# Kr-Stam/CUDA_Optical_Flow_2

Hardware: AMD Instinct MI355X
Metric: Mpix/s dense LK flow (higher is better)
Workload: dtype i32/f64; 1 GPU; 3840x2160 pair, 5-level pyramid, 9x9 window, iters=5 (BASELINE.json config as written; iterations = extension lk_iter: bilinear-warp refinement, iteration 1 = the reference bit for bit), mode lk_float, stream path: new frame's pyramid + every LK level and iteration, inputs resident in HBM; SURVEY 8d's smooth texture translating by (2,1) px per frame; warmup_steps_run=5

## Files before the change

### cuda_optical_flow_2_amd/build.py

```python
from __future__ import annotations

import os
import shutil
import subprocess
import sys
from concurrent.futures import ThreadPoolExecutor

PKG = os.path.dirname(os.path.abspath(__file__))
ROOT = os.path.dirname(PKG)
CSRC = os.path.join(PKG, "csrc")
INCLUDE = os.path.join(ROOT, "include")
OUT = os.path.join(PKG, os.environ.get("OFX_BUILD_OUT", "libofx_hip.so"))
OBJ = os.path.join(PKG, "csrc", "_obj" + os.environ.get("OFX_BUILD_TAG", ""))
ARCH = "gfx950"

SOURCES = ["lk_inst_stream_f8.hip", "lk_inst_stream_fast8.hip", "lk_inst_stream_fw.hip", "lk_inst_stream_fastw.hip", "lk_inst_stream_fwr.hip", "lk_inst_stream_fastwr.hip", "lk_inst_iter_f4.hip", "lk_inst_iter_fast4.hip", "lk_inst_stream_f.hip", "lk_inst_stream_fast.hip", "lk_inst_stream_c.hip", "lk_inst_levels_f.hip", "lk_inst_levels_fast.hip",
           "lk_inst_levels_c.hip", "lk_inst_iter_f2.hip", "lk_inst_iter_fast2.hip", "lk_inst_iter_f3.hip", "lk_inst_iter_fast3.hip", "lk_inst_iter_f1.hip", "lk_inst_iter_fast1.hip", "lk_level.hip", "corner.hip", "pyr_corner.hip", "pyramid.hip", "compose_ring.hip", "sample_ring.hip", "frontend.hip", "primitives.hip", "srm_march.hip", "ofx_core.cpp", "session.cpp",
           "compat_gpu.cpp", "compat_cpu.cpp", "compat_stage.cpp"]
FLAGS = ["-O3", "-std=c++17", "-fPIC", "-ffp-contract=off", "-fno-slp-vectorize", f"--offload-arch={ARCH}", "-I" + INCLUDE, "-I" + CSRC,
         "-Wall", "-Wno-unused-function"] + os.environ.get("OFX_BUILD_DEFS", "").split()


def hipcc() -> str:
    exe = shutil.which("hipcc") or "/opt/rocm/bin/hipcc"
    if not os.path.exists(exe):
        raise RuntimeError("hipcc not found: the HIP library cannot be built (there is no CPU fallback)")
    return exe


def _stale(target: str, deps) -> bool:
    if not os.path.exists(target):
        return True
    t = os.path.getmtime(target)
    return any(os.path.getmtime(d) > t for d in deps)


def _headers():
    hs = [os.path.join(CSRC, f) for f in os.listdir(CSRC) if f.endswith(".h")]
    hs += [os.path.join(INCLUDE, f) for f in os.listdir(INCLUDE)]
    return hs


def build(force: bool = False, verbose: bool = False) -> str:
    os.makedirs(OBJ, exist_ok=True)
    cc = hipcc()
    hdrs = _headers()
    srcs = [s for s in SOURCES if os.path.exists(os.path.join(CSRC, s))]
    jobs = []
    for s in srcs:
        src = os.path.join(CSRC, s)
        obj = os.path.join(OBJ, s + ".o")
        if force or _stale(obj, [src] + hdrs):
            lang = ["-x", "hip"] if s.endswith(".cpp") else []
            jobs.append((s, [cc] + FLAGS + lang + ["-c", src, "-o", obj]))

    def run(job):
        name, cmd = job
        r = subprocess.run(cmd, capture_output=True, text=True)
        if r.returncode != 0:
            raise RuntimeError(f"hipcc failed on {name}:\n{r.stderr}")
        if verbose and r.stderr.strip():
            print(r.stderr, file=sys.stderr)
        return name

    if jobs:
        with ThreadPoolExecutor(max_workers=min(os.cpu_count() or 4, 8, len(jobs))) as ex:
            list(ex.map(run, jobs))
    objs = [os.path.join(OBJ, s + ".o") for s in srcs]
    if force or jobs or _stale(OUT, objs):
        cmd = [cc, "-shared", "-fPIC", "-pthread", "-Wl,--no-undefined", f"--offload-arch={ARCH}", "-o", OUT] + objs + ["-ldl"]
        r = subprocess.run(cmd, capture_output=True, text=True)
        if r.returncode != 0:
            raise RuntimeError("link failed:\n" + r.stderr)
    return OUT


if __name__ == "__main__":
    print(build(force="--force" in sys.argv, verbose=True))
```

### cuda_optical_flow_2_amd/csrc/lk_body.h

```cpp
#pragma once

#include <type_traits>

#include "lk_solve.h"
#include "ofx_internal.h"

namespace ofx_dev {

struct LkArgs {
    const uint8_t *prev;
    const uint8_t *next;
    const float *uv;
    float *flow;
    int32_t *sums;
    size_t sums_plane;
    int w, h, pitch, row0, row_end;
    int out_y0, out_y1, flow_row0;
    int strip_h, tiles_x;
    int accumulate;
    float min_det;
    const uint8_t *warp_src;
    uint8_t *warp_out;
    float warp_scale;
    int *warp_status;
    int warp_status_bit;
};

struct LkTable {
    LkArgs lv[OFX_MAX_LK_ITEMS];
    int first_block[OFX_MAX_LK_ITEMS + 1];
    int n;
};

#define OFX_GLOBAL __attribute__((address_space(1)))
struct __attribute__((packed)) UnalignedU32 {
    uint32_t v;
};
typedef float f32x2 __attribute__((ext_vector_type(2)));
typedef float f32x4 __attribute__((ext_vector_type(4)));
__device__ __forceinline__ uint32_t lane_off(uint32_t off)
{
    asm volatile("" : "+v"(off));
    return off;
}
__device__ __forceinline__ uint32_t lane_off_var(uint32_t &off)
{
    asm volatile("" : "+v"(off));
    return off;
}
__device__ __forceinline__ uint32_t gload_u32_var(const uint8_t *base, uint32_t &off)
{
    return *(const OFX_GLOBAL uint32_t *)((const OFX_GLOBAL uint8_t *)base + lane_off_var(off));
}
__device__ __forceinline__ uint32_t gload_u32_unaligned_var(const uint8_t *base, uint32_t &off)
{
    return ((const OFX_GLOBAL UnalignedU32 *)((const OFX_GLOBAL uint8_t *)base + lane_off_var(off)))->v;
}
__device__ __forceinline__ uint32_t gload_u32(const uint8_t *base, uint32_t off)
{
    return *(const OFX_GLOBAL uint32_t *)((const OFX_GLOBAL uint8_t *)base + lane_off(off));
}
__device__ __forceinline__ uint32_t gload_u32_nt(const uint8_t *base, uint32_t off)
{
    return __builtin_nontemporal_load((const OFX_GLOBAL uint32_t *)((const OFX_GLOBAL uint8_t *)base + lane_off(off)));
}
typedef OFX_GLOBAL float *gfloat_ptr;
__device__ __forceinline__ gfloat_ptr gptr_f32_var(float *base, uint32_t &byte_off)
{
    return (gfloat_ptr)((OFX_GLOBAL uint8_t *)base + lane_off_var(byte_off));
}
__device__ __forceinline__ void gstore_f32x2(gfloat_ptr p, float a, float b)
{
    __builtin_nontemporal_store(f32x2{a, b}, (OFX_GLOBAL f32x2 *)p);
}
__device__ __forceinline__ void gstore_f32x4(gfloat_ptr p, f32x4 v)
{
    typedef float f32x4_a8 __attribute__((ext_vector_type(4), aligned(8)));
    __builtin_nontemporal_store((f32x4_a8)v, (OFX_GLOBAL f32x4_a8 *)p);
}
__device__ __forceinline__ void gstore_i32(int32_t *p, int32_t v) { *(OFX_GLOBAL int32_t *)p = v; }
__device__ __forceinline__ void gstore_u32(uint8_t *base, uint32_t off, uint32_t v)
{
    *(OFX_GLOBAL uint32_t *)((OFX_GLOBAL uint8_t *)base + lane_off(off)) = v;
}
__device__ __forceinline__ void gstore_u32x2(uint8_t *base, uint32_t off, uint32_t a, uint32_t b)
{
    typedef uint32_t u32x2 __attribute__((ext_vector_type(2), aligned(4)));
    *(OFX_GLOBAL u32x2 *)((OFX_GLOBAL uint8_t *)base + lane_off(off)) = u32x2{a, b};
}
__device__ __forceinline__ void gstore_u16(uint8_t *base, uint32_t off, uint16_t v)
{
    *(OFX_GLOBAL uint16_t *)((OFX_GLOBAL uint8_t *)base + lane_off(off)) = v;
}
__device__ __forceinline__ void gstore_u8(uint8_t *base, uint32_t off, uint8_t v) { *((OFX_GLOBAL uint8_t *)base + lane_off(off)) = v; }

template <typename T>
__device__ __forceinline__ void pin_scalar(T &x)
{
    asm volatile("" : "+s"(x));
}

__device__ __forceinline__ int lane_shift_right(int x)
{
    int r = __builtin_amdgcn_update_dpp(0, x, 0x138 , 0xf, 0xf, true);
    asm volatile("" : "+v"(r));
    return r;
}
__device__ __forceinline__ int lane_shift_left(int x)
{
    int r = __builtin_amdgcn_update_dpp(0, x, 0x130 , 0xf, 0xf, true);
    asm volatile("" : "+v"(r));
    return r;
}

template <int D>
__device__ __forceinline__ int lane_from(int x)
{
    if constexpr (D == 0) {
        return x;
    } else if constexpr (D > 0) {
        return lane_from<D - 1>(lane_shift_left(x));
    } else {
        return lane_from<D + 1>(lane_shift_right(x));
    }
}

template <int D>
__device__ __forceinline__ int add_from(int acc, int x)
{
    if constexpr (D == 0) {
        return acc + x;
    } else {
        const int near = lane_from<(D > 0 ? D - 1 : D + 1)>(x);
        int r = acc + __builtin_amdgcn_update_dpp(0, near, D > 0 ? 0x130  : 0x138 , 0xf, 0xf, true);
        asm volatile("" : "+v"(r));
        return r;
    }
}

template <int R, int I, int D>
__device__ __forceinline__ int hbox_right(const int (&q)[4], int acc)
{
    constexpr int hi = I + R;
    if constexpr (hi < 4 * D) {
        return acc;
    } else if constexpr (hi >= 4 * D + 3) {
        return hbox_right<R, I, D + 1>(q, add_from<D>(acc, q[3]));
    } else {
        return add_from<D>(acc, q[hi - 4 * D]);
    }
}

template <int R, int I, int D>
__device__ __forceinline__ int hbox_left(const int (&s)[4], int acc)
{
    constexpr int lo = I - R;
    if constexpr (lo > -4 * D + 3) {
        return acc;
    } else if constexpr (lo <= -4 * D) {
        return hbox_left<R, I, D + 1>(s, add_from<-D>(acc, s[0]));
    } else {
        return add_from<-D>(acc, s[lo + 4 * D]);
    }
}

template <int R, int I>
__device__ __forceinline__ int hbox_one(const int (&q)[4], const int (&s)[4])
{
    constexpr int lo = I - R, hi = I + R;
    constexpr int olo = lo > 0 ? lo : 0, ohi = hi < 3 ? hi : 3;
    int own;
    if constexpr (olo == 0) {
        own = q[ohi];
    } else if constexpr (ohi == 3) {
        own = s[olo];
    } else {
        own = q[ohi] - q[olo - 1];
    }
    return hbox_left<R, I, 1>(s, hbox_right<R, I, 1>(q, own));
}

template <int C>
__device__ __forceinline__ int col_minus(const int (&a)[4], int y)
{
    if constexpr (C >= 0 && C <= 3) {
        return a[C] - y;
    } else {
        constexpr int idx = ((C % 4) + 4) % 4;
        constexpr int dist = (C - idx) / 4;
        const int near = lane_from<(dist > 0 ? dist - 1 : dist + 1)>(a[idx]);
        int r = __builtin_amdgcn_update_dpp(0, near, dist > 0 ? 0x130  : 0x138 , 0xf, 0xf, true) - y;
        asm volatile("" : "+v"(r));
        return r;
    }
}

template <int R>
__device__ __forceinline__ void hbox4(const int (&a)[4], int (&out)[4])
{
    int q[4], s[4];
    q[0] = a[0];
    q[1] = q[0] + a[1];
    q[2] = q[1] + a[2];
    q[3] = q[2] + a[3];
    s[3] = a[3];
    s[2] = s[3] + a[2];
    s[1] = s[2] + a[1];
    s[0] = q[3];
    out[0] = hbox_one<R, 0>(q, s);
    out[3] = hbox_one<R, 3>(q, s);
    out[1] = col_minus<1 + R>(a, col_minus<0 - R>(a, out[0]));
    out[2] = col_minus<2 - R>(a, col_minus<3 + R>(a, out[3]));
}

template <int K>
__device__ __forceinline__ void lane_from5(const int (&x)[5], int (&r)[5])
{
    if constexpr (K == 0) {
#pragma unroll
        for (int n = 0; n < 5; ++n) r[n] = x[n];
    } else {
        int t[5];
#pragma unroll
        for (int n = 0; n < 5; ++n) t[n] = K > 0 ? lane_shift_left(x[n]) : lane_shift_right(x[n]);
        lane_from5<(K > 0 ? K - 1 : K + 1)>(t, r);
    }
}

template <int D>
__device__ __forceinline__ void add_from5(int (&acc)[5], const int (&x)[5])
{
    if constexpr (D == 0) {
#pragma unroll
        for (int n = 0; n < 5; ++n) acc[n] += x[n];
    } else {
        int near[5];
        lane_from5<(D > 0 ? D - 1 : D + 1)>(x, near);
#pragma unroll
        for (int n = 0; n < 5; ++n) {
            int r = acc[n] + __builtin_amdgcn_update_dpp(0, near[n], D > 0 ? 0x130  : 0x138 , 0xf, 0xf, true);
            asm volatile("" : "+v"(r));
            acc[n] = r;
        }
    }
}

template <int C>
__device__ __forceinline__ void column5(const int (&a)[5][4], int (&x)[5])
{
#pragma unroll
    for (int n = 0; n < 5; ++n) x[n] = a[n][C];
}

template <int R, int I, int D>
__device__ __forceinline__ void hbox_right5(const int (&q)[5][4], int (&acc)[5])
{
    constexpr int hi = I + R;
    if constexpr (hi < 4 * D) {
        return;
    } else if constexpr (hi >= 4 * D + 3) {
        int x[5];
        column5<3>(q, x);
        add_from5<D>(acc, x);
        hbox_right5<R, I, D + 1>(q, acc);
    } else {
        int x[5];
        column5<hi - 4 * D>(q, x);
        add_from5<D>(acc, x);
    }
}

template <int R, int I, int D>
__device__ __forceinline__ void hbox_left5(const int (&s)[5][4], int (&acc)[5])
{
    constexpr int lo = I - R;
    if constexpr (lo > -4 * D + 3) {
        return;
    } else if constexpr (lo <= -4 * D) {
        int x[5];
        column5<0>(s, x);
        add_from5<-D>(acc, x);
        hbox_left5<R, I, D + 1>(s, acc);
    } else {
        int x[5];
        column5<lo + 4 * D>(s, x);
        add_from5<-D>(acc, x);
    }
}

template <int R, int I>
__device__ __forceinline__ void hbox_one5(const int (&q)[5][4], const int (&s)[5][4], int (&out)[5])
{
    constexpr int lo = I - R, hi = I + R;
    constexpr int olo = lo > 0 ? lo : 0, ohi = hi < 3 ? hi : 3;
#pragma unroll
    for (int n = 0; n < 5; ++n) {
        if constexpr (olo == 0) out[n] = q[n][ohi];
        else if constexpr (ohi == 3) out[n] = s[n][olo];
        else out[n] = q[n][ohi] - q[n][olo - 1];
    }
    hbox_right5<R, I, 1>(q, out);
    hbox_left5<R, I, 1>(s, out);
}

template <int C>
__device__ __forceinline__ void col_minus5(const int (&a)[5][4], const int (&y)[5], int (&r)[5])
{
    if constexpr (C >= 0 && C <= 3) {
#pragma unroll
        for (int n = 0; n < 5; ++n) r[n] = a[n][C] - y[n];
    } else {
        constexpr int idx = ((C % 4) + 4) % 4;
        constexpr int dist = (C - idx) / 4;
        int x[5], near[5];
        column5<idx>(a, x);
        lane_from5<(dist > 0 ? dist - 1 : dist + 1)>(x, near);
#pragma unroll
        for (int n = 0; n < 5; ++n) {
            int t = __builtin_amdgcn_update_dpp(0, near[n], dist > 0 ? 0x130  : 0x138 , 0xf, 0xf, true) - y[n];
            asm volatile("" : "+v"(t));
            r[n] = t;
        }
    }
}

template <int R>
__device__ __forceinline__ void hbox4x5(const int (&a)[5][4], int (&out)[5][4])
{
    int q[5][4], s[5][4];
#pragma unroll
    for (int n = 0; n < 5; ++n) {
        q[n][0] = a[n][0];
        q[n][1] = q[n][0] + a[n][1];
        q[n][2] = q[n][1] + a[n][2];
        q[n][3] = q[n][2] + a[n][3];
        s[n][3] = a[n][3];
        s[n][2] = s[n][3] + a[n][2];
        s[n][1] = s[n][2] + a[n][1];
        s[n][0] = q[n][3];
    }
    int o0[5], o1[5], o2[5], o3[5];
    hbox_one5<R, 0>(q, s, o0);
    hbox_one5<R, 3>(q, s, o3);
    int t[5];
    col_minus5<0 - R>(a, o0, t);
    col_minus5<1 + R>(a, t, o1);
    col_minus5<3 + R>(a, o3, t);
    col_minus5<2 - R>(a, t, o2);
#pragma unroll
    for (int n = 0; n < 5; ++n) out[n][0] = o0[n], out[n][1] = o1[n], out[n][2] = o2[n], out[n][3] = o3[n];
}

template <int R>
struct TileGeom {
    static constexpr int LO_LANE = (R + 1 + 3) / 4;
    static constexpr int HI_LANE = (251 - R) / 4;
    static constexpr int OUT_W = (HI_LANE - LO_LANE + 1) * 4;
};

typedef short s2 __attribute__((ext_vector_type(2)));

__device__ __forceinline__ s2 as_s2(uint32_t v) { return __builtin_bit_cast(s2, v); }
__device__ __forceinline__ uint32_t as_u32(s2 v) { return __builtin_bit_cast(uint32_t, v); }
__device__ __forceinline__ s2 lane_shift_s2(s2 v, bool from_left)
{
    return as_s2((uint32_t)(from_left ? lane_shift_right((int)as_u32(v)) : lane_shift_left((int)as_u32(v))));
}

__device__ __forceinline__ s2 pk_two()
{
    uint32_t v = 0x00020002u;
    asm volatile("" : "+s"(v));
    return as_s2(v);
}

template <int MODE>
struct RowPk;
template <>
struct RowPk<OFX_MODE_LK_FLOAT> {
    s2 p[4];
    s2 d[4];
};
template <>
struct RowPk<OFX_MODE_COMPAT_CPU> {
    s2 p[4];
    s2 n[4];
};

__device__ __forceinline__ void pin_row(RowPk<OFX_MODE_LK_FLOAT> &r)
{
    asm volatile("" : "+v"(r.p[0]), "+v"(r.p[1]), "+v"(r.p[2]), "+v"(r.p[3]), "+v"(r.d[0]), "+v"(r.d[1]), "+v"(r.d[2]), "+v"(r.d[3]));
}
__device__ __forceinline__ void pin_row(RowPk<OFX_MODE_COMPAT_CPU> &r)
{
    asm volatile("" : "+v"(r.p[0]), "+v"(r.p[1]), "+v"(r.p[2]), "+v"(r.p[3]), "+v"(r.n[0]), "+v"(r.n[1]), "+v"(r.n[2]), "+v"(r.n[3]));
}

template <int J>
__device__ __forceinline__ s2 pair_bytes(uint32_t in_raw, uint32_t out_raw)
{
    constexpr uint32_t sel = (uint32_t)J | (0x0cu << 8) | ((uint32_t)(4 + J) << 16) | (0x0cu << 24);
    return as_s2(__builtin_amdgcn_perm(out_raw, in_raw, sel));
}

__device__ __forceinline__ void unpack_pk(uint32_t pi, uint32_t ni, uint32_t po, uint32_t no, RowPk<OFX_MODE_LK_FLOAT> &r)
{
    r.p[0] = pair_bytes<0>(pi, po);
    r.p[1] = pair_bytes<1>(pi, po);
    r.p[2] = pair_bytes<2>(pi, po);
    r.p[3] = pair_bytes<3>(pi, po);
    r.d[0] = pair_bytes<0>(ni, no) - r.p[0];
    r.d[1] = pair_bytes<1>(ni, no) - r.p[1];
    r.d[2] = pair_bytes<2>(ni, no) - r.p[2];
    r.d[3] = pair_bytes<3>(ni, no) - r.p[3];
}

__device__ __forceinline__ void unpack_pk(uint32_t pi, uint32_t ni, uint32_t po, uint32_t no, RowPk<OFX_MODE_COMPAT_CPU> &r)
{
    r.p[0] = pair_bytes<0>(pi, po);
    r.p[1] = pair_bytes<1>(pi, po);
    r.p[2] = pair_bytes<2>(pi, po);
    r.p[3] = pair_bytes<3>(pi, po);
    r.n[0] = pair_bytes<0>(ni, no);
    r.n[1] = pair_bytes<1>(ni, no);
    r.n[2] = pair_bytes<2>(ni, no);
    r.n[3] = pair_bytes<3>(ni, no);
}

__device__ __forceinline__ void derivs_pk(const RowPk<OFX_MODE_LK_FLOAT> &t, const RowPk<OFX_MODE_LK_FLOAT> &m,
                                          const RowPk<OFX_MODE_LK_FLOAT> &b, const s2 two, s2 (&ix)[4], s2 (&iy)[4], s2 (&it)[4])
{
    s2 sm[6], df[6], g[6];
#pragma unroll
    for (int j = 0; j < 4; ++j) {
        sm[j + 1] = m.p[j] * two + (t.p[j] + b.p[j]);
        df[j + 1] = b.p[j] - t.p[j];
        g[j + 1] = m.d[j] * two + (t.d[j] + b.d[j]);
    }
    sm[0] = lane_shift_s2(sm[4], true);
    sm[5] = lane_shift_s2(sm[1], false);
    df[0] = lane_shift_s2(df[4], true);
    df[5] = lane_shift_s2(df[1], false);
    g[0] = lane_shift_s2(g[4], true);
    g[5] = lane_shift_s2(g[1], false);
#pragma unroll
    for (int j = 0; j < 4; ++j) {
        ix[j] = sm[j + 2] - sm[j];
        iy[j] = df[j + 1] * two + (df[j] + df[j + 2]);
        it[j] = g[j + 1] * two + (g[j] + g[j + 2]) - m.d[j];
    }
}

__device__ __forceinline__ void derivs_pk(const RowPk<OFX_MODE_COMPAT_CPU> &t, const RowPk<OFX_MODE_COMPAT_CPU> &m,
                                          const RowPk<OFX_MODE_COMPAT_CPU> &b, const s2, s2 (&ix)[4], s2 (&iy)[4], s2 (&it)[4])
{
    s2 sm[6], df[6], sp[6], sn[6], mp[4], mn[4];
#pragma unroll
    for (int j = 0; j < 4; ++j) {
        sm[j + 1] = (m.p[j] + m.p[j]) + t.p[j] + b.p[j];
        df[j + 1] = b.p[j] - t.p[j];
        sp[j + 1] = (t.p[j] >> 4) + (m.p[j] >> 3) + (b.p[j] >> 4);
        sn[j + 1] = (t.n[j] >> 4) + (m.n[j] >> 3) + (b.n[j] >> 4);
        mp[j] = (t.p[j] >> 3) + (m.p[j] >> 2) + (b.p[j] >> 3);
        mn[j] = (t.n[j] >> 3) + (m.n[j] >> 2) + (b.n[j] >> 3);
    }
    sm[0] = lane_shift_s2(sm[4], true);
    sm[5] = lane_shift_s2(sm[1], false);
    df[0] = lane_shift_s2(df[4], true);
    df[5] = lane_shift_s2(df[1], false);
    sp[0] = lane_shift_s2(sp[4], true);
    sp[5] = lane_shift_s2(sp[1], false);
    sn[0] = lane_shift_s2(sn[4], true);
    sn[5] = lane_shift_s2(sn[1], false);
#pragma unroll
    for (int j = 0; j < 4; ++j) {
        constexpr uint32_t m8 = 0x00ff00ffu;
        ix[j] = as_s2(as_u32(sm[j + 2] - sm[j]) & m8);
        iy[j] = as_s2(as_u32((df[j + 1] + df[j + 1]) + df[j] + df[j + 2]) & m8);
        const s2 gp = sp[j] + mp[j] + sp[j + 2], gn = sn[j] + mn[j] + sn[j + 2];
        it[j] = as_s2(as_u32(gn - gp) & 0x00ff00ffu);
    }
}

__device__ __forceinline__ void accumulate_pk(const s2 (&ix)[4], const s2 (&iy)[4], const s2 (&it)[4], const uint32_t (&mm)[4],
                                              int (&vxx)[4], int (&vyy)[4], int (&vxy)[4], int (&vxt)[4], int (&vyt)[4])
{
#pragma unroll
    for (int j = 0; j < 4; ++j) {
        const s2 nx = ix[j] * as_s2(mm[j]), ny = iy[j] * as_s2(mm[j]);
        vxx[j] = __builtin_amdgcn_sdot2(ix[j], nx, vxx[j], false);
        vyy[j] = __builtin_amdgcn_sdot2(iy[j], ny, vyy[j], false);
        vxy[j] = __builtin_amdgcn_sdot2(ix[j], ny, vxy[j], false);
        vxt[j] = __builtin_amdgcn_sdot2(nx, it[j], vxt[j], false);
        vyt[j] = __builtin_amdgcn_sdot2(ny, it[j], vyt[j], false);
    }
}

constexpr int kLkWaveLds = 2048 + 128;
typedef __attribute__((address_space(3))) uint8_t *lds_ptr;

template <int R, int MODE, bool SUMS, bool MAY_ACC, bool FAST, bool INTERIOR>
__device__ __forceinline__ void lk_wave_impl(const LkTable &T, int wave, int lane, uint8_t *xlds)
{
    using G = TileGeom<R>;
    constexpr int NS = 2 * R + 1;

    if (wave >= T.first_block[T.n]) return;
    int level = 0, hi = T.n;
    while (hi - level > 1) {
        const int mid = (level + hi) >> 1;
        if (wave >= T.first_block[mid]) level = mid;
        else hi = mid;
    }
    LkArgs A = T.lv[level];
    pin_scalar(A.prev);
    pin_scalar(A.next);
    pin_scalar(A.flow);
    pin_scalar(A.w);
    pin_scalar(A.h);
    pin_scalar(A.pitch);
    pin_scalar(A.row0);
    pin_scalar(A.row_end);
    pin_scalar(A.flow_row0);
    pin_scalar(A.accumulate);
    pin_scalar(A.min_det);
    const SolveOpts sopt{A.min_det};
    if constexpr (SUMS) {
        pin_scalar(A.sums);
        pin_scalar(A.sums_plane);
    }
    const int block = wave - T.first_block[level];
    const int tile = block % A.tiles_x;
    const int strip = block / A.tiles_x;
    const int cb = tile * G::OUT_W - G::LO_LANE * 4 + 4 * lane;
    const int ys = A.out_y0 + strip * A.strip_h;
    const int ye = min(ys + A.strip_h, A.out_y1);

    const bool ld_ok = INTERIOR || (cb >= 0 && cb < A.w);
    uint32_t bmask = INTERIOR ? 0xffffffffu : 0u;
    int cm[4] = {-1, -1, -1, -1};
    if constexpr (!INTERIOR) {
#pragma unroll
        for (int j = 0; j < 4; ++j) {
            const bool in = (cb + j) >= 0 && (cb + j) < A.w;
            cm[j] = in ? -1 : 0;
            bmask |= in ? (0xffu << (8 * j)) : 0u;
        }
    }
    uint32_t col_off = ld_ok ? (uint32_t)cb : 0u;
    uint32_t flow_off = 8u * (uint32_t)(cb > 0 ? cb : 0);
    const int x0 = tile * G::OUT_W;
    const int nv = min(x0 + G::OUT_W, A.w) - x0;
    uint32_t l16 = 16u * (uint32_t)lane;
    const int lim = 8 * nv - 16, c16 = 16 * lane;
    const bool st_lo4 = c16 <= lim, st_lo2 = c16 == lim + 8, st_hi4 = c16 <= lim - 1024, st_hi2 = c16 == lim + 8 - 1024;
    const lds_ptr xl_w = (lds_ptr)xlds + 32 * lane;
    const lds_ptr xl_base = (lds_ptr)xlds + 32 * G::LO_LANE;

    const int y_lim = min(min(ye + R + 1, A.h), A.row_end);
    const int y_min = max(0, A.row0);
    auto fetch_row = [&](const uint8_t *img, int y) -> uint32_t {
        uint32_t v = 0u;
        if (y >= y_min && y < y_lim) {
            const uint8_t *row = img + (size_t)(uint32_t)(y - A.row0) * (size_t)(uint32_t)A.pitch;
            pin_scalar(row);
            v = gload_u32_var(row, col_off);
        }
        return v;
    };
    auto finish_row = [&](uint32_t raw) -> uint32_t {
        if constexpr (INTERIOR) return raw;
        else return raw & bmask;
    };

    const float su = A.uv ? A.uv[0] : 0.0f, sv = A.uv ? A.uv[1] : 0.0f;
    uint32_t nb_off = 0u, sel = 0u, own_sel = 0u;
    bool all_in;
    {
        int n[4], nb = 0x7fffffff;
        bool in[4], lane_all_in = true;
#pragma unroll
        for (int j = 0; j < 4; ++j) {
            const int x = cb + j;
            const float tx = (float)x + su;
            in[j] = x >= 0 && x < A.w && tx > -1.0f && tx < (float)A.w;
            n[j] = in[j] ? (int)tx : 0;
            if (in[j]) nb = min(nb, n[j]);
        }
        nb = max(0, min(nb == 0x7fffffff ? 0 : nb, A.pitch - 4));
        sel = 0u;
#pragma unroll
        for (int j = 0; j < 4; ++j) {
            const int x = cb + j;
            const uint32_t sj = !(x >= 0 && x < A.w) ? 0x0cu : (in[j] ? (uint32_t)(n[j] - nb) : (uint32_t)(4 + j));
            sel |= sj << (8 * j);
            own_sel |= (!(x >= 0 && x < A.w) ? 0x0cu : (uint32_t)(4 + j)) << (8 * j);
            if (x >= 0 && x < A.w && !in[j]) lane_all_in = false;
        }
        nb_off = (uint32_t)nb;
        all_in = __all(lane_all_in) != 0;
    }
    const int y_none = (A.h + 2) / 3, y_part = (A.h % 3) ? A.h / 3 : -1;
    struct NextRaw {
        uint32_t own, sh;
        uint32_t have;
    };
    int map_base = 0, row_map = -1;
    auto refresh_map = [&](int y0) {
        map_base = y0;
        const float ty = (float)(y0 + lane) + sv;
        const bool yin = ty > -1.0f && ty < (float)A.h;
        const int ny = yin ? (int)ty : 0;
        row_map = (yin && ny >= A.row0 && ny < A.row_end) ? ny : -1;
    };
    auto fetch_next = [&](int y) -> NextRaw {
        NextRaw r = {0u, 0u, 0u};
        if (y >= y_min && y < y_lim) {
            const int ny = __builtin_amdgcn_readlane(row_map, y - map_base);
            const bool have = ny >= 0;
            r.have = have ? ~0u : 0u;
            if (have) {
                const uint8_t *srow = A.next + (size_t)(uint32_t)(ny - A.row0) * (size_t)(uint32_t)A.pitch;
                pin_scalar(srow);
                r.sh = gload_u32_unaligned_var(srow, nb_off);
            }
            if (!(have && all_in) && y < y_none) {
                const uint8_t *orow = A.next + (size_t)(uint32_t)(y - A.row0) * (size_t)(uint32_t)A.pitch;
                pin_scalar(orow);
                r.own = gload_u32_var(orow, col_off);
                if (y == y_part) {
                    uint32_t km = 0u;
#pragma unroll
                    for (int j = 0; j < 4; ++j)
                        if (3ll * (cb + j) < (long long)A.w * (A.h % 3)) km |= 0xffu << (8 * j);
                    r.own &= km;
                }
            }
        }
        return r;
    };
    auto finish_next = [&](const NextRaw &r) -> uint32_t {
        return __builtin_amdgcn_perm(r.own, r.sh, (sel & r.have) | (own_sel & ~r.have));
    };
    auto load_row = [&](const uint8_t *img, int y) -> uint32_t { return finish_row(fetch_row(img, y)); };
    auto load_next = [&](int y) -> uint32_t { return finish_next(fetch_next(y)); };

    constexpr int H = R - 1;
    constexpr int PR = 2 * R - H;
    const int y_first = ys - R;
    const int y_lo0 = y_first + H;
    const int nsteps = (ye - ys) + PR;
    RowPk<MODE> wp[3];
    const s2 two = pk_two();
    auto fetch_out_prev = [&](int r) -> uint32_t { return r < y_first - 1 ? 0u : fetch_row(A.prev, r); };
    auto fetch_out_next = [&](int r) -> NextRaw { return r < y_first - 1 ? NextRaw{0u, 0u, 0u} : fetch_next(r); };
    refresh_map(y_first - 1);
    if constexpr (H > 0) {
        unpack_pk(load_row(A.prev, y_lo0 - 1), load_next(y_lo0 - 1), load_row(A.prev, y_first - 1), load_next(y_first - 1), wp[0]);
        unpack_pk(load_row(A.prev, y_lo0), load_next(y_lo0), load_row(A.prev, y_first), load_next(y_first), wp[1]);
        unpack_pk(load_row(A.prev, y_lo0 + 1), load_next(y_lo0 + 1), load_row(A.prev, y_first + 1), load_next(y_first + 1), wp[2]);
    } else {
        unpack_pk(load_row(A.prev, y_lo0 - 1), load_next(y_lo0 - 1), 0u, 0u, wp[0]);
        unpack_pk(load_row(A.prev, y_lo0), load_next(y_lo0), 0u, 0u, wp[1]);
        unpack_pk(load_row(A.prev, y_lo0 + 1), load_next(y_lo0 + 1), 0u, 0u, wp[2]);
    }

    int vxx[4] = {0, 0, 0, 0}, vyy[4] = {0, 0, 0, 0}, vxy[4] = {0, 0, 0, 0}, vxt[4] = {0, 0, 0, 0}, vyt[4] = {0, 0, 0, 0};

    auto body = [&](auto K, int s) {
        constexpr int k = decltype(K)::value;
        const int yy = y_lo0 + s;
        const int yo = yy - NS;
        const bool folded = H > 0 && s < H;
        const int yh = folded ? y_first + s : yo;

        if (yy + 2 - map_base >= 64) refresh_map(yo + 2);
        const int ro = (H > 1 && s + 1 < H) ? y_first + s + 2 : yo + 2;
        const uint32_t pf_ip = fetch_row(A.prev, yy + 2), pf_op = fetch_out_prev(ro);
        const NextRaw pf_in = fetch_next(yy + 2), pf_on = fetch_out_next(ro);
        const bool emit = s >= PR;
        const int y = yy - R;
        const bool out_lane = lane >= G::LO_LANE && lane <= G::HI_LANE && cb < A.w;
        const size_t rowpix = (size_t)(y - A.flow_row0) * (size_t)A.w;
        float old_uv[8] = {0.0f, 0.0f, 0.0f, 0.0f, 0.0f, 0.0f, 0.0f, 0.0f};
        if constexpr (!SUMS && MAY_ACC) {
            if (A.accumulate && emit && out_lane) {
                float *frow = A.flow + 2 * rowpix;
                pin_scalar(frow);
                const gfloat_ptr src = gptr_f32_var(frow, flow_off);
#pragma unroll
                for (int j = 0; j < 4; ++j)
                    if (cb + j < A.w) old_uv[2 * j] = src[2 * j], old_uv[2 * j + 1] = src[2 * j + 1];
            }
        }

        const uint32_t him = folded ? 0x00010000u : (yo >= y_first ? 0xffff0000u : 0u);
        uint32_t rowm = ((yy >= 0 && yy < A.h) ? 0x00000001u : 0u) | ((yh >= 0 && yh < A.h) ? him : 0u);
        if constexpr (INTERIOR) rowm = (uint32_t)__builtin_amdgcn_readfirstlane((int)rowm);
        const uint32_t mm[4] = {(uint32_t)cm[0] & rowm, (uint32_t)cm[1] & rowm, (uint32_t)cm[2] & rowm, (uint32_t)cm[3] & rowm};
        s2 ix[4], iy[4], it[4];
        derivs_pk(wp[k], wp[(k + 1) % 3], wp[(k + 2) % 3], two, ix, iy, it);
        accumulate_pk(ix, iy, it, mm, vxx, vyy, vxy, vxt, vyt);
        auto take_rows = [&]() {
            __builtin_amdgcn_sched_barrier(0);
            unpack_pk(finish_row(pf_ip), finish_next(pf_in), finish_row(pf_op), finish_next(pf_on), wp[k]);
            pin_row(wp[k]);
        };

        int hxx[4], hyy[4], hxy[4], hxt[4], hyt[4];
        float uv[8];
        f32x4 xlo, xhi;
        asm("" : "=v"(xlo), "=v"(xhi));
        if (emit) {
            hbox4<R>(vxx, hxx);
            hbox4<R>(vyy, hyy);
            hbox4<R>(vxy, hxy);
            hbox4<R>(vxt, hxt);
            hbox4<R>(vyt, hyt);
            if constexpr (!SUMS) {
                solve_lane<MODE, FAST>(hxx, hyy, hxy, hxt, hyt, sopt, uv);
                if constexpr (MAY_ACC) {
                    if (A.accumulate) {
#pragma unroll
                        for (int j = 0; j < 8; ++j) uv[j] = old_uv[j] + uv[j];
                    }
                }
                *(__attribute__((address_space(3))) f32x4 *)(xl_w) = f32x4{uv[0], uv[1], uv[2], uv[3]};
                *(__attribute__((address_space(3))) f32x4 *)(xl_w + 16) = f32x4{uv[4], uv[5], uv[6], uv[7]};
                __builtin_amdgcn_fence(__ATOMIC_SEQ_CST, "wavefront");
                __builtin_amdgcn_wave_barrier();
                const lds_ptr xl_r = xl_base + lane_off_var(l16);
                xlo = *(__attribute__((address_space(3))) f32x4 *)(xl_r);
                xhi = *(__attribute__((address_space(3))) f32x4 *)(xl_r + 1024);
            }
        }
        take_rows();
        if (emit) {
            if constexpr (SUMS) {
                if (out_lane) {
                    const size_t pix = rowpix + (uint32_t)cb;
#pragma unroll
                    for (int j = 0; j < 4; ++j) {
                        if (cb + j < A.w) {
                            gstore_i32(A.sums + pix + j, hxx[j]);
                            gstore_i32(A.sums + A.sums_plane + pix + j, hyy[j]);
                            gstore_i32(A.sums + 2 * A.sums_plane + pix + j, hxy[j]);
                            gstore_i32(A.sums + 3 * A.sums_plane + pix + j, hxt[j]);
                            gstore_i32(A.sums + 4 * A.sums_plane + pix + j, hyt[j]);
                        }
                    }
                }
            } else {
                float *frow = A.flow + 2 * (rowpix + (size_t)x0);
                pin_scalar(frow);
                if (st_lo4) {
                    gstore_f32x4(gptr_f32_var(frow, l16), xlo);
                } else if (st_lo2) {
                    gstore_f32x2(gptr_f32_var(frow, l16), xlo.x, xlo.y);
                }
                if (st_hi4) {
                    gstore_f32x4(gptr_f32_var(frow, l16) + 256, xhi);
                } else if (st_hi2) {
                    gstore_f32x2(gptr_f32_var(frow, l16) + 256, xhi.x, xhi.y);
                }
            }
        }
    };

    const int q1 = nsteps / 4, q2 = nsteps / 2, q3 = nsteps - nsteps / 4;
    __builtin_amdgcn_s_setprio(3);
#define OFX_LK_PRIO_STEP()                               \
    do {                                                 \
        if (s >= q3) __builtin_amdgcn_s_setprio(0);      \
        else if (s >= q2) __builtin_amdgcn_s_setprio(1); \
        else if (s >= q1) __builtin_amdgcn_s_setprio(2); \
    } while (0)
    int s = 0;
    while (true) {
        body(std::integral_constant<int, 0>{}, s);
        if (++s >= nsteps) break;
        body(std::integral_constant<int, 1>{}, s);
        if (++s >= nsteps) break;
        body(std::integral_constant<int, 2>{}, s);
        if (++s >= nsteps) break;
        OFX_LK_PRIO_STEP();
    }
}


}
#include "lk_body_warp.h"
#include "lk_body_buf.h"
#include "lk_body_wide.h"
#undef OFX_LK_PRIO_STEP
namespace ofx_dev {

template <int R, int MODE, bool SUMS, bool MAY_ACC = true, bool FAST = false, bool LDS_ROWS = false, int ITER = 0>
__device__ __forceinline__ void lk_wave(const LkTable &T, int wave, int lane, uint8_t *xlds)
{
    if (wave >= T.first_block[T.n]) return;
    int level = 0, hi = T.n;
    while (hi - level > 1) {
        const int mid = (level + hi) >> 1;
        if (wave >= T.first_block[mid]) level = mid;
        else hi = mid;
    }
    const int tile = (wave - T.first_block[level]) % T.lv[level].tiles_x;
    const int cb0 = tile * TileGeom<R>::OUT_W - TileGeom<R>::LO_LANE * 4;
    if constexpr (!SUMS && !MAY_ACC) {
        if (cb0 >= 0 && cb0 + 256 <= T.lv[level].w) lk_wave_buf<R, MODE, FAST, true, LDS_ROWS, ITER>(T, wave, lane, xlds);
        else lk_wave_buf<R, MODE, FAST, false, LDS_ROWS, ITER>(T, wave, lane, xlds);
        return;
    }
    if (cb0 >= 0 && cb0 + 256 <= T.lv[level].w) lk_wave_impl<R, MODE, SUMS, MAY_ACC, FAST, true>(T, wave, lane, xlds);
    else lk_wave_impl<R, MODE, SUMS, MAY_ACC, FAST, false>(T, wave, lane, xlds);
}

}
```

### cuda_optical_flow_2_amd/csrc/lk_inst.h

```cpp
#pragma once

#include "lk_launch.h"

namespace ofx_launch {

template <int MODE, bool FAST>
int levels(int radius, const LkLevelIn *lv, int n, bool sums, hipStream_t st)
{
    int rc = OFX_E_UNSUPPORTED;
    const bool known = dispatch_radius<lk_max_radius(MODE)>(radius, [&](auto R) {
        if constexpr (!FAST) {
            if (sums) {
                rc = launch_r<decltype(R)::value, MODE, true, false>(lv, n, st);
                return;
            }
        }
        rc = launch_r<decltype(R)::value, MODE, false, FAST>(lv, n, st);
    });
    if (!known) ofx_set_error("ofx_lk_level: window %d not supported in mode %d", 2 * radius + 1, MODE);
    return rc;
}

template <int MODE, bool FAST, int ITER, int NC>
int iter(int radius, const LkLevelIn *lv, int n, hipStream_t st)
{
    int rc = OFX_E_UNSUPPORTED;
    const bool known = dispatch_radius<lk_max_radius(MODE, NC)>(radius, [&](auto R) {
        if constexpr (NC == 8) rc = launch_iter_rd<decltype(R)::value, MODE, FAST, ITER, false, 8>(lv, n, st);
        else rc = launch_iter_r<decltype(R)::value, MODE, FAST, ITER>(lv, n, st);
    });
    if (!known) {
        if constexpr (NC == 8) ofx_set_error("ofx_lk_levels: window %d not supported with eight columns per lane", 2 * radius + 1);
        else ofx_set_error("ofx_lk_level: window %d not supported in mode %d", 2 * radius + 1, MODE);
    }
    return rc;
}

template <int MODE, bool FAST, int WOUT, int NC>
int stream(int radius, const LkLevelIn *lv, int n, StreamArgs &S, const int *stage_blocks, size_t lds, hipStream_t st)
{
    int rc = OFX_E_UNSUPPORTED;
    const bool known = dispatch_radius<lk_max_radius(MODE, NC)>(radius, [&](auto R) {
        if constexpr (NC == 8) rc = launch_stream_rd<decltype(R)::value, MODE, FAST, false, WOUT, 8>(lv, n, S, stage_blocks, lds, st);
        else rc = launch_stream_r<decltype(R)::value, MODE, FAST, WOUT>(lv, n, S, stage_blocks, lds, st);
    });
    if (!known) {
        if constexpr (NC == 8) ofx_set_error("ofx_stream_launch: window %d not supported with eight columns per lane", 2 * radius + 1);
        else ofx_set_error("ofx_stream_launch: window %d not supported in mode %d", 2 * radius + 1, MODE);
    }
    return rc;
}

}
```

### cuda_optical_flow_2_amd/csrc/lk_launch.h

```cpp
#pragma once

#include <stdio.h>
#include <stdlib.h>

#include "corner_body.h"
#include "lk_body.h"
#include "pyr_march.h"
#include "stages_body.h"

using namespace ofx_dev;

namespace ofx_launch {
constexpr int kPyrStages = 2 * OFX_STREAM_MAX_BATCH;
using ofx_dev::kCornerScratch;
struct StreamArgs {
    LkTable lk;
    PyrMarchArgs pyr[kPyrStages];
    CornerHead corner[OFX_STREAM_MAX_BATCH];
    CornerLevel corner_lv[OFX_MAX_LK_ITEMS];
    PatchBuild patch;
    int patch_build;
    PatchBuildSlot patch_slot[OFX_STREAM_MAX_BATCH];
    int first[kPyrStages + 1];
    int n_corner;
    unsigned long long *trace;
    int trace_blocks;
};
struct LkLevelIn {
    LkArgs a;
    int rows_out;
};
}

namespace {

constexpr int kLkMinWaves = 3;
template <int R, int MODE, bool SUMS, bool FAST>
__global__ __launch_bounds__(64, kLkMinWaves) void lk_level_kernel(const LkTable T)
{
    __shared__ __attribute__((aligned(16))) uint8_t xlds[kLkWaveLds];
    lk_wave<R, MODE, SUMS, true, FAST>(T, (int)blockIdx.x, (int)threadIdx.x, xlds);
}

template <int R, int MODE, bool FAST, int ITER, bool DMA = false, int NC = 4>
__global__ __launch_bounds__(64, NC == 8 ? 2 : 3) void lk_iter_kernel(const LkTable T)
{
    __shared__ __attribute__((aligned(16))) uint8_t xlds[NC == 8 ? kLkWaveLdsW : (DMA ? kLkWaveLdsDma : kLkWaveLdsX)];
    const int wave = (int)blockIdx.x, lane = (int)threadIdx.x;
    if constexpr (NC == 8) {
        static_assert(!DMA, "the wide march has no deep fetch");
        lk_wave_w<R, MODE, FAST, ITER, 8>(T, wave, lane, xlds);
        return;
    }
    if (wave >= T.first_block[T.n]) return;
    int level = 0, hi = T.n;
    while (hi - level > 1) {
        const int mid = (level + hi) >> 1;
        if (wave >= T.first_block[mid]) level = mid;
        else hi = mid;
    }
    const int tile = (wave - T.first_block[level]) % T.lv[level].tiles_x;
    const int cb0 = tile * TileGeom<R>::OUT_W - TileGeom<R>::LO_LANE * 4;
    if (cb0 >= 0 && cb0 + 256 <= T.lv[level].w) lk_wave_buf<R, MODE, FAST, true, DMA, ITER>(T, wave, lane, xlds);
    else lk_wave_buf<R, MODE, FAST, false, DMA, ITER>(T, wave, lane, xlds);
}

using ofx_launch::kCornerScratch;
using ofx_launch::kPyrStages;
using ofx_launch::StreamArgs;

}
namespace ofx_launch {
extern unsigned long long *g_stream_trace;
extern int g_stream_trace_blocks;
extern int g_trace_header[2 * OFX_STREAM_MAX_BATCH + 1];
extern thread_local int g_stream_deep_fetch;
}
namespace {
using ofx_launch::g_stream_trace;
using ofx_launch::g_stream_trace_blocks;
using ofx_launch::g_trace_header;
using ofx_launch::g_stream_deep_fetch;

constexpr int kPyrPrio = 3;
constexpr int stream_min_blocks(int mode, int wout, int nc)
{
    return nc == 8 ? (wout ? 2 : 3) : (wout ? 3 : (mode == OFX_MODE_LK_FLOAT ? 5 : 4));
}
template <int R, int MODE, bool FAST, bool DMA, int WOUT = 0, int NC = 4>
__global__ __launch_bounds__(256, stream_min_blocks(MODE, WOUT, NC)) void stream_kernel(const StreamArgs S)
{
    extern __shared__ __attribute__((aligned(16))) uint8_t lds[];
    const int b = (int)blockIdx.x, tid = (int)threadIdx.x;
    const unsigned long long t_start = S.trace ? wall_clock64() : 0ull;
    const int wv = __builtin_amdgcn_readfirstlane(tid >> 6);
    if (b < OFX_STREAM_MAX_BATCH) {
        __builtin_amdgcn_s_setprio(3);
        if (b < S.n_corner) {
            if (S.patch_build) patch_build_block(S.patch, S.patch_slot[b], tid);
            corner_block<MODE, FAST>(S.corner[b], S.corner_lv + S.corner[b].lv0, S.patch, tid, wv, reinterpret_cast<float *>(lds), lds + kCornerScratch,
                                     reinterpret_cast<int *>(lds + kCornerScratch - 32));
        }
    } else if (b < S.first[0]) {
        if constexpr (NC == 8) lk_wave_w<R, MODE, FAST, WOUT, 8>(S.lk, 4 * (b - OFX_STREAM_MAX_BATCH) + wv, tid & 63, lds + wv * kLkWaveLdsW);
        else lk_wave<R, MODE, false, false, FAST, DMA, WOUT>(S.lk, 4 * (b - OFX_STREAM_MAX_BATCH) + wv, tid & 63, lds + wv * (DMA ? kLkWaveLdsDma : kLkWaveLdsX));
    } else {
        int i = 0;
        while (i + 1 < kPyrStages && b >= S.first[i + 1]) ++i;
        __builtin_amdgcn_s_setprio(kPyrPrio);
        pyr_march_wave(S.pyr[i], 4 * (b - S.first[i]) + wv, tid & 63);
    }
    if (S.trace && b < S.trace_blocks && (tid & 63) == 0) {
        const unsigned hw = __builtin_amdgcn_s_getreg((4) | (0 << 6) | (15 << 11));
        const unsigned xcc = __builtin_amdgcn_s_getreg((20) | (0 << 6) | (3 << 11));
        S.trace[2 * (4 * b + wv)] = t_start;
        S.trace[2 * (4 * b + wv) + 1] = (wall_clock64() & 0x0000ffffffffffffull) | ((unsigned long long)(hw & 0xffffu) << 48);
        S.trace[2 * (4 * b + wv)] = (t_start & 0x0000ffffffffffffull) | ((unsigned long long)(xcc & 0xfu) << 48);
    }
}

using ofx_launch::LkLevelIn;

int env_int(const char *name, int dflt)
{
    const char *e = getenv(name);
    return e && atoi(e) > 0 ? atoi(e) : dflt;
}

template <int R, int NC = 4>
int plan_table(const LkLevelIn *lv, int n, int capacity, LkTable *out)
{
    using G = TileGeomW<R, NC>;
    const int min_h = env_int("OFX_LK_MIN_STRIP", 8);
    int max_rows = 1;
    for (int i = 0; i < n; ++i) max_rows = lv[i].rows_out > max_rows ? lv[i].rows_out : max_rows;
    auto height = [&](int i, int H) {
        const int hi = H < min_h ? min_h : H;
        return hi < lv[i].rows_out ? hi : lv[i].rows_out;
    };
    auto item_waves = [&](int i, int H) { return (long)ofx_div_up(lv[i].a.w, G::OUT_W) * ofx_div_up(lv[i].rows_out, height(i, H)); };
    int strip_h = min_h;
    for (; strip_h < max_rows; ++strip_h) {
        long waves = 0;
        for (int i = 0; i < n; ++i) waves += item_waves(i, strip_h);
        if (waves <= (long)capacity) break;
    }
    LkTable t{};
    t.n = n;
    int blocks = 0;
    for (int i = 0; i < n; ++i) {
        t.lv[i] = lv[i].a;
        t.lv[i].tiles_x = ofx_div_up(lv[i].a.w, G::OUT_W);
        t.lv[i].strip_h = height(i, strip_h);
        t.first_block[i] = blocks;
        blocks += t.lv[i].tiles_x * ofx_div_up(lv[i].rows_out, t.lv[i].strip_h);
    }
    t.first_block[n] = blocks;
    *out = t;
    return blocks;
}

template <typename K>
int lk_wave_target(K kernel, int threads, size_t lds, int reserve, int dflt_per_simd)
{
    int dev = 0, cus = 256, per_cu = 0;
    hipDeviceProp_t prop;
    if (hipGetDevice(&dev) == hipSuccess && hipGetDeviceProperties(&prop, dev) == hipSuccess) cus = prop.multiProcessorCount;
    if (hipOccupancyMaxActiveBlocksPerMultiprocessor(&per_cu, kernel, threads, lds) != hipSuccess || per_cu <= 0) per_cu = 8 * 64 / threads;
    (void)hipGetLastError();
    const int occ = per_cu * (threads / 64) / 4;
    int per_simd = env_int("OFX_LK_WAVES_PER_SIMD", dflt_per_simd);
    if (per_simd > occ - reserve) per_simd = occ - reserve;
    if (per_simd < 1) per_simd = 1;
    const int fill = env_int("OFX_LK_FILL", per_simd < occ ? 100 : 95);
    return env_int("OFX_LK_TARGET_WAVES", (int)((long)cus * 4 * per_simd * fill / 100));
}

template <int R, int MODE, bool SUMS, bool FAST>
int launch_r(const LkLevelIn *lv, int n, hipStream_t st)
{
    static const int capacity = lk_wave_target(lk_level_kernel<R, MODE, SUMS, FAST>, 64, 0, 0, 4);
    LkTable t{};
    const int blocks = plan_table<R>(lv, n, capacity, &t);
    hipLaunchKernelGGL((lk_level_kernel<R, MODE, SUMS, FAST>), dim3((unsigned)blocks), dim3(64), 0, st, t);
    OFX_HIP(hipGetLastError());
    return OFX_OK;
}

template <int R, int MODE, bool FAST, int ITER, bool DMA, int NC = 4>
int launch_iter_rd(const LkLevelIn *lv, int n, hipStream_t st)
{
    static const int capacity = lk_wave_target(lk_iter_kernel<R, MODE, FAST, ITER, DMA, NC>, 64, 0, 0, NC == 8 ? env_int("OFX_WIDE_WAVES_PER_SIMD", 2) : 4);
    LkTable t{};
    const int blocks = plan_table<R, NC>(lv, n, capacity, &t);
    hipLaunchKernelGGL((lk_iter_kernel<R, MODE, FAST, ITER, DMA, NC>), dim3((unsigned)blocks), dim3(64), 0, st, t);
    OFX_HIP(hipGetLastError());
    return OFX_OK;
}

template <int R, int MODE, bool FAST, int ITER>
int launch_iter_r(const LkLevelIn *lv, int n, hipStream_t st)
{
    static const int forced = [] { const char *e = getenv("OFX_ITER_DMA"); return e ? atoi(e) : -1; }();
    long max_px = 0;
    for (int i = 0; i < n; ++i) max_px = (long)lv[i].a.w * lv[i].a.h > max_px ? (long)lv[i].a.w * lv[i].a.h : max_px;
    if (forced > 0 || (forced < 0 && max_px >= 16l * 1000 * 1000)) return launch_iter_rd<R, MODE, FAST, ITER, true>(lv, n, st);
    return launch_iter_rd<R, MODE, FAST, ITER, false>(lv, n, st);
}

template <int R, int MODE, bool FAST, bool DMA, int WOUT, int NC = 4>
int launch_stream_rd(const LkLevelIn *lv, int n, StreamArgs &S, const int *stage_blocks, size_t lds, hipStream_t st)
{
    constexpr size_t wave_lds = NC == 8 ? kLkWaveLdsW : (DMA ? kLkWaveLdsDma : kLkWaveLdsX);
    static const int capacity1 = lk_wave_target(stream_kernel<R, MODE, FAST, DMA, WOUT, NC>, 256, 4 * wave_lds, 1, NC == 8 ? 1 : 2);
    static const int capacity2 = lk_wave_target(stream_kernel<R, MODE, FAST, DMA, WOUT, NC>, 256, 4 * wave_lds, 1, NC == 8 ? env_int("OFX_WIDE_WAVES_PER_SIMD", 2) : 4);
    int pairs = 0;
    for (int i = 0; i < n; ++i) pairs += (lv[i].a.w == lv[0].a.w && lv[i].a.h == lv[0].a.h) ? 1 : 0;
    const int capacity = pairs >= 2 ? capacity2 : capacity1;
    int lk_blocks = 0;
    if (n > 0) lk_blocks = ofx_div_up(plan_table<R, NC>(lv, n, capacity, &S.lk), 4);
    S.first[0] = OFX_STREAM_MAX_BATCH + lk_blocks;
    for (int i = 0; i < kPyrStages; ++i) S.first[i + 1] = S.first[i] + stage_blocks[i];
    const int blocks = S.first[kPyrStages];
    S.trace = g_stream_trace;
    S.trace_blocks = g_stream_trace_blocks;
    if (g_stream_trace)
        for (int i = 0; i <= kPyrStages; ++i) g_trace_header[i] = S.first[i];
    size_t corner_lds = 0;
    for (int i = 0; i < S.n_corner; ++i) {
        const size_t need = (size_t)kCornerScratch + kCornerTileBytes + (size_t)S.corner[i].levels * kCornerCacheBytes;
        corner_lds = need > corner_lds ? need : corner_lds;
    }
    if (lds < corner_lds) lds = corner_lds;
    if (lds < 4 * wave_lds) lds = 4 * wave_lds;
    hipLaunchKernelGGL((stream_kernel<R, MODE, FAST, DMA, WOUT, NC>), dim3((unsigned)blocks), dim3(256), lds, st, S);
    OFX_HIP(hipGetLastError());
    return OFX_OK;
}

template <int R, int MODE, bool FAST, int WOUT>
int launch_stream_r(const LkLevelIn *lv, int n, StreamArgs &S, const int *stage_blocks, size_t lds, hipStream_t st)
{
    if constexpr (!WOUT) {
        static const int forced = [] { const char *e = getenv("OFX_LK_DMA"); return e ? atoi(e) : -1; }();
        long max_px = 0;
        for (int i = 0; i < n; ++i) max_px = (long)lv[i].a.w * lv[i].a.h > max_px ? (long)lv[i].a.w * lv[i].a.h : max_px;
        const int want = forced >= 0 ? (forced > 0 ? 1 : -1) : g_stream_deep_fetch;
        if (want > 0 || (want == 0 && max_px >= 16l * 1000 * 1000)) return launch_stream_rd<R, MODE, FAST, true, WOUT>(lv, n, S, stage_blocks, lds, st);
    }
    return launch_stream_rd<R, MODE, FAST, false, WOUT>(lv, n, S, stage_blocks, lds, st);
}

template <int MAX_R, int R = 1, typename F>
bool dispatch_radius(int radius, F &&f)
{
    if constexpr (R <= MAX_R) {
        if (radius == R) {
            f(std::integral_constant<int, R>{});
            return true;
        }
        return dispatch_radius<MAX_R, R + 1>(radius, f);
    } else {
        return false;
    }
}
constexpr int lk_max_radius(int mode, int nc = 4) { return mode == OFX_MODE_COMPAT_CPU && nc == 4 ? 12 : 11; }

}

namespace ofx_launch {
template <int MODE, bool FAST>
int levels(int radius, const LkLevelIn *lv, int n, bool sums, hipStream_t st);
template <int MODE, bool FAST, int ITER, int NC = 4>
int iter(int radius, const LkLevelIn *lv, int n, hipStream_t st);
template <int MODE, bool FAST, int WOUT = 0, int NC = 4>
int stream(int radius, const LkLevelIn *lv, int n, StreamArgs &S, const int *stage_blocks, size_t lds, hipStream_t st);
}
```

### cuda_optical_flow_2_amd/csrc/lk_level.hip

```cpp
#include <string.h>

#include "lk_launch.h"


namespace ofx_launch {
unsigned long long *g_stream_trace = nullptr;
int g_stream_trace_blocks = 0;
int g_trace_header[2 * OFX_STREAM_MAX_BATCH + 1] = {0};
thread_local int g_stream_deep_fetch = 0;
}

namespace {

int lk_build_levels(const ofx_lk_desc *d, int n, int window, int mode, int32_t *d_sums, LkLevelIn *lv, int *count)
{
    OFX_REQUIRE(d != nullptr && n >= 1 && n <= OFX_MAX_LK_ITEMS, "ofx_lk_levels: bad descriptor count %d", n);
    OFX_REQUIRE(window >= 3 && (window & 1), "ofx_lk_level: window must be odd and >= 3 (got %d)", window);
    OFX_REQUIRE(mode == OFX_MODE_COMPAT_CPU || mode == OFX_MODE_LK_FLOAT || mode == OFX_MODE_LK_FLOAT_FAST, "ofx_lk_level: bad mode %d", mode);
    const int radius = window >> 1;
    int m = 0;
    for (int i = 0; i < n; ++i) {
        const ofx_geom *g = &d[i].geom;
        OFX_TRY(ofx_check_geom(g, "ofx_lk_level"));
        OFX_REQUIRE(d[i].d_prev && d[i].d_next && (d[i].d_flow || d_sums), "ofx_lk_level: null pointer");
        OFX_REQUIRE(((uintptr_t)d[i].d_prev & 3) == 0 && ((uintptr_t)d[i].d_next & 3) == 0, "ofx_lk_level: planes must be 4-byte aligned");
        OFX_REQUIRE(d[i].flow_row0 <= g->out_y0, "ofx_lk_level: flow_row0 %d > out_y0 %d", d[i].flow_row0, g->out_y0);
        OFX_TRY(ofx_check_halo(g, radius + 1, "ofx_lk_level"));
        const int rows_out = g->out_y1 - g->out_y0;
        if (rows_out <= 0) continue;
        LkArgs a{};
        a.prev = d[i].d_prev;
        a.next = d[i].d_next;
        a.uv = d[i].d_uv;
        a.accumulate = d[i].accumulate;
        a.min_det = d[0].min_det;
        a.flow = d[i].d_flow;
        a.sums = d_sums;
        a.sums_plane = (size_t)(g->out_y1 - d[i].flow_row0) * (size_t)g->w;
        a.w = g->w;
        a.h = g->h;
        a.pitch = g->pitch;
        a.row0 = g->row0;
        a.row_end = g->row0 + g->rows;
        a.out_y0 = g->out_y0;
        a.out_y1 = g->out_y1;
        a.flow_row0 = d[i].flow_row0;
        OFX_REQUIRE((d[i].d_warp_out != nullptr) == (d[0].d_warp_out != nullptr) && (d[i].accumulate != 0) == (d[0].accumulate != 0),
                    "ofx_lk_levels: accumulate and d_warp_out must be set for all descriptors of a launch or for none");
        if (d[i].d_warp_out) {
            OFX_REQUIRE(!d_sums && d[i].d_warp_src && d[i].d_flow, "ofx_lk_levels: d_warp_out needs d_warp_src and d_flow");
            OFX_REQUIRE(d[i].d_warp_out != d[i].d_next && d[i].d_warp_out != d[i].d_warp_src && d[i].d_warp_out != d[i].d_prev,
                        "ofx_lk_levels: d_warp_out must be a plane of its own");
            a.warp_src = d[i].d_warp_src;
            a.warp_out = d[i].d_warp_out;
            a.warp_scale = d[i].warp_scale;
            a.warp_status = d[i].d_warp_status;
            a.warp_status_bit = d[i].warp_status_bit;
            OFX_REQUIRE(a.warp_status == nullptr || (a.warp_status_bit >= 0 && a.warp_status_bit < 31), "ofx_lk_levels: bad warp_status_bit");
        }
        lv[m].a = a;
        lv[m].rows_out = rows_out;
        ++m;
    }
    *count = m;
    return OFX_OK;
}

bool fits_buffer_offsets(const LkArgs &a)
{
    return (long long)(a.row_end - a.row0) * a.pitch < (1ll << 31) && (long long)(a.out_y1 - a.flow_row0) * a.w * 8 < (1ll << 31);
}
bool fit_buffer_offsets(const LkLevelIn *lv, int m)
{
    for (int i = 0; i < m; ++i)
        if (!fits_buffer_offsets(lv[i].a)) return false;
    return true;
}

#ifndef OFX_LK_COLS_DEFAULT
#define OFX_LK_COLS_DEFAULT 4
#endif
int lk_cols(const LkLevelIn *lv, int m, int radius)
{
    static const int forced = [] { const char *e = getenv("OFX_LK_COLS"); return e ? atoi(e) : 0; }();
    static const int dma_forced = [] { const char *e = getenv("OFX_LK_DMA"); return e ? atoi(e) : -1; }();
    if (radius < 1 || radius > 11 || m <= 0) return 4;
    if (dma_forced < 0 && ofx_launch::g_stream_deep_fetch > 0) return 4;
    if (forced == 4 || forced == 8) return forced;
    long max_px = 0;
    for (int i = 0; i < m; ++i) max_px = (long)lv[i].a.w * lv[i].a.h > max_px ? (long)lv[i].a.w * lv[i].a.h : max_px;
    if (dma_forced > 0 || (dma_forced < 0 && max_px >= 16l * 1000 * 1000)) return 4;
    return OFX_LK_COLS_DEFAULT;
}

int lk_dispatch(const ofx_lk_desc *d, int n, int window, int mode, int32_t *d_sums, void *stream)
{
    LkLevelIn lv[OFX_MAX_LK_ITEMS];
    int m = 0;
    OFX_TRY(lk_build_levels(d, n, window, mode, d_sums, lv, &m));
    if (m == 0) return OFX_OK;
    const int radius = window >> 1;
    hipStream_t st = ofx_stream(stream);
    if ((lv[0].a.accumulate || lv[0].a.warp_out) && !d_sums) {
        const bool small = fit_buffer_offsets(lv, m);
        const bool wout = lv[0].a.warp_out != nullptr;
        OFX_REQUIRE(!wout || (small && mode != OFX_MODE_COMPAT_CPU), "ofx_lk_levels: d_warp_out needs mode lk_float and levels below 2 GB");
        bool rowwin = false;
        for (int i = 0; i < m; ++i) rowwin = rowwin || lv[i].a.row0 != 0 || lv[i].a.row_end != lv[i].a.h;
        OFX_REQUIRE(!(wout && rowwin && !lv[0].a.accumulate), "ofx_lk_levels: iteration 1 with d_warp_out on a row window runs in the stream tick only");
        const int iter = wout ? (lv[0].a.accumulate ? (rowwin ? 4 : 2) : 3) : 1;
        if (small && mode != OFX_MODE_COMPAT_CPU) {
            auto run = [&](auto FAST) {
                constexpr bool F = decltype(FAST)::value;
                switch (iter) {
                case 1: return ofx_launch::iter<OFX_MODE_LK_FLOAT, F, 1>(radius, lv, m, st);
                case 2: return ofx_launch::iter<OFX_MODE_LK_FLOAT, F, 2>(radius, lv, m, st);
                case 3: return ofx_launch::iter<OFX_MODE_LK_FLOAT, F, 3>(radius, lv, m, st);
                default: return ofx_launch::iter<OFX_MODE_LK_FLOAT, F, 4>(radius, lv, m, st);
                }
            };
            return mode == OFX_MODE_LK_FLOAT_FAST ? run(std::true_type{}) : run(std::false_type{});
        }
    }
    static const bool plain_wide = [] { const char *e = getenv("OFX_LK_PLAIN_COLS"); return e && atoi(e) == 8; }();
    if (plain_wide && !d_sums && mode == OFX_MODE_LK_FLOAT && !lv[0].a.accumulate && !lv[0].a.warp_out && radius >= 1 && radius <= 11 &&
        fit_buffer_offsets(lv, m))
        return ofx_launch::iter<OFX_MODE_LK_FLOAT, false, 0, 8>(radius, lv, m, st);
    const bool sums = d_sums != nullptr;
    if (mode == OFX_MODE_COMPAT_CPU) return ofx_launch::levels<OFX_MODE_COMPAT_CPU, false>(radius, lv, m, sums, st);
    if (mode == OFX_MODE_LK_FLOAT_FAST && !sums) return ofx_launch::levels<OFX_MODE_LK_FLOAT, true>(radius, lv, m, false, st);
    return ofx_launch::levels<OFX_MODE_LK_FLOAT, false>(radius, lv, m, sums, st);
}

}

extern "C" int ofx_stream_launch(const ofx_stream_stages *g, int window, int mode, void *stream)
{
    OFX_REQUIRE(g != nullptr, "ofx_stream_launch: null argument");
    OFX_REQUIRE(window >= 3 && (window & 1), "ofx_stream_launch: window must be odd and >= 3 (got %d)", window);
    OFX_REQUIRE(mode == OFX_MODE_COMPAT_CPU || mode == OFX_MODE_LK_FLOAT || mode == OFX_MODE_LK_FLOAT_FAST, "ofx_stream_launch: bad mode %d", mode);
    OFX_REQUIRE(g->n_pyr >= 0 && g->n_pyr <= OFX_STREAM_MAX_BATCH && g->n_corner >= 0 && g->n_corner <= OFX_STREAM_MAX_BATCH,
                "ofx_stream_launch: at most %d frames / pairs per tick", OFX_STREAM_MAX_BATCH);
    StreamArgs S{};
    size_t lds = 0;
    int stage_blocks[kPyrStages] = {0};
    int any = 0;
    static const int simds = [] {
        int dev = 0, cus = 256;
        hipDeviceProp_t prop;
        if (hipGetDevice(&dev) == hipSuccess && hipGetDeviceProperties(&prop, dev) == hipSuccess) cus = prop.multiProcessorCount;
        return 4 * cus;
    }();
    const int pyr_target = g->n_pyr > 0 ? env_int("OFX_PYR_WAVES", simds * 85 / 100) / g->n_pyr : 0;
    for (int i = 0; i < g->n_pyr; ++i) {
        const ofx_pyramid_stage &P = g->pyr[i];
        if (P.levels < 2) continue;
        int items = 0;
        OFX_TRY(ofx_pyramid_march_args(P.d_frame, P.frame_pitch, P.w, P.h, P.d_levels, P.pitches, P.levels, P.d_levels[0], P.pitches[0],
                                       P.windowed ? P.row0 : nullptr, P.windowed ? P.rows : nullptr, pyr_target, &S.pyr[2 * i], &items));
        stage_blocks[2 * i] = ofx_div_up(items, 4);
        if (P.patch_levels >= 2) {
            OFX_REQUIRE(P.patch_w > 0 && P.patch_h > 0 && P.patch_w <= P.w && P.patch_h <= P.h,
                        "ofx_stream_launch: the patch must lie inside the frame");
            OFX_TRY(ofx_pyramid_march_args(P.d_frame, P.frame_pitch, P.patch_w, P.patch_h, P.d_patch_levels, P.patch_pitches, P.patch_levels,
                                           P.d_patch_levels[0], P.patch_pitches[0], nullptr, nullptr, 16, &S.pyr[2 * i + 1], &items));
            stage_blocks[2 * i + 1] = ofx_div_up(items, 4);
        }
        any += stage_blocks[2 * i] + stage_blocks[2 * i + 1];
    }
    int n_clv = 0, n_build = 0;
    for (int i = 0; i < g->n_corner; ++i) {
        const ofx_corner_stage &C = g->corner[i];
        OFX_REQUIRE(C.levels > 0, "ofx_stream_launch: empty corner stage");
        OFX_REQUIRE(n_clv + C.levels <= OFX_MAX_LK_ITEMS, "ofx_stream_launch: the corner stages have more than %d (pair, level) items", OFX_MAX_LK_ITEMS);
        OFX_TRY(ofx_corner_args(C.level, C.levels, window, mode, C.d_uv, C.cols, C.d_status, &C.shard_rows[0][0], &S.corner[i], S.corner_lv + n_clv));
        S.corner[i].lv0 = n_clv;
        n_clv += C.levels;
        const bool reloc = C.levels >= 2 && C.d_patch_reloc[1] != nullptr;
        S.corner[i].pair_status = C.d_pair_status;
        if (C.build_patch || reloc) {
            OFX_REQUIRE(C.levels >= 2 && C.patch_w > 0 && C.patch_h > 0, "ofx_stream_launch: corner stage %d: incomplete patch description", i);
            OFX_REQUIRE(!C.build_patch || (C.d_patch_src[0] && C.d_patch_src[1] && C.d_patch[0][1] && C.d_patch[1][1]),
                        "ofx_stream_launch: corner stage %d: incomplete patch description", i);
            uint8_t *const *planes = C.build_patch ? C.d_patch[0] : C.d_patch_reloc;
            PatchBuild pb{};
            pb.n = C.levels - 1;
            pb.frame_stride = C.build_patch ? (int)(C.d_patch[1][1] - C.d_patch[0][1]) : 0;
            for (int k = 0; k < C.levels; ++k) {
                pb.pw[k] = C.patch_w >> k;
                pb.ph[k] = C.patch_h >> k;
                pb.pitch[k] = k ? C.patch_pitch[k] : 0;
                pb.off[k] = k ? (int)(planes[k] - planes[1]) : 0;
                OFX_REQUIRE(pb.pw[k] > 0 && pb.ph[k] > 0, "ofx_stream_launch: the patch is too small for %d levels", C.levels);
                if (k) {
                    OFX_REQUIRE(planes[k] != nullptr && (C.patch_pitch[k] & 3) == 0 && C.patch_pitch[k] >= ((pb.pw[k] + 3) & ~3) && ((uintptr_t)planes[k] & 3) == 0,
                                "ofx_stream_launch: corner stage %d: bad patch plane at level %d", i, k);
                    OFX_REQUIRE(!C.build_patch || C.d_patch[1][k] == C.d_patch[0][k] + pb.frame_stride,
                                "ofx_stream_launch: corner stage %d: bad patch plane at level %d", i, k);
                    OFX_REQUIRE(!reloc || (C.d_patch_reloc[k] != nullptr && C.d_patch_reloc[k] - C.d_patch_reloc[1] == pb.off[k] && ((uintptr_t)C.d_patch_reloc[k] & 3) == 0),
                                "ofx_stream_launch: corner stage %d: the relocated patch planes must be laid out like the patch planes (level %d)", i, k);
                    OFX_REQUIRE(((C.patch_w >> (k - 1)) & 1) == 0 && ((C.patch_h >> (k - 1)) & 1) == 0, "ofx_stream_launch: the patch must have even dimensions below its top level");
                }
            }
            if (C.build_patch)
                for (int f = 0; f < 2; ++f)
                    OFX_REQUIRE((C.patch_src_pitch[f] & 3) == 0 && C.patch_src_pitch[f] >= C.patch_w && ((uintptr_t)C.d_patch_src[f] & 3) == 0,
                                "ofx_stream_launch: corner stage %d: bad patch source", i);
            if (reloc) {
                const ofx_geom &g0 = C.level[0].geom;
                OFX_REQUIRE(g0.row0 == 0 && g0.rows == g0.h && (C.cols[0] == 0 || C.cols[0] >= g0.w),
                            "ofx_stream_launch: corner stage %d: the repair needs level 0 to be the whole frames", i);
                OFX_REQUIRE(C.patch_w <= g0.w && C.patch_h <= g0.h, "ofx_stream_launch: corner stage %d: the patch must lie inside the frame", i);
                const int lc = C.levels - 1, need = (window >> 1) + 5;
                OFX_REQUIRE((pb.pw[lc] >= need || pb.pw[lc] >= (g0.w >> lc)) && (pb.ph[lc] >= need || pb.ph[lc] >= (g0.h >> lc)),
                            "ofx_stream_launch: corner stage %d: a %dx%d patch leaves %dx%d at the coarsest level, the repair needs %d", i, C.patch_w,
                            C.patch_h, pb.pw[lc], pb.ph[lc], need);
                S.corner[i].reloc = C.d_patch_reloc[1];
            }
            if (S.patch.n == 0) S.patch = pb;
            else OFX_REQUIRE(memcmp(&S.patch, &pb, sizeof pb) == 0, "ofx_stream_launch: the corner stages of a launch must share one patch geometry");
            if (C.build_patch) {
                S.patch_slot[i] = PatchBuildSlot{{C.d_patch_src[0], C.d_patch_src[1]}, {C.patch_src_pitch[0], C.patch_src_pitch[1]}, C.d_patch[0][1]};
                ++n_build;
            }
        }
    }
    OFX_REQUIRE(n_build == 0 || n_build == g->n_corner, "ofx_stream_launch: either every corner stage builds its patch or none does");
    S.patch_build = n_build > 0 ? 1 : 0;
    S.n_corner = g->n_corner;
    LkLevelIn lv[OFX_MAX_LK_ITEMS];
    int m = 0;
    if (g->n_lk > 0) {
        OFX_REQUIRE(!g->lk[0].accumulate, "ofx_stream_launch: a tick's LK stage is iteration 1 (no accumulate)");
        OFX_REQUIRE(g->lk[0].d_warp_out == nullptr || mode != OFX_MODE_COMPAT_CPU, "ofx_stream_launch: d_warp_out needs mode lk_float");
        OFX_TRY(lk_build_levels(g->lk, g->n_lk, window, mode, nullptr, lv, &m));
    }
    for (int i = 0; i < m; ++i) {
        const LkArgs &a = lv[i].a;
        OFX_REQUIRE(fits_buffer_offsets(a),
                    "ofx_stream_launch: level %dx%d is too large for one launch item (planes and flow rows must stay below 2 GB: "
                    "shard the level by rows)", a.w, a.h);
    }
    if (any == 0 && m == 0 && g->n_corner == 0) return OFX_OK;
    hipStream_t st = ofx_stream(stream);
    OFX_REQUIRE(g->deep_fetch >= -1 && g->deep_fetch <= 1, "ofx_stream_launch: deep_fetch must be -1, 0 or +1 (got %d)", g->deep_fetch);
    ofx_launch::g_stream_deep_fetch = g->deep_fetch;
    const int radius = window >> 1;
    if (mode == OFX_MODE_COMPAT_CPU) return ofx_launch::stream<OFX_MODE_COMPAT_CPU, false>(radius, lv, m, S, stage_blocks, lds, st);
    auto tick = [&](auto FAST) {
        constexpr bool F = decltype(FAST)::value;
        if (m > 0 && lv[0].a.warp_out) {
            bool rw = false;
            for (int i = 0; i < m; ++i) rw = rw || lv[i].a.row0 != 0 || lv[i].a.row_end != lv[i].a.h;
            return rw ? ofx_launch::stream<OFX_MODE_LK_FLOAT, F, 5>(radius, lv, m, S, stage_blocks, lds, st)
                      : ofx_launch::stream<OFX_MODE_LK_FLOAT, F, 3>(radius, lv, m, S, stage_blocks, lds, st);
        }
        if (lk_cols(lv, m, radius) == 8) return ofx_launch::stream<OFX_MODE_LK_FLOAT, F, 0, 8>(radius, lv, m, S, stage_blocks, lds, st);
        return ofx_launch::stream<OFX_MODE_LK_FLOAT, F>(radius, lv, m, S, stage_blocks, lds, st);
    };
    return mode == OFX_MODE_LK_FLOAT_FAST ? tick(std::true_type{}) : tick(std::false_type{});
}

extern "C" int ofx_debug_stream_trace(unsigned long long *d_buf, int capacity_blocks, int *first)
{
    g_stream_trace = d_buf;
    g_stream_trace_blocks = d_buf ? capacity_blocks : 0;
    if (first)
        for (int i = 0; i <= kPyrStages; ++i) first[i] = g_trace_header[i];
    return OFX_OK;
}

extern "C" int ofx_lk_levels(const ofx_lk_desc *levels, int n, int window, int mode, void *stream)
{
    return lk_dispatch(levels, n, window, mode, nullptr, stream);
}

extern "C" int ofx_lk_level(const uint8_t *d_prev, const uint8_t *d_next, const ofx_geom *g, int window, int mode,
                            float *d_flow, int flow_row0, void *stream)
{
    OFX_REQUIRE(d_flow && g, "ofx_lk_level: null argument");
    ofx_lk_desc d{d_prev, d_next, *g, d_flow, flow_row0, nullptr, 0, 0.0f};
    return lk_dispatch(&d, 1, window, mode, nullptr, stream);
}

extern "C" int ofx_lk_level_sums(const uint8_t *d_prev, const uint8_t *d_next, const ofx_geom *g, int window, int mode,
                                 int32_t *d_sums5, int flow_row0, void *stream)
{
    OFX_REQUIRE(d_sums5 && g, "ofx_lk_level_sums: null argument");
    ofx_lk_desc d{d_prev, d_next, *g, nullptr, flow_row0, nullptr, 0, 0.0f};
    return lk_dispatch(&d, 1, window, mode, d_sums5, stream);
}
```

### cuda_optical_flow_2_amd/csrc/ofx_internal.h

```cpp
#pragma once

#include <hip/hip_runtime.h>
#include <stdint.h>

#include "ofx.h"

void ofx_set_error(const char *fmt, ...) __attribute__((format(printf, 1, 2)));

#define OFX_HIP(call)                                                                                    \
    do {                                                                                                 \
        hipError_t e_ = (call);                                                                          \
        if (e_ != hipSuccess) {                                                                          \
            ofx_set_error("%s: %s (%s:%d)", #call, hipGetErrorString(e_), __FILE__, __LINE__);           \
            return OFX_E_HIP;                                                                            \
        }                                                                                                \
    } while (0)

#define OFX_REQUIRE(cond, ...)          \
    do {                                \
        if (!(cond)) {                  \
            ofx_set_error(__VA_ARGS__); \
            return OFX_E_INVALID;       \
        }                               \
    } while (0)

#define OFX_TRY(expr)               \
    do {                            \
        int rc_ = (expr);           \
        if (rc_ != OFX_OK) return rc_; \
    } while (0)

static inline hipStream_t ofx_stream(void *s) { return reinterpret_cast<hipStream_t>(s); }

static inline int ofx_div_up(int a, int b) { return (a + b - 1) / b; }

void ofx_range_push(const char *name);
void ofx_range_pop(void);
struct OfxRange {
    explicit OfxRange(const char *name) { ofx_range_push(name); }
    ~OfxRange() { ofx_range_pop(); }
    OfxRange(const OfxRange &) = delete;
    OfxRange &operator=(const OfxRange &) = delete;
};

int ofx_check_geom(const ofx_geom *g, const char *who);

int ofx_check_halo(const ofx_geom *g, int halo, const char *who);

namespace ofx_dev {
struct PyrArgs;
struct PyrMarchArgs;
struct ShiftTable;
struct CornerHead;
struct CornerLevel;
}
int ofx_pyramid_args(const uint8_t *d_level0, int pitch0, int w, int h, uint8_t *const *d_levels, const int *pitches, int levels,
                     uint8_t *d_level0_copy, int copy_pitch, const int *row0, const int *rows, ofx_dev::PyrArgs *out,
                     size_t *lds_bytes, int *blocks_x, int *blocks_y);
int ofx_pyramid_march_args(const uint8_t *d_level0, int pitch0, int w, int h, uint8_t *const *d_levels, const int *pitches, int levels,
                           uint8_t *d_level0_copy, int copy_pitch, const int *row0, const int *rows, int target_waves,
                           ofx_dev::PyrMarchArgs *out, int *items);
int ofx_shift_table(const ofx_shift_desc *levels, int n, ofx_dev::ShiftTable *out, int *blocks_out);
int ofx_corner_args(const ofx_lk_desc *levels, int n_levels, int window, int mode, float *d_uv, const int *cols, int *d_status,
                    const int *shard_rows, ofx_dev::CornerHead *out, ofx_dev::CornerLevel *lv_out);
int ofx_pyramid_corner_1ch(const uint8_t *d_level0, int pitch0, int w, int h, uint8_t *const *d_levels, const int *pitches, int levels,
                           const ofx_corner_stage *C, int first, int window, int mode, void *stream);
int ofx_shard_margin_check(const float *d_uv, int levels, const int *heights, const int *shard_rows, int *d_status, void *stream);

struct ofx_compose_batch {
    const float *lv[OFX_STREAM_MAX_BATCH][OFX_MAX_LEVELS];
    float *dst[OFX_STREAM_MAX_BATCH];
    int own0[OFX_MAX_LEVELS];
    int n, w, rows, levels, level;
    unsigned n_px;
};
int ofx_compose_batch_launch(const ofx_compose_batch *a, void *stream);

struct ofx_sample_batch {
    const float *lv[OFX_STREAM_MAX_BATCH][OFX_MAX_LEVELS];
    int32_t *arrows[OFX_STREAM_MAX_BATCH];
    float *hist[OFX_STREAM_MAX_BATCH];
    float *points;
    int32_t *status;
    int own0[OFX_MAX_LEVELS];
    int n, levels;
    int a_level, a_w, a_h, a_offset, a_ny, a_nx;
    int t_level, t_w, t_h, n_points, pair0;
};
int ofx_sample_batch_launch(const ofx_sample_batch *a, void *stream);
int ofx_arrow_grid(int w, int h, int arrow_res, int *offset, int *ny, int *nx, const char *who);
int ofx_check_sample_pyramid(int w, int h, int levels, int level, const char *who);

struct ofx_frontend_tables;
int ofx_frontend_tables_make(int window, double sigma_s, double sigma_b, ofx_frontend_tables **out);
void ofx_frontend_tables_free(ofx_frontend_tables *t);
int ofx_frontend_run(const ofx_frontend_tables *t, const uint8_t *const *src3, const int *src_pitch, uint8_t *const *dst, const int *dst_pitch,
                     const int *modes, int n, int w, int h, hipStream_t st);
```

### cuda_optical_flow_2_amd/csrc/session.cpp

```cpp
#include <stdlib.h>
#include <string.h>

#include <new>
#include <vector>

#include "compat_scratch.h"
#include "ofx_internal.h"

namespace {
constexpr size_t kAlign = 256;
constexpr int kMaxBatch = OFX_STREAM_MAX_BATCH;
constexpr int kSets = 3 * kMaxBatch + 2;
constexpr int kUvSlots = 2 * kMaxBatch;
inline size_t align_up(size_t v, size_t a) { return (v + a - 1) / a * a; }
}

struct ofx_session {
    ofx_params p{};
    int w[OFX_MAX_LEVELS]{}, h[OFX_MAX_LEVELS]{}, pitch[OFX_MAX_LEVELS]{};
    int own0[OFX_MAX_LEVELS]{}, own1[OFX_MAX_LEVELS]{};
    int buf0[OFX_MAX_LEVELS]{}, buf1[OFX_MAX_LEVELS]{};
    int cmp0[OFX_MAX_LEVELS]{}, cmp1[OFX_MAX_LEVELS]{};
    int fl0[OFX_MAX_LEVELS]{}, fl1[OFX_MAX_LEVELS]{};
    size_t flow_own_offset(int k) const { return (size_t)(own0[k] - fl0[k]) * (size_t)w[k] * 2; }
    uint8_t *img[kSets][OFX_MAX_LEVELS]{};
    uint8_t *sh[2][OFX_MAX_LEVELS]{};
    uint8_t *itsh[kMaxBatch][3][OFX_MAX_LEVELS]{};
    bool fused_iters = false;
    int cur = 0, sht = 0;
    uint8_t *plane[3][OFX_MAX_LEVELS]{};
    hipStream_t aux = nullptr;
    hipEvent_t ev_ready = nullptr;
    hipEvent_t ev_set_done[3] = {nullptr, nullptr, nullptr};
    bool set_busy[3] = {false, false, false};
    bool staged = false;
    int uv_slot = 0;
    float *uv_cur() { return uv + (size_t)uv_slot * 2 * OFX_MAX_LEVELS; }
    long stream_n = -1;
    long stream_frames = -1;
    int pitch0_next() const { return pitch[0]; }
    uint8_t *pimg[kSets][OFX_MAX_LEVELS]{};
    int pw[OFX_MAX_LEVELS]{}, ph[OFX_MAX_LEVELS]{}, ppitch[OFX_MAX_LEVELS]{};
    uint8_t *pscr[kMaxBatch][2][OFX_MAX_LEVELS]{};
    uint8_t *preloc[kMaxBatch][OFX_MAX_LEVELS]{};
    bool repair = false;
    bool plain_fuse = false;
    bool corner_done = false;
    int pset_img[2] = {-1, -1};
    long pset_gen[2] = {0, 0}, img_gen[3] = {0, 0, 0};
    int debug_extent = 0;
    int *corner_status = nullptr;
    int *pair_status = nullptr;
    const uint8_t *pframe[3] = {nullptr, nullptr, nullptr};
    float *flow[OFX_MAX_LEVELS]{};
    float *flowset[kMaxBatch][OFX_MAX_LEVELS]{};
    const uint8_t *held_frame[kMaxBatch]{};
    int held_pitch[kMaxBatch]{};
    int n_held = 0;
    const uint8_t *bframe[kSets]{};
    int bpitch[kSets]{};
    long reported = 0;
    long corner_newest = 0;
    float *uv = nullptr;
    uint8_t *staging = nullptr;
    void *arena = nullptr;
    size_t arena_bytes = 0;
    bool have_next = false, have_prev = false;
    bool timing = false;
    std::vector<hipEvent_t> ev;
    std::vector<int> ev_kind;
    size_t ev_used = 0;
    hipEvent_t ev_frame = nullptr;
    int n_sets = 0;
    float *ring = nullptr;
    size_t ring_stride = 0;
    int ring_slots = 0, ring_level = 0;
    long composed = 0;
    int32_t *arrow_ring = nullptr;
    size_t arrow_stride = 0;
    int arrow_slots = 0, arrow_level = 0, arrow_offset = 0, arrow_ny = 0, arrow_nx = 0;
    float *trk_points = nullptr, *trk_hist = nullptr;
    int32_t *trk_status = nullptr;
    size_t trk_stride = 0;
    int trk_n = 0, trk_slots = 0, trk_level = 0;
    long sampled = 0;
    int fe_mode = 0, fe_flags = 0;
    ofx_frontend_tables *fe = nullptr;
    void *fe_arena = nullptr;
    uint8_t *fplane[kSets]{};
    int stream_input = 0;
};

template <typename F>
static int timed_launch(ofx_session *s, int kind, void *stream, F &&launch)
{
    static const char *const names[OFX_TIME_KINDS] = {"ofx.lk_levels", "ofx.lk_levels_accumulate", "ofx.warp_levels", "ofx.stream_tick",
                                                      "ofx.shift_levels", "ofx.corner_flows", "ofx.pyramid", "ofx.lk_levels_accumulate_warp",
                                                      "ofx.compose_ring"};
    OfxRange range(names[kind]);
    const bool timed = s->timing && s->ev_used + 2 <= s->ev.size();
    if (timed) OFX_HIP(hipEventRecord(s->ev[s->ev_used], ofx_stream(stream)));
    OFX_TRY(launch());
    if (timed) {
        OFX_HIP(hipEventRecord(s->ev[s->ev_used + 1], ofx_stream(stream)));
        s->ev_kind[s->ev_used / 2] = kind;
        s->ev_used += 2;
    }
    return OFX_OK;
}

static void repoint(ofx_session *s)
{
    for (int k = 0; k < s->p.levels; ++k) {
        s->plane[0][k] = s->img[s->cur][k];
        s->plane[1][k] = s->img[(s->cur + 1) % 3][k];
        s->plane[2][k] = s->sh[s->sht][k];
    }
    const size_t skip = (size_t)s->buf0[0] * (size_t)s->pitch[0];
    if (s->pframe[s->cur]) s->plane[0][0] = const_cast<uint8_t *>(s->pframe[s->cur]) + skip;
    if (s->pframe[(s->cur + 1) % 3]) s->plane[1][0] = const_cast<uint8_t *>(s->pframe[(s->cur + 1) % 3]) + skip;
}

static ofx_geom level_geom(const ofx_session *s, int k, int out0, int out1)
{
    ofx_geom g;
    g.w = s->w[k];
    g.h = s->h[k];
    g.pitch = s->pitch[k];
    g.row0 = s->buf0[k];
    g.rows = s->buf1[k] - s->buf0[k];
    g.out_y0 = out0;
    g.out_y1 = out1;
    return g;
}

extern "C" int ofx_session_create(const ofx_params *p_in, ofx_session **out)
{
    OFX_REQUIRE(p_in && out, "ofx_session_create: null argument");
    ofx_params eff = *p_in;
    if (eff.levels == 1 && eff.iters > 1 && eff.borrow_frames) eff.borrow_frames = 0, eff.stream_two_stage = 0;
    const ofx_params *p = &eff;
    OFX_REQUIRE(p->width > 0 && p->height > 0, "ofx_session_create: bad size %dx%d", p->width, p->height);
    OFX_REQUIRE(p->levels >= 1 && p->levels <= OFX_MAX_LEVELS, "ofx_session_create: levels %d out of range", p->levels);
    OFX_REQUIRE(p->window >= 3 && (p->window & 1), "ofx_session_create: window must be odd and >= 3");
    OFX_REQUIRE(p->mode == OFX_MODE_COMPAT_CPU || p->mode == OFX_MODE_LK_FLOAT || p->mode == OFX_MODE_LK_FLOAT_FAST,
                "ofx_session_create: bad mode %d", p->mode);
    OFX_REQUIRE(p->min_det >= 0.0f, "ofx_session_create: min_det must be >= 0 (0 = the reference's unguarded solve)");
    OFX_REQUIRE(p->iters >= 0 && p->iters <= 64, "ofx_session_create: iters %d out of range", p->iters);
    OFX_REQUIRE(p->stream_batch >= 0 && p->stream_batch <= OFX_STREAM_MAX_BATCH, "ofx_session_create: stream_batch %d (0 .. %d)", p->stream_batch,
                OFX_STREAM_MAX_BATCH);
    OFX_REQUIRE(p->stream_batch * p->levels <= OFX_MAX_LK_ITEMS, "ofx_session_create: stream_batch %d needs levels <= %d",
                p->stream_batch, OFX_MAX_LK_ITEMS / (p->stream_batch > 0 ? p->stream_batch : 1));
    OFX_REQUIRE(!p->stream_two_stage || p->borrow_frames, "ofx_session_create: stream_two_stage needs borrow_frames (the corner stage reads "
                                                            "both frames of a pair in the tick in which the second one arrives)");
    OFX_REQUIRE(p->iters <= 1 || p->mode != OFX_MODE_COMPAT_CPU, "ofx_session_create: refinement iterations need mode lk_float");
    OFX_REQUIRE(p->deep_fetch >= -1 && p->deep_fetch <= 1, "ofx_session_create: deep_fetch must be -1, 0 or +1 (got %d)", p->deep_fetch);
    OFX_REQUIRE(!p->frames_partial || (p->sharded && p->local_corner && !p->stream_two_stage),
                "ofx_session_create: frames_partial describes the frames of a sharded local_corner session (not stream_two_stage)");
    OFX_REQUIRE(p->iters <= 1 || !p->sharded || p->local_corner,
                "ofx_session_create: refinement iterations on a sharded session run through the stream pipeline, which needs local_corner");
    OFX_REQUIRE((p->width >> (p->levels - 1)) > 0 && (p->height >> (p->levels - 1)) > 0,
                "ofx_session_create: %d levels is too many for %dx%d", p->levels, p->width, p->height);
    for (int k = 0; k + 1 < p->levels; ++k)
        OFX_REQUIRE(((p->width >> k) & 1) == 0 && ((p->height >> k) & 1) == 0,
                    "ofx_session_create: level %d is %dx%d; every level that is downsampled must have even dimensions "
                    "(the reference assumes a source stride of exactly 2*w, OptFlowCPU.cpp:117)",
                    k, p->width >> k, p->height >> k);
    OFX_HIP(hipSetDevice(p->device));

    ofx_session *s = new (std::nothrow) ofx_session();
    OFX_REQUIRE(s != nullptr, "ofx_session_create: out of host memory");
    s->p = *p;
    const int n_sets = (p->stream_two_stage ? 2 : 3) * (p->stream_batch >= 2 ? p->stream_batch : 1) + 2;
    s->n_sets = n_sets;
    size_t total = 0;
    const int n_iter_sets = p->iters > 1 ? 3 * (p->stream_batch >= 2 ? p->stream_batch : 1) : 0;
    std::vector<size_t> off_plane[kSets + 2 + 3 * kMaxBatch], off_flow, off_flow2, flow_stride;
    for (int k = 0; k < p->levels; ++k) {
        s->w[k] = p->width >> k;
        s->h[k] = p->height >> k;
        s->pitch[k] = (int)align_up((size_t)s->w[k], 64);
        if (p->sharded) {
            s->own0[k] = p->own_y0[k];
            s->own1[k] = p->own_y1[k];
            s->buf0[k] = p->buf_y0[k];
            s->buf1[k] = p->buf_y1[k];
            const bool has_comp = p->comp_y1[k] > 0;
            s->cmp0[k] = has_comp ? p->comp_y0[k] : s->own0[k];
            s->cmp1[k] = has_comp ? p->comp_y1[k] : s->own1[k];
            const bool ok = 0 <= s->buf0[k] && s->buf0[k] <= s->own0[k] && s->own0[k] <= s->own1[k] &&
                            s->own1[k] <= s->buf1[k] && s->buf1[k] <= s->h[k] && s->buf0[k] < s->buf1[k] &&
                            s->buf0[k] <= s->cmp0[k] && s->cmp0[k] <= s->own0[k] && s->own1[k] <= s->cmp1[k] &&
                            s->cmp1[k] <= s->buf1[k];
            if (!ok) {
                ofx_set_error("ofx_session_create: level %d shard rows own [%d,%d) buf [%d,%d) invalid for height %d", k,
                              s->own0[k], s->own1[k], s->buf0[k], s->buf1[k], s->h[k]);
                delete s;
                return OFX_E_INVALID;
            }
        } else {
            s->own0[k] = s->buf0[k] = s->cmp0[k] = 0;
            s->own1[k] = s->buf1[k] = s->cmp1[k] = s->h[k];
        }
        s->fl0[k] = s->own0[k];
        s->fl1[k] = s->own1[k];
        if (p->sharded && p->iters > 1) {
            const int reach = (p->window >> 1) + 1, ext = reach * (p->iters - 1);
            s->fl0[k] = s->own0[k] - ext > 0 ? s->own0[k] - ext : 0;
            s->fl1[k] = s->own1[k] + ext < s->h[k] ? s->own1[k] + ext : s->h[k];
            const int lo = s->fl0[k] - reach > 0 ? s->fl0[k] - reach : 0, hi = s->fl1[k] + reach < s->h[k] ? s->fl1[k] + reach : s->h[k];
            if (lo < s->buf0[k] || hi > s->buf1[k]) {
                ofx_set_error("ofx_session_create: level %d: %d iterations need rows [%d,%d) in the buffers (own rows +- (radius + 1) * iters), "
                              "they hold [%d,%d): plan the shard with its iterations (ShardPlan(iters=...))", k, p->iters, lo, hi, s->buf0[k], s->buf1[k]);
                delete s;
                return OFX_E_INVALID;
            }
        }
        const size_t plane_bytes = align_up((size_t)s->pitch[k] * (size_t)(s->buf1[k] - s->buf0[k]) + 64, kAlign);
        for (int t = 0; t < n_sets + 2 + n_iter_sets; ++t) {
            off_plane[t].push_back(total);
            total += plane_bytes;
        }
        off_flow.push_back(total);
        const size_t own_rows = (size_t)(s->fl1[k] - s->fl0[k]);
        const size_t flow_bytes = align_up((own_rows ? own_rows : 1) * (size_t)s->w[k] * 2 * sizeof(float), kAlign);
        total += flow_bytes;
        off_flow2.push_back(total);
        if (p->stream_batch >= 2) total += flow_bytes * (size_t)(p->stream_batch - 1);
        flow_stride.push_back(flow_bytes);
    }
    std::vector<size_t> off_patch[kSets];
    std::vector<size_t> off_pscr;
    size_t pscr_frame = 0;
    const int n_slots = p->stream_batch >= 2 ? p->stream_batch : 1;
    size_t patch_bytes[OFX_MAX_LEVELS] = {};
    const bool plain_fuse_wanted = !p->local_corner && !p->stream_two_stage && !p->sharded && p->levels >= 2 && p->levels - 1 <= 6 &&
                                   [] { const char *e = getenv("OFX_PLAIN_FUSED"); return e && atoi(e) != 0; }();
    bool plain_repair = false;
    if (p->local_corner || p->stream_two_stage || plain_fuse_wanted) {
        const int step = 1 << (p->levels - 1);
        int side = p->patch_size > 0 ? p->patch_size : step * ((p->window >> 1) + 2 + 8);
        if (p->patch_size <= 0 && side < 256) side = 256;
        if (plain_fuse_wanted && p->patch_size <= 0) {
            const char *e = getenv("OFX_PLAIN_PATCH");
            if (e && atoi(e) > 0) side = atoi(e);
        }
        side = (int)align_up((size_t)side, (size_t)step);
        const int pw0 = side < p->width ? side : p->width, ph0 = side < p->height ? side : p->height;
        for (int k = 0; k < p->levels; ++k) {
            s->pw[k] = pw0 >> k;
            s->ph[k] = ph0 >> k;
            s->ppitch[k] = (int)align_up((size_t)s->pw[k], 64);
            patch_bytes[k] = align_up((size_t)s->ppitch[k] * (size_t)s->ph[k] + 64, kAlign);
        }
        const int need = (p->window >> 1) + 2;
        const int lc = p->levels - 1;
        if (!plain_fuse_wanted && (s->pw[lc] < (need < s->w[lc] ? need : s->w[lc]) || s->ph[lc] < (need < s->h[lc] ? need : s->h[lc]))) {
            ofx_set_error("ofx_session_create: patch_size %d leaves %dx%d at the coarsest level, the corner needs %d", side, s->pw[lc],
                          s->ph[lc], need);
            delete s;
            return OFX_E_INVALID;
        }
        const int need_r = (p->window >> 1) + 5;
        const bool room = (s->pw[lc] >= need_r || s->pw[lc] >= s->w[lc]) && (s->ph[lc] >= need_r || s->ph[lc] >= s->h[lc]);
        s->repair = !plain_fuse_wanted && p->borrow_frames && !p->frames_partial && p->levels >= 3 && room;
        if (plain_fuse_wanted) {
            const bool whole = pw0 == p->width && ph0 == p->height;
            const bool enough = s->pw[lc] >= (need < s->w[lc] ? need : s->w[lc]) && s->ph[lc] >= (need < s->h[lc] ? need : s->h[lc]);
            bool even = true;
            for (int k = 0; k + 1 < p->levels; ++k) even = even && (s->pw[k] & 1) == 0 && (s->ph[k] & 1) == 0;
            plain_repair = p->levels >= 3 && room && !whole;
            s->plain_fuse = enough && even && (whole || plain_repair);
        }
    }
    if (s->repair || plain_repair) {
        const char *e = getenv("OFX_DEBUG_CORNER_EXTENT");
        s->debug_extent = e ? atoi(e) : 0;
    }
    const int frames_per_slot = (p->stream_two_stage || s->plain_fuse ? 2 : 0) + (s->repair || (s->plain_fuse && plain_repair) ? 1 : 0);
    if (p->local_corner || p->stream_two_stage || s->plain_fuse) {
        for (int k = 0; k < p->levels; ++k) {
            off_pscr.push_back(pscr_frame);
            if (k >= 1) pscr_frame += patch_bytes[k];
            if (p->stream_two_stage || s->plain_fuse) continue;
            for (int t = 0; t < n_sets; ++t) {
                off_patch[t].push_back(total);
                total += patch_bytes[k];
            }
        }
        const size_t off_pscr_base = total;
        total += pscr_frame * (size_t)frames_per_slot * (size_t)n_slots;
        for (size_t &o : off_pscr) o += off_pscr_base;
    }
    const size_t off_status = total;
    total += align_up(sizeof(int) * (size_t)(1 + kUvSlots), kAlign);
    const size_t off_uv = total;
    total += align_up((size_t)OFX_MAX_LEVELS * 2 * sizeof(float) * kUvSlots, kAlign);
    const size_t off_staging = total;
    if (!p->sharded) total += align_up((size_t)p->width * (size_t)p->height * 3, kAlign);

    hipError_t e = hipMalloc(&s->arena, total);
    if (e != hipSuccess) {
        ofx_set_error("ofx_session_create: hipMalloc(%zu bytes): %s", total, hipGetErrorString(e));
        delete s;
        return OFX_E_HIP;
    }
    s->arena_bytes = total;
    e = hipMemset(s->arena, 0, total);
    if (e != hipSuccess) {
        ofx_set_error("ofx_session_create: hipMemset: %s", hipGetErrorString(e));
        (void)hipFree(s->arena);
        delete s;
        return OFX_E_HIP;
    }
    uint8_t *base = static_cast<uint8_t *>(s->arena);
    for (int k = 0; k < p->levels; ++k) {
        for (int t = 0; t < n_sets; ++t) s->img[t][k] = base + off_plane[t][k];
        for (int t = 0; t < 2; ++t) s->sh[t][k] = base + off_plane[n_sets + t][k];
        for (int t = 0; t < n_iter_sets; ++t) s->itsh[t / 3][t % 3][k] = base + off_plane[n_sets + 2 + t][k];
        s->flowset[0][k] = reinterpret_cast<float *>(base + off_flow[k]);
        for (int t = 1; t < kMaxBatch; ++t)
            s->flowset[t][k] = reinterpret_cast<float *>(base + (t < p->stream_batch ? off_flow2[k] + (size_t)(t - 1) * flow_stride[k] : off_flow[k]));
        s->flow[k] = s->flowset[0][k];
    }
    if (p->local_corner && !p->stream_two_stage)
        for (int k = 0; k < p->levels; ++k)
            for (int t = 0; t < n_sets; ++t) s->pimg[t][k] = base + off_patch[t][k];
    for (int i = 0; i < n_slots && frames_per_slot > 0; ++i)
        for (int k = 1; k < p->levels; ++k) {
            uint8_t *slot = base + off_pscr[k] + (size_t)(frames_per_slot * i) * pscr_frame;
            if (p->stream_two_stage || s->plain_fuse) {
                s->pscr[i][0][k] = slot;
                s->pscr[i][1][k] = slot + pscr_frame;
            }
            if (s->repair || (s->plain_fuse && plain_repair)) s->preloc[i][k] = slot + (size_t)(frames_per_slot - 1) * pscr_frame;
        }
    s->corner_status = reinterpret_cast<int *>(base + off_status);
    s->pair_status = s->corner_status + 1;
    s->uv = reinterpret_cast<float *>(base + off_uv);
    s->staging = p->sharded ? nullptr : base + off_staging;
    s->fused_iters = p->iters > 1 && [] { const char *e = getenv("OFX_ITER_FUSED"); return !e || atoi(e) != 0; }();
    if ((size_t)(s->buf1[0] - s->buf0[0]) * (size_t)s->pitch[0] >= ((size_t)1 << 31) ||
        (size_t)(s->buf1[0] - s->buf0[0]) * (size_t)s->w[0] * 8 >= ((size_t)1 << 31))
        s->fused_iters = false;
    repoint(s);
    *out = s;
    return OFX_OK;
}

extern "C" int ofx_session_destroy(ofx_session *s)
{
    if (!s) return OFX_OK;
    hipError_t e = hipSuccess;
    (void)hipSetDevice(s->p.device);
    for (hipEvent_t ev : s->ev) (void)hipEventDestroy(ev);
    if (s->ev_frame) (void)hipEventDestroy(s->ev_frame);
    if (s->ev_ready) (void)hipEventDestroy(s->ev_ready);
    for (hipEvent_t ev : s->ev_set_done)
        if (ev) (void)hipEventDestroy(ev);
    if (s->aux) (void)hipStreamDestroy(s->aux);
    if (s->arena) e = hipFree(s->arena);
    if (s->fe_arena && e == hipSuccess) e = hipFree(s->fe_arena);
    ofx_frontend_tables_free(s->fe);
    delete s;
    if (e != hipSuccess) {
        ofx_set_error("ofx_session_destroy: hipFree: %s", hipGetErrorString(e));
        return OFX_E_HIP;
    }
    return OFX_OK;
}

static void new_next(ofx_session *s)
{
    ++s->img_gen[(s->cur + 1) % 3];
    s->corner_done = false;
}

static int load_level0(ofx_session *s, const uint8_t *src, bool src_is_host, int src_pitch, hipStream_t st)
{
    const int rows = s->buf1[0] - s->buf0[0];
    if (s->pframe[(s->cur + 1) % 3]) {
        s->pframe[(s->cur + 1) % 3] = nullptr;
        repoint(s);
    }
    OFX_HIP(hipMemcpy2DAsync(s->plane[1][0], (size_t)s->pitch[0], src + (size_t)s->buf0[0] * (size_t)src_pitch, (size_t)src_pitch,
                             (size_t)s->w[0], (size_t)rows, src_is_host ? hipMemcpyHostToDevice : hipMemcpyDeviceToDevice, st));
    s->have_next = true;
    new_next(s);
    return OFX_OK;
}

extern "C" int ofx_session_set_frame_host(ofx_session *s, const uint8_t *h_gray1, void *stream)
{
    OFX_REQUIRE(s && h_gray1, "ofx_session_set_frame_host: null argument");
    return load_level0(s, h_gray1, true, s->w[0], ofx_stream(stream));
}

extern "C" int ofx_session_set_frame_device(ofx_session *s, const uint8_t *d_gray1, int pitch, void *stream)
{
    OFX_REQUIRE(s && d_gray1, "ofx_session_set_frame_device: null argument");
    OFX_REQUIRE(pitch >= s->w[0], "ofx_session_set_frame_device: pitch %d < width %d", pitch, s->w[0]);
    if (s->p.borrow_frames) {
        OFX_REQUIRE(pitch == s->pitch[0] && ((uintptr_t)d_gray1 & 3) == 0,
                    "ofx_session_set_frame_device: a borrowed frame needs the session's level-0 pitch (%d bytes: the width rounded up to 64; "
                    "got %d) and a 4-byte aligned address", s->pitch[0], pitch);
        s->pframe[(s->cur + 1) % 3] = d_gray1;
        repoint(s);
        s->have_next = true;
        new_next(s);
        return OFX_OK;
    }
    return load_level0(s, d_gray1, false, pitch, ofx_stream(stream));
}

extern "C" int ofx_session_set_frame_host_3ch(ofx_session *s, const uint8_t *h_img3, void *stream)
{
    OFX_REQUIRE(s && h_img3, "ofx_session_set_frame_host_3ch: null argument");
    OFX_REQUIRE(!s->p.sharded, "ofx_session_set_frame_host_3ch: not available on a sharded session");
    hipStream_t st = ofx_stream(stream);
    if (s->pframe[(s->cur + 1) % 3]) {
        s->pframe[(s->cur + 1) % 3] = nullptr;
        repoint(s);
    }
    OFX_HIP(hipMemcpyAsync(s->staging, h_img3, (size_t)s->w[0] * (size_t)s->h[0] * 3, hipMemcpyHostToDevice, st));
    OFX_TRY(ofx_extract_ch0(s->staging, s->plane[1][0], s->w[0], s->h[0], s->pitch[0], stream));
    s->have_next = true;
    new_next(s);
    return OFX_OK;
}

extern "C" int ofx_session_downsample_level(ofx_session *s, int k, void *stream)
{
    OFX_REQUIRE(s, "ofx_session_downsample_level: null session");
    OFX_REQUIRE(k >= 1 && k < s->p.levels, "ofx_session_downsample_level: level %d out of range", k);
    OFX_REQUIRE(s->have_next, "ofx_session_downsample_level: no frame loaded");
    const ofx_geom g = level_geom(s, k, s->cmp0[k], s->cmp1[k]);
    return ofx_downsample_1ch(s->plane[1][k - 1], s->pitch[k - 1], s->buf0[k - 1], s->buf1[k - 1] - s->buf0[k - 1],
                              s->plane[1][k], &g, stream);
}

static int build_pyramid(ofx_session *s, void *stream)
{
    if (s->p.levels == 1) return OFX_OK;
    if (!s->p.sharded && s->p.levels - 1 <= 6) {
        uint8_t *lv[OFX_MAX_LEVELS] = {};
        int pitches[OFX_MAX_LEVELS] = {};
        for (int k = 1; k < s->p.levels; ++k) {
            lv[k] = s->plane[1][k];
            pitches[k] = s->pitch[k];
        }
        if (s->plain_fuse && s->have_prev && (s->pitch0_next() & 3) == 0 && (((uintptr_t)s->plane[0][0] | (uintptr_t)s->plane[1][0]) & 3) == 0) {
            const int L = s->p.levels, ip = s->cur, in = (s->cur + 1) % 3;
            int have = -1;
            for (int t = 0; t < 2; ++t)
                if (s->pset_img[t] == ip && s->pset_gen[t] == s->img_gen[ip]) have = t;
            const int tp = have >= 0 ? have : 0, tn = 1 - tp;
            ofx_corner_stage C{};
            C.levels = L;
            C.d_uv = s->uv_cur();
            C.build_patch = 1;
            C.patch_w = s->pw[0];
            C.patch_h = s->ph[0];
            C.d_patch_src[0] = s->plane[0][0], C.d_patch_src[1] = s->plane[1][0];
            C.patch_src_pitch[0] = s->pitch[0], C.patch_src_pitch[1] = s->pitch0_next();
            auto extent = [&](int k, int full) {
                if (s->debug_extent <= 0 || k == 0 || s->preloc[0][1] == nullptr) return full;
                const int need = (s->p.window >> 1) + 2, lim = s->debug_extent >> k;
                const int e = lim > need ? lim : need;
                return e < full ? e : full;
            };
            for (int k = 0; k < L; ++k) {
                C.patch_pitch[k] = s->ppitch[k];
                C.d_patch[0][k] = s->pscr[0][tp][k];
                C.d_patch[1][k] = s->pscr[0][tn][k];
                C.d_patch_reloc[k] = s->preloc[0][k];
                const uint8_t *pp = k ? s->pscr[0][tp][k] : s->plane[0][0], *pn = k ? s->pscr[0][tn][k] : s->plane[1][0];
                ofx_geom pg{s->w[k], s->h[k], k ? s->ppitch[k] : s->pitch[0], 0, k ? extent(k, s->ph[k]) : s->h[0], 0, k ? extent(k, s->ph[k]) : s->h[0]};
                C.level[k] = ofx_lk_desc{pp, pn, pg, nullptr, 0, nullptr, 0, s->p.min_det};
                C.cols[k] = k ? extent(k, s->pw[k]) : 0;
            }
            OFX_TRY(timed_launch(s, OFX_TIME_PYRAMID, stream, [&] {
                return ofx_pyramid_corner_1ch(s->plane[1][0], s->pitch0_next(), s->w[0], s->h[0], lv, pitches, L, &C, have >= 0 ? 1 : 0, s->p.window, s->p.mode,
                                              stream);
            }));
            s->pset_img[tp] = ip, s->pset_gen[tp] = s->img_gen[ip];
            s->pset_img[tn] = in, s->pset_gen[tn] = s->img_gen[in];
            s->corner_done = true;
            return OFX_OK;
        }
        return timed_launch(s, OFX_TIME_PYRAMID, stream,
                            [&] { return ofx_pyramid_1ch(s->plane[1][0], s->pitch0_next(), s->w[0], s->h[0], lv, pitches, s->p.levels, stream); });
    }
    for (int k = 1; k < s->p.levels; ++k) OFX_TRY(ofx_session_downsample_level(s, k, stream));
    return OFX_OK;
}

extern "C" int ofx_session_build_pyramid(ofx_session *s, void *stream)
{
    OFX_REQUIRE(s, "ofx_session_build_pyramid: null session");
    if (!s->have_next) {
        ofx_set_error("ofx_session_build_pyramid: no frame loaded");
        return OFX_E_STATE;
    }
    return build_pyramid(s, stream);
}

extern "C" int ofx_session_compute_uv(ofx_session *s, int level, void *stream)
{
    OFX_REQUIRE(s, "ofx_session_compute_uv: null session");
    OFX_REQUIRE(level >= 0 && level < s->p.levels, "ofx_session_compute_uv: level %d out of range", level);
    if (level == s->p.levels - 1) return OFX_OK;
    const float *lv[OFX_MAX_LEVELS] = {};
    for (int k = 0; k < s->p.levels; ++k) lv[k] = s->flow[k];
    return ofx_shift_vector(lv, level, s->p.levels, s->uv_cur() + 2 * level, stream);
}

extern "C" int ofx_session_run_level(ofx_session *s, int level, void *stream)
{
    OFX_REQUIRE(s, "ofx_session_run_level: null session");
    OFX_REQUIRE(level >= 0 && level < s->p.levels, "ofx_session_run_level: level %d out of range", level);
    if (!s->have_prev || !s->have_next) {
        ofx_set_error("ofx_session_run_level: need a previous and a next frame (load, build, swap, load, build)");
        return OFX_E_STATE;
    }
    OFX_REQUIRE(!(s->p.sharded && s->p.iters > 1), "ofx_session_run_level: refinement iterations on a sharded session run through the stream "
                                                    "pipeline (ofx_session_stream_*)");
    const uint8_t *next = s->plane[1][level];
    if (level != s->p.levels - 1) {
        const int halo = (s->p.window >> 1) + 1;
        int y0 = s->own0[level] - halo, y1 = s->own1[level] + halo;
        if (y0 < s->buf0[level]) y0 = s->buf0[level];
        if (y1 > s->buf1[level]) y1 = s->buf1[level];
        const ofx_geom gs = level_geom(s, level, y0, y1);
        OFX_TRY(ofx_shift_1ch(s->plane[1][level], s->plane[2][level], &gs, s->uv_cur() + 2 * level, stream));
        next = s->plane[2][level];
    }
    const ofx_geom g = level_geom(s, level, s->own0[level], s->own1[level]);
    auto launch = [&] { return ofx_lk_level(s->plane[0][level], next, &g, s->p.window, s->p.mode, s->flow[level], s->own0[level], stream); };
    if (level != 0) return launch();
    return timed_launch(s, OFX_TIME_LK, stream, launch);
}

extern "C" int ofx_session_timing(ofx_session *s, int max_launches)
{
    OFX_REQUIRE(s && max_launches >= 0, "ofx_session_timing: bad arguments");
    for (hipEvent_t e : s->ev) (void)hipEventDestroy(e);
    s->ev.clear();
    s->ev_kind.assign((size_t)max_launches, 0);
    s->ev_used = 0;
    s->timing = max_launches > 0;
    for (int i = 0; i < 2 * max_launches; ++i) {
        hipEvent_t e;
        OFX_HIP(hipEventCreate(&e));
        s->ev.push_back(e);
    }
    return OFX_OK;
}

static int timing_stats(ofx_session *s, unsigned kind_mask, double *avg_us, double *min_us, int *launches)
{
    double sum = 0, mn = 1e30;
    int n = 0;
    for (size_t i = 0; i < s->ev_used / 2; ++i) {
        if (!((kind_mask >> s->ev_kind[i]) & 1u)) continue;
        OFX_HIP(hipEventSynchronize(s->ev[2 * i + 1]));
        float ms = 0;
        OFX_HIP(hipEventElapsedTime(&ms, s->ev[2 * i], s->ev[2 * i + 1]));
        sum += ms * 1e3;
        if (ms * 1e3 < mn) mn = ms * 1e3;
        ++n;
    }
    *avg_us = n ? sum / n : 0.0;
    if (min_us) *min_us = n ? mn : 0.0;
    *launches = n;
    return OFX_OK;
}

extern "C" int ofx_session_timing_read(ofx_session *s, double *avg_us, double *min_us, int *launches)
{
    OFX_REQUIRE(s && avg_us && launches, "ofx_session_timing_read: bad arguments");
    OFX_TRY(timing_stats(s, (1u << OFX_TIME_LK) | (1u << OFX_TIME_LK_ACC) | (1u << OFX_TIME_LK_ACC_WARP) | (1u << OFX_TIME_STREAM), avg_us, min_us, launches));
    s->ev_used = 0;
    return OFX_OK;
}

extern "C" int ofx_session_timing_read_kind(ofx_session *s, int kind, double *avg_us, double *min_us, int *launches)
{
    OFX_REQUIRE(s && avg_us && launches && kind >= 0 && kind < OFX_TIME_KINDS, "ofx_session_timing_read_kind: bad arguments");
    return timing_stats(s, 1u << kind, avg_us, min_us, launches);
}

extern "C" int ofx_session_corner_flows(ofx_session *s, void *stream)
{
    OFX_REQUIRE(s, "ofx_session_corner_flows: null session");
    if (!s->have_prev || !s->have_next) {
        ofx_set_error("ofx_session_corner_flows: need a previous and a next frame");
        return OFX_E_STATE;
    }
    if (s->corner_done) return OFX_OK;
    ofx_lk_desc d[OFX_MAX_LEVELS];
    for (int k = 0; k < s->p.levels; ++k)
        d[k] = ofx_lk_desc{s->plane[0][k], s->plane[1][k], level_geom(s, k, s->own0[k], s->own1[k]), nullptr, s->own0[k], nullptr, 0, s->p.min_det};
    return timed_launch(s, OFX_TIME_CORNER, stream, [&] { return ofx_corner_flows(d, s->p.levels, s->p.window, s->p.mode, s->uv_cur(), stream); });
}

static int timed_lk_launch(ofx_session *s, const ofx_lk_desc *lk, int nl, void *stream)
{
    return timed_launch(s, lk[0].accumulate ? (lk[0].d_warp_out ? OFX_TIME_LK_ACC_WARP : OFX_TIME_LK_ACC) : OFX_TIME_LK, stream,
                        [&] { return ofx_lk_levels(lk, nl, s->p.window, s->p.mode, stream); });
}

static int lk_all_levels(ofx_session *s, const float *uv, void *stream)
{
    const int L = s->p.levels;
    ofx_lk_desc lk[OFX_MAX_LEVELS];
    if (s->p.iters <= 1) {
        int nl = 0;
        for (int k = L - 1; k >= 0; --k)
            lk[nl++] = ofx_lk_desc{s->plane[0][k], s->plane[1][k], level_geom(s, k, s->own0[k], s->own1[k]), s->flow[k], s->own0[k],
                                   k == L - 1 ? nullptr : uv + 2 * k, 0, s->p.min_det};
        return timed_lk_launch(s, lk, nl, stream);
    }
    OFX_REQUIRE(!s->p.sharded, "refinement iterations on a sharded session run through the stream pipeline (ofx_session_stream_*)");
    ofx_shift_desc sd[OFX_MAX_LEVELS];
    int ns = 0;
    for (int k = L - 2; k >= 0; --k)
        sd[ns++] = ofx_shift_desc{s->plane[1][k], s->sh[0][k], level_geom(s, k, 0, s->h[k]), uv + 2 * k};
    if (ns) OFX_TRY(timed_launch(s, OFX_TIME_SHIFT, stream, [&] { return ofx_shift_levels(sd, ns, stream); }));
    auto src = [&](int k) { return k == L - 1 ? s->plane[1][k] : s->sh[0][k]; };
    uint8_t *const *wbuf[2] = {s->sh[1], s->itsh[0][2]};
    int nl = 0;
    for (int k = L - 1; k >= 0; --k) {
        lk[nl] = ofx_lk_desc{s->plane[0][k], src(k), level_geom(s, k, 0, s->h[k]), s->flow[k], 0, nullptr, 0, s->p.min_det};
        if (s->fused_iters) lk[nl].d_warp_src = src(k), lk[nl].d_warp_out = wbuf[0][k], lk[nl].warp_scale = OFX_ITER_SCALE;
        ++nl;
    }
    OFX_TRY(timed_lk_launch(s, lk, nl, stream));
    for (int it = 1; it < s->p.iters; ++it) {
        const bool fused = s->fused_iters, need_warp = !fused, wout = fused && it + 1 < s->p.iters;
        uint8_t *const *win = fused ? wbuf[(it - 1) & 1] : s->sh[1], *const *wnext = wbuf[it & 1];
        ofx_warp_desc wd[OFX_MAX_LEVELS];
        nl = 0;
        for (int k = L - 1; k >= 0; --k) {
            wd[nl] = ofx_warp_desc{src(k), win[k], level_geom(s, k, 0, s->h[k]), s->flow[k], 0, OFX_ITER_SCALE, nullptr, 0};
            lk[nl] = ofx_lk_desc{s->plane[0][k], win[k], level_geom(s, k, 0, s->h[k]), s->flow[k], 0, nullptr, 1, s->p.min_det};
            if (wout) lk[nl].d_warp_src = src(k), lk[nl].d_warp_out = wnext[k], lk[nl].warp_scale = OFX_ITER_SCALE;
            ++nl;
        }
        if (need_warp) OFX_TRY(timed_launch(s, OFX_TIME_WARP, stream, [&] { return ofx_warp_levels(wd, nl, stream); }));
        OFX_TRY(timed_lk_launch(s, lk, nl, stream));
    }
    return OFX_OK;
}

static void shard_reach(const ofx_session *s, int (*rows)[4])
{
    const int reach = s->p.window / 2 + 1;
    for (int k = 0; k < s->p.levels; ++k) {
        const int n0 = s->fl0[k] - reach, n1 = s->fl1[k] + reach;
        rows[k][0] = n0 < 0 ? 0 : n0;
        rows[k][1] = n1 > s->h[k] ? s->h[k] : n1;
        rows[k][2] = s->buf0[k];
        rows[k][3] = s->buf1[k];
    }
}

extern "C" int ofx_session_run_levels(ofx_session *s, void *stream)
{
    OFX_REQUIRE(s, "ofx_session_run_levels: null session");
    if (!s->have_prev || !s->have_next) {
        ofx_set_error("ofx_session_run_levels: need a previous and a next frame");
        return OFX_E_STATE;
    }
    if (s->p.sharded && !s->p.local_corner && s->p.levels > 1) {
        int rows[OFX_MAX_LEVELS][4];
        shard_reach(s, rows);
        OFX_TRY(ofx_shard_margin_check(s->uv_cur(), s->p.levels, s->h, &rows[0][0], s->corner_status, stream));
    }
    return lk_all_levels(s, s->uv_cur(), stream);
}

extern "C" int ofx_session_run_flow(ofx_session *s, void *stream)
{
    OFX_REQUIRE(s, "ofx_session_run_flow: null session");
    OFX_REQUIRE(!s->p.sharded || s->buf0[0] == 0, "ofx_session_run_flow: on a sharded session only the rank holding row 0 can "
                                                   "form the shift vectors; use corner_flows + broadcast + run_levels");
    OFX_TRY(ofx_session_corner_flows(s, stream));
    return ofx_session_run_levels(s, stream);
}

extern "C" int ofx_session_run_flow_sequential(ofx_session *s, void *stream)
{
    OFX_REQUIRE(s, "ofx_session_run_flow_sequential: null session");
    for (int k = s->p.levels - 1; k >= 0; --k) {
        OFX_TRY(ofx_session_compute_uv(s, k, stream));
        OFX_TRY(ofx_session_run_level(s, k, stream));
    }
    return OFX_OK;
}

extern "C" int ofx_session_swap(ofx_session *s)
{
    OFX_REQUIRE(s, "ofx_session_swap: null session");
    s->cur = (s->cur + 1) % 3;
    s->uv_slot ^= 1;
    repoint(s);
    s->have_prev = s->have_next;
    s->have_next = false;
    s->staged = false;
    s->corner_done = false;
    return OFX_OK;
}

static int ensure_pipeline(ofx_session *s)
{
    if (s->ev_ready) return OFX_OK;
    OFX_HIP(hipEventCreateWithFlags(&s->ev_ready, hipEventDisableTiming));
    OFX_HIP(hipEventCreateWithFlags(&s->ev_frame, hipEventDisableTiming));
    for (int i = 0; i < 3; ++i) OFX_HIP(hipEventCreateWithFlags(&s->ev_set_done[i], hipEventDisableTiming));
    int prio_lo = 0, prio_hi = 0;
    OFX_HIP(hipDeviceGetStreamPriorityRange(&prio_lo, &prio_hi));
    OFX_HIP(hipStreamCreateWithPriority(&s->aux, hipStreamNonBlocking, prio_hi));
    return OFX_OK;
}

extern "C" int ofx_session_aux_stream(ofx_session *s, void **stream)
{
    OFX_REQUIRE(s && stream, "ofx_session_aux_stream: null argument");
    OFX_TRY(ensure_pipeline(s));
    *stream = s->aux;
    return OFX_OK;
}

extern "C" int ofx_session_stage_frame(ofx_session *s, const uint8_t *d_gray1, int pitch, void *aux_stream)
{
    OFX_REQUIRE(s && d_gray1, "ofx_session_stage_frame: null argument");
    OFX_REQUIRE(pitch >= s->w[0], "ofx_session_stage_frame: pitch %d < width %d", pitch, s->w[0]);
    if (!s->have_prev) {
        ofx_set_error("ofx_session_stage_frame: no previous frame (load, build, swap first)");
        return OFX_E_STATE;
    }
    OFX_TRY(ensure_pipeline(s));
    hipStream_t aux = aux_stream ? ofx_stream(aux_stream) : s->aux;
    const int nxt = (s->cur + 1) % 3;
    if (s->set_busy[nxt]) OFX_HIP(hipStreamWaitEvent(aux, s->ev_set_done[nxt], 0));
    OFX_TRY(load_level0(s, d_gray1, false, pitch, aux));
    return build_pyramid(s, aux);
}

extern "C" int ofx_session_stage_shift(ofx_session *s, void *aux_stream)
{
    OFX_REQUIRE(s, "ofx_session_stage_shift: null session");
    if (!s->have_prev || !s->have_next) {
        ofx_set_error("ofx_session_stage_shift: stage a frame first");
        return OFX_E_STATE;
    }
    OFX_TRY(ensure_pipeline(s));
    hipStream_t aux = aux_stream ? ofx_stream(aux_stream) : s->aux;
    OFX_HIP(hipEventRecord(s->ev_ready, aux));
    s->staged = true;
    return OFX_OK;
}

extern "C" int ofx_session_solve_staged(ofx_session *s, void *stream)
{
    OFX_REQUIRE(s, "ofx_session_solve_staged: null session");
    if (!s->staged) {
        ofx_set_error("ofx_session_solve_staged: nothing staged (stage_frame, corner_flows, stage_shift first)");
        return OFX_E_STATE;
    }
    hipStream_t st = ofx_stream(stream);
    OFX_HIP(hipStreamWaitEvent(st, s->ev_ready, 0));
    OFX_TRY(lk_all_levels(s, s->uv_cur(), stream));
    OFX_HIP(hipEventRecord(s->ev_set_done[s->cur], st));
    s->set_busy[s->cur] = true;
    return ofx_session_swap(s);
}

extern "C" int ofx_session_submit_device(ofx_session *s, const uint8_t *d_gray1, int pitch, void *stream)
{
    OFX_REQUIRE(s, "ofx_session_submit_device: null session");
    OFX_REQUIRE(!s->p.sharded || s->buf0[0] == 0, "ofx_session_submit_device: on a sharded session drive the halves yourself "
                                                   "(stage_frame, corner_flows on the rank holding row 0, broadcast, stage_shift, "
                                                   "solve_staged)");
    OFX_TRY(ensure_pipeline(s));
    OFX_HIP(hipEventRecord(s->ev_frame, ofx_stream(stream)));
    OFX_HIP(hipStreamWaitEvent(s->aux, s->ev_frame, 0));
    OFX_TRY(ofx_session_stage_frame(s, d_gray1, pitch, nullptr));
    OFX_TRY(ofx_session_corner_flows(s, s->aux));
    OFX_TRY(ofx_session_stage_shift(s, nullptr));
    return ofx_session_solve_staged(s, stream);
}

extern "C" int ofx_session_plane(ofx_session *s, int which, int level, uint8_t **d_ptr, ofx_geom *geom)
{
    OFX_REQUIRE(s && which >= 0 && which < 3 && level >= 0 && level < s->p.levels, "ofx_session_plane: bad arguments");
    if (d_ptr) *d_ptr = s->plane[which][level];
    if (geom) *geom = level_geom(s, level, s->own0[level], s->own1[level]);
    return OFX_OK;
}

extern "C" int ofx_session_flow(ofx_session *s, int level, float **d_ptr, int *row0, int *rows)
{
    OFX_REQUIRE(s && level >= 0 && level < s->p.levels, "ofx_session_flow: bad arguments");
    if (d_ptr) *d_ptr = s->flow[level] + s->flow_own_offset(level);
    if (row0) *row0 = s->own0[level];
    if (rows) *rows = s->own1[level] - s->own0[level];
    return OFX_OK;
}

extern "C" int ofx_session_shift_uv(ofx_session *s, int level, float **d_uv)
{
    OFX_REQUIRE(s && d_uv && level >= 0 && level < s->p.levels, "ofx_session_shift_uv: bad arguments");
    *d_uv = s->uv_cur() + 2 * level;
    return OFX_OK;
}

extern "C" int ofx_session_get_flow_host(ofx_session *s, int level, float *h_dst, void *stream)
{
    OFX_REQUIRE(s && h_dst && level >= 0 && level < s->p.levels, "ofx_session_get_flow_host: bad arguments");
    const size_t bytes = (size_t)(s->own1[level] - s->own0[level]) * (size_t)s->w[level] * 2 * sizeof(float);
    hipStream_t st = ofx_stream(stream);
    OFX_HIP(hipMemcpyAsync(h_dst, s->flow[level] + s->flow_own_offset(level), bytes, hipMemcpyDeviceToHost, st));
    OFX_HIP(hipStreamSynchronize(st));
    return OFX_OK;
}

extern "C" int ofx_session_corner_status(ofx_session *s, int *h_status, void *stream)
{
    OFX_REQUIRE(s && h_status, "ofx_session_corner_status: null argument");
    hipStream_t st = ofx_stream(stream);
    OFX_HIP(hipMemcpyAsync(h_status, s->corner_status, sizeof(int), hipMemcpyDeviceToHost, st));
    OFX_HIP(hipMemsetAsync(s->corner_status, 0, sizeof(int), st));
    OFX_HIP(hipStreamSynchronize(st));
    return OFX_OK;
}

extern "C" int ofx_session_pair_status(ofx_session *s, int pair, int *h_status, void *stream)
{
    OFX_REQUIRE(s && h_status, "ofx_session_pair_status: null argument");
    const int slots = 2 * (s->p.stream_batch >= 2 ? s->p.stream_batch : 1);
    OFX_REQUIRE(pair >= 1, "ofx_session_pair_status: pairs are counted from 1 (frame 0 -> frame 1)");
    OFX_REQUIRE(pair <= s->corner_newest && pair > s->corner_newest - slots,
                "ofx_session_pair_status: pair %d is not among the newest %d pairs whose corner stage has run (newest: %ld)", pair, slots, s->corner_newest);
    hipStream_t st = ofx_stream(stream);
    OFX_HIP(hipMemcpyAsync(h_status, s->pair_status + (pair % slots), sizeof(int), hipMemcpyDeviceToHost, st));
    OFX_HIP(hipStreamSynchronize(st));
    return OFX_OK;
}

static int stream_batch_of(const ofx_session *s) { return s->p.stream_batch >= 2 ? s->p.stream_batch : 1; }
static int stream_sets(const ofx_session *s) { return (s->p.stream_two_stage ? 2 : 3) * stream_batch_of(s) + 2; }

static int compose_ring(ofx_session *s, long first, long last, void *stream)
{
    const int B = stream_batch_of(s), lv = s->ring_level;
    static thread_local ofx_compose_batch cb;
    memset(&cb, 0, sizeof cb);
    cb.w = s->w[lv];
    cb.rows = s->own1[lv] - s->own0[lv];
    cb.n_px = (unsigned)((size_t)cb.w * (size_t)cb.rows);
    cb.levels = s->p.levels;
    cb.level = lv;
    for (int k = 0; k < s->p.levels; ++k) cb.own0[k] = s->own0[k];
    for (long p = first; p <= last; ++p, ++cb.n) {
        for (int k = lv; k < s->p.levels; ++k) cb.lv[cb.n][k] = s->flowset[p % B][k] + s->flow_own_offset(k);
        cb.dst[cb.n] = reinterpret_cast<float *>(reinterpret_cast<char *>(s->ring) + (size_t)((p - 1) % s->ring_slots) * s->ring_stride);
    }
    s->composed = last;
    return timed_launch(s, OFX_TIME_COMPOSE, stream, [&] { return ofx_compose_batch_launch(&cb, stream); });
}

static int sample_ring(ofx_session *s, long first, long last, void *stream)
{
    const int B = stream_batch_of(s);
    static thread_local ofx_sample_batch sb;
    memset(&sb, 0, sizeof sb);
    sb.levels = s->p.levels;
    for (int k = 0; k < s->p.levels; ++k) sb.own0[k] = s->own0[k];
    if (s->arrow_ring) {
        sb.a_level = s->arrow_level, sb.a_w = s->w[s->arrow_level], sb.a_h = s->h[s->arrow_level];
        sb.a_offset = s->arrow_offset, sb.a_ny = s->arrow_ny, sb.a_nx = s->arrow_nx;
    }
    if (s->trk_points) {
        sb.points = s->trk_points, sb.status = s->trk_status, sb.n_points = s->trk_n;
        sb.t_level = s->trk_level, sb.t_w = s->w[s->trk_level], sb.t_h = s->h[s->trk_level];
        sb.pair0 = (int)first;
    }
    for (long p = first; p <= last; ++p, ++sb.n) {
        for (int k = 0; k < s->p.levels; ++k) sb.lv[sb.n][k] = s->flowset[p % B][k] + s->flow_own_offset(k);
        if (s->arrow_ring)
            sb.arrows[sb.n] = reinterpret_cast<int32_t *>(reinterpret_cast<char *>(s->arrow_ring) + (size_t)((p - 1) % s->arrow_slots) * s->arrow_stride);
        if (s->trk_points && s->trk_hist)
            sb.hist[sb.n] = reinterpret_cast<float *>(reinterpret_cast<char *>(s->trk_hist) + (size_t)((p - 1) % s->trk_slots) * s->trk_stride);
    }
    s->sampled = last;
    OfxRange range("ofx.sample_ring");
    return ofx_sample_batch_launch(&sb, stream);
}

static int stream_tick(ofx_session *s, const uint8_t *const *frames, const int *pitches, int n_frames, void *stream, int *completed_pair)
{
    const int B = stream_batch_of(s);
    const int D = s->p.stream_two_stage ? 1 : 2;
    const int sets = (D + 1) * B + 2, slots = 2 * B;
    const long f0 = s->stream_n;
    const int L = s->p.levels;
    auto uvslot = [&](long pair) { return s->uv + (size_t)(pair % slots) * 2 * OFX_MAX_LEVELS; };
    auto set_of = [&](long frame) { return (int)(frame % sets); };
    const long last_frame = s->stream_frames >= 0 ? s->stream_frames - 1 : f0 + n_frames - 1;
    auto plane_of = [&](long frame, int k) -> const uint8_t * {
        const int set = set_of(frame);
        if (k == 0 && s->p.borrow_frames) return s->bframe[set] + (size_t)s->buf0[0] * (size_t)s->bpitch[set];
        return s->img[set][k];
    };
    auto patch_of = [&](long frame, int k) -> const uint8_t * {
        const int set = set_of(frame);
        return (k == 0 && s->p.borrow_frames) ? s->bframe[set] : s->pimg[set][k];
    };
    auto pitch_of = [&](long frame, int k, bool patch) {
        if (k == 0 && s->p.borrow_frames) return s->bpitch[set_of(frame)];
        return patch ? s->ppitch[k] : s->pitch[k];
    };
    auto chain_extent = [&](int k, int full) {
        if (s->debug_extent <= 0 || k == 0) return full;
        const int need = (s->p.window >> 1) + 2, lim = s->debug_extent >> k;
        const int e = lim > need ? lim : need;
        return e < full ? e : full;
    };
    static thread_local ofx_stream_stages g;
    memset(&g, 0, sizeof g);
    for (int i = 0; i < n_frames; ++i) {
        OFX_REQUIRE(pitches[i] >= s->w[0] && (pitches[i] & 3) == 0 && ((uintptr_t)frames[i] & 3) == 0,
                    "ofx_session_stream_submit: frame must be 4-byte aligned with a pitch multiple of 4 and >= width");
        if (s->p.borrow_frames && f0 + i >= 1)
            OFX_REQUIRE(pitches[i] == s->bpitch[set_of(f0 + i - 1)] || (i > 0 && pitches[i] == pitches[i - 1]),
                        "ofx_session_stream_submit: borrowed frames must all have the same pitch");
        ofx_pyramid_stage &P = g.pyr[g.n_pyr++];
        const int set = set_of(f0 + i);
        P.d_frame = frames[i];
        P.frame_pitch = pitches[i];
        P.w = s->w[0];
        P.h = s->h[0];
        P.levels = L;
        P.windowed = s->p.sharded ? 1 : 0;
        for (int k = 0; k < L; ++k) {
            P.d_levels[k] = s->img[set][k];
            P.pitches[k] = s->pitch[k];
            P.row0[k] = s->buf0[k];
            P.rows[k] = s->buf1[k] - s->buf0[k];
        }
        if (s->p.local_corner && D == 2) {
            P.patch_w = s->pw[0];
            P.patch_h = s->ph[0];
            P.patch_levels = L;
            for (int k = 0; k < L; ++k) {
                P.d_patch_levels[k] = s->pimg[set][k];
                P.patch_pitches[k] = s->ppitch[k];
            }
        }
        if (s->p.borrow_frames) {
            s->bframe[set] = frames[i];
            s->bpitch[set] = pitches[i];
            P.d_levels[0] = nullptr;
            P.d_patch_levels[0] = nullptr;
        } else if (s->stream_input == 2) {
            P.d_levels[0] = nullptr;
        }
    }
    for (long pc = f0 - (D - 1) * B; pc <= f0 - (D - 1) * B + B - 1; ++pc) {
        if (pc < 1 || pc > last_frame) continue;
        const int slot_i = g.n_corner;
        if (pc > s->corner_newest) s->corner_newest = pc;
        ofx_corner_stage &C = g.corner[g.n_corner++];
        C.levels = L;
        C.d_uv = uvslot(pc);
        if (D == 1) {
            C.build_patch = 1;
            C.patch_w = s->pw[0];
            C.patch_h = s->ph[0];
            for (int f = 0; f < 2; ++f) {
                C.d_patch_src[f] = s->bframe[set_of(pc - 1 + f)];
                C.patch_src_pitch[f] = s->bpitch[set_of(pc - 1 + f)];
            }
            for (int k = 0; k < L; ++k) {
                C.patch_pitch[k] = s->ppitch[k];
                C.d_patch[0][k] = s->pscr[slot_i][0][k];
                C.d_patch[1][k] = s->pscr[slot_i][1][k];
                C.d_patch_reloc[k] = s->repair ? s->preloc[slot_i][k] : nullptr;
                const uint8_t *pp = k ? s->pscr[slot_i][0][k] : C.d_patch_src[0], *pn = k ? s->pscr[slot_i][1][k] : C.d_patch_src[1];
                ofx_geom pg{s->w[k], s->h[k], k ? s->ppitch[k] : C.patch_src_pitch[1], 0, k ? chain_extent(k, s->ph[k]) : s->h[0], 0,
                            k ? chain_extent(k, s->ph[k]) : s->h[0]};
                C.level[k] = ofx_lk_desc{pp, pn, pg, nullptr, 0, nullptr, 0, s->p.min_det};
                C.cols[k] = k ? chain_extent(k, s->pw[k]) : 0;
            }
            C.d_status = s->corner_status;
            C.d_pair_status = s->pair_status + (pc % slots);
            if (s->p.sharded) shard_reach(s, C.shard_rows);
            continue;
        }
        for (int k = 0; k < L; ++k) {
            if (s->p.local_corner) {
                const bool whole0 = k == 0 && s->p.borrow_frames && !s->p.frames_partial;
                const int rows_k = whole0 ? s->h[0] : chain_extent(k, s->ph[k]);
                ofx_geom pg{s->w[k], s->h[k], pitch_of(pc, k, true), 0, rows_k, 0, rows_k};
                C.level[k] = ofx_lk_desc{patch_of(pc - 1, k), patch_of(pc, k), pg, nullptr, 0, nullptr, 0, s->p.min_det};
                C.cols[k] = whole0 ? 0 : chain_extent(k, s->pw[k]);
            } else {
                ofx_geom cg = level_geom(s, k, 0, s->h[k]);
                cg.pitch = pitch_of(pc, k, false);
                C.level[k] = ofx_lk_desc{plane_of(pc - 1, k), plane_of(pc, k), cg, nullptr, 0, nullptr, 0, s->p.min_det};
            }
        }
        C.d_pair_status = s->pair_status + (pc % slots);
        if (s->p.local_corner) {
            C.d_status = s->corner_status;
            if (s->p.sharded) shard_reach(s, C.shard_rows);
            if (s->repair) {
                C.patch_w = s->pw[0];
                C.patch_h = s->ph[0];
                for (int k = 0; k < L; ++k) {
                    C.patch_pitch[k] = s->ppitch[k];
                    C.d_patch_reloc[k] = s->preloc[slot_i][k];
                }
            }
        }
    }
    long newest = -1, oldest = -1;
    static thread_local ofx_shift_desc sd0[OFX_MAX_LK_ITEMS];
    int ns0 = 0;
    for (long pl = f0 - D * B; pl <= f0 - D * B + B - 1; ++pl) {
        if (pl < 1 || pl > last_frame) continue;
        const int b = (int)(pl % B);
        float *const *fl = s->flowset[b];
        if (s->fused_iters)
            OFX_REQUIRE(!s->p.borrow_frames || (pitch_of(pl, 0, false) == s->pitch[0] && pitch_of(pl - 1, 0, false) == s->pitch[0]),
                        "ofx_session_stream_submit: with refinement iterations borrowed frames need a row pitch of %d bytes (the "
                        "width rounded up to 64), got %d", s->pitch[0], pitch_of(pl, 0, false));
        for (int k = L - 1; k >= 0; --k) {
            ofx_geom lg = level_geom(s, k, s->fl0[k], s->fl1[k]);
            lg.pitch = pitch_of(pl, k, false);
            ofx_lk_desc &d = g.lk[g.n_lk++];
            d = ofx_lk_desc{plane_of(pl - 1, k), plane_of(pl, k), lg, fl[k], s->fl0[k], k == L - 1 ? nullptr : uvslot(pl) + 2 * k, 0, s->p.min_det};
            if (s->fused_iters) {
                const uint8_t *src = d.d_next;
                if (k != L - 1) {
                    sd0[ns0++] = ofx_shift_desc{d.d_next, s->itsh[b][0][k], level_geom(s, k, s->buf0[k], s->buf1[k]), uvslot(pl) + 2 * k};
                    src = s->itsh[b][0][k];
                }
                d.d_next = src, d.d_uv = nullptr;
                d.d_warp_src = src, d.d_warp_out = s->itsh[b][1][k], d.warp_scale = OFX_ITER_SCALE;
                if (s->p.sharded) d.d_warp_status = s->corner_status, d.warp_status_bit = 16 + k;
            }
        }
        if (oldest < 0) oldest = pl;
        newest = pl;
    }
    if (ns0) OFX_TRY(timed_launch(s, OFX_TIME_SHIFT, stream, [&] { return ofx_shift_levels(sd0, ns0, stream); }));
    *completed_pair = -1;
    if (newest > s->reported) {
        *completed_pair = (int)newest;
        s->reported = newest;
        for (int k = 0; k < L; ++k) s->flow[k] = s->flowset[newest % B][k];
    }
    bool time_it = g.n_lk > 0;
    g.deep_fetch = s->p.deep_fetch;
#ifdef OFX_EXPERIMENTS
    static const int skip = [] { const char *e = getenv("OFX_STREAM_SKIP"); return e ? atoi(e) : 0; }();
    if (skip & 1) g.n_pyr = 0;
    if (skip & 2) g.n_corner = 0;
    if (skip & 8) g.n_lk = 0;
    time_it = time_it || (skip & 8);
#endif
    if (time_it)
        OFX_TRY(timed_launch(s, OFX_TIME_STREAM, stream, [&] { return ofx_stream_launch(&g, s->p.window, s->p.mode, stream); }));
    else
        OFX_TRY(ofx_stream_launch(&g, s->p.window, s->p.mode, stream));
    if (s->p.iters > 1 && newest >= 1) {
        static thread_local ofx_shift_desc sd[OFX_MAX_LK_ITEMS];
        static thread_local ofx_warp_desc wd[OFX_MAX_LK_ITEMS];
        static thread_local ofx_lk_desc ld[OFX_MAX_LK_ITEMS];
        const int reach = s->p.window / 2 + 1;
        auto clip = [](int v, int lo, int hi) { return v < lo ? lo : (v > hi ? hi : v); };
        for (int it = 1; it < s->p.iters; ++it) {
            const bool fused = s->fused_iters, need_warp = !fused, wout = fused && it + 1 < s->p.iters;
            const int wi = fused ? 1 + ((it - 1) & 1) : 1, wo = 1 + (it & 1);
            int ns = 0, nw = 0;
            for (long pl = f0 - D * B; pl <= f0 - D * B + B - 1; ++pl) {
                if (pl < 1 || pl > last_frame) continue;
                const int b = (int)(pl % B);
                OFX_REQUIRE(!s->p.borrow_frames || (pitch_of(pl, 0, false) == s->pitch[0] && pitch_of(pl - 1, 0, false) == s->pitch[0]),
                            "ofx_session_stream_submit: with refinement iterations borrowed frames need a row pitch of %d bytes (the "
                            "width rounded up to 64), got %d", s->pitch[0], pitch_of(pl, 0, false));
                for (int k = L - 1; k >= 0; --k) {
                    const int ext = s->p.sharded ? reach * (s->p.iters - 1 - it) : 0;
                    const int a = clip(s->own0[k] - ext, 0, s->h[k]), e = clip(s->own1[k] + ext, 0, s->h[k]);
                    const int wa = clip(a - reach, s->buf0[k], s->buf1[k]), we = clip(e + reach, s->buf0[k], s->buf1[k]);
                    const uint8_t *next_k = plane_of(pl, k);
                    const uint8_t *src = next_k;
                    if (k != L - 1) {
                        if (it == 1 && !fused) sd[ns++] = ofx_shift_desc{next_k, s->itsh[b][0][k], level_geom(s, k, s->buf0[k], s->buf1[k]), uvslot(pl) + 2 * k};
                        src = s->itsh[b][0][k];
                    }
                    wd[nw] = ofx_warp_desc{src, s->itsh[b][wi][k], level_geom(s, k, wa, we), s->flowset[b][k], s->fl0[k], OFX_ITER_SCALE,
                                           s->p.sharded ? s->corner_status : nullptr, 16 + k};
                    ld[nw] = ofx_lk_desc{plane_of(pl - 1, k), s->itsh[b][wi][k], level_geom(s, k, a, e), s->flowset[b][k], s->fl0[k], nullptr, 1, s->p.min_det};
                    if (wout) {
                        ld[nw].d_warp_src = src, ld[nw].d_warp_out = s->itsh[b][wo][k], ld[nw].warp_scale = OFX_ITER_SCALE;
                        if (s->p.sharded) ld[nw].d_warp_status = s->corner_status, ld[nw].warp_status_bit = 16 + k;
                    }
                    ++nw;
                }
            }
            if (ns) OFX_TRY(timed_launch(s, OFX_TIME_SHIFT, stream, [&] { return ofx_shift_levels(sd, ns, stream); }));
            if (need_warp) OFX_TRY(timed_launch(s, OFX_TIME_WARP, stream, [&] { return ofx_warp_levels(wd, nw, stream); }));
            OFX_TRY(timed_launch(s, wout ? OFX_TIME_LK_ACC_WARP : OFX_TIME_LK_ACC, stream, [&] { return ofx_lk_levels(ld, nw, s->p.window, s->p.mode, stream); }));
        }
    }
    if (s->ring && newest >= 1) OFX_TRY(compose_ring(s, oldest, newest, stream));
    if ((s->arrow_ring || s->trk_points) && newest >= 1) OFX_TRY(sample_ring(s, oldest, newest, stream));
    s->stream_n = f0 + B;
    return OFX_OK;
}

extern "C" int ofx_session_stream_begin(ofx_session *s)
{
    OFX_REQUIRE(s, "ofx_session_stream_begin: null session");
    OFX_REQUIRE(!s->p.sharded || s->p.local_corner,
                "ofx_session_stream_begin: on a sharded session the stream pipeline needs local_corner (the corner flows "
                "computed from each frame's top-left patch); otherwise drive the staged API");
    OFX_REQUIRE(s->p.levels >= 2 && s->p.levels - 1 <= 6, "ofx_session_stream_begin: %d levels unsupported (2..7)", s->p.levels);
    if (s->aux) OFX_HIP(hipStreamSynchronize(s->aux));
    for (bool &b : s->set_busy) b = false;
    s->stream_n = 0;
    s->stream_frames = -1;
    s->n_held = 0;
    s->reported = 0;
    s->corner_newest = 0;
    s->composed = 0;
    s->sampled = 0;
    s->stream_input = 0;
    s->have_prev = s->have_next = s->staged = false;
    s->corner_done = false;
    s->pset_img[0] = s->pset_img[1] = -1;
    for (int k = 0; k < s->p.levels; ++k) s->flow[k] = s->flowset[0][k];
    return OFX_OK;
}

static int frontend_tick(ofx_session *s, const uint8_t *const *img3, const int *pitch3, int n, void *stream, int *completed_pair)
{
    const uint8_t *fr[kMaxBatch];
    int pt[kMaxBatch];
    if (n > 0) {
        uint8_t *dst[kMaxBatch];
        int dp[kMaxBatch], md[kMaxBatch];
        const int sets = stream_sets(s);
        for (int i = 0; i < n; ++i) {
            const long f = s->stream_n + i;
            dst[i] = s->p.borrow_frames ? s->fplane[f % sets] : s->img[f % sets][0];
            dp[i] = s->pitch[0];
            md[i] = f == 0 && (s->fe_flags & OFX_FRONTEND_FLAG_FIRST_GREY) ? OFX_FRONTEND_GREY : s->fe_mode;
            fr[i] = dst[i];
            pt[i] = s->pitch[0];
        }
        OfxRange range("ofx.frontend");
        OFX_TRY(ofx_frontend_run(s->fe, img3, pitch3, dst, dp, md, n, s->w[0], s->h[0], ofx_stream(stream)));
    }
    return stream_tick(s, fr, pt, n, stream, completed_pair);
}

static int stream_submit(ofx_session *s, const uint8_t *frame, int pitch, void *stream, int *completed_pair, int input, const char *who)
{
    OFX_REQUIRE(s && frame, "%s: null argument", who);
    if (s->stream_n < 0) {
        ofx_set_error("%s: call ofx_session_stream_begin first", who);
        return OFX_E_STATE;
    }
    OFX_REQUIRE(s->stream_frames < 0, "%s: the stream is being drained", who);
    if (input == 2 && !s->fe_mode) {
        ofx_set_error("%s: colour frames need the front end (ofx_session_stream_frontend)", who);
        return OFX_E_STATE;
    }
    if (s->stream_input != 0 && s->stream_input != input) {
        ofx_set_error("%s: this stream has received %s frames; a stream takes grey frames or colour frames, not both", who,
                      s->stream_input == 1 ? "grey" : "colour");
        return OFX_E_STATE;
    }
    if (input == 2)
        OFX_REQUIRE(pitch >= 3 * s->w[0] && ((uintptr_t)frame & 3) == 0,
                    "%s: a colour frame must be 4-byte aligned with a pitch of at least 3 * %d bytes (got %d)", who, s->w[0], pitch);
    s->stream_input = input;
    int dummy = -1;
    if (!completed_pair) completed_pair = &dummy;
    const int B = stream_batch_of(s);
    if (s->n_held + 1 < B) {
        s->held_frame[s->n_held] = frame;
        s->held_pitch[s->n_held] = pitch;
        ++s->n_held;
        *completed_pair = -1;
        return OFX_OK;
    }
    const uint8_t *fr[kMaxBatch];
    int pt[kMaxBatch];
    for (int i = 0; i < s->n_held; ++i) fr[i] = s->held_frame[i], pt[i] = s->held_pitch[i];
    fr[s->n_held] = frame;
    pt[s->n_held] = pitch;
    const int n = s->n_held + 1;
    s->n_held = 0;
    return input == 2 ? frontend_tick(s, fr, pt, n, stream, completed_pair) : stream_tick(s, fr, pt, n, stream, completed_pair);
}

extern "C" int ofx_session_stream_submit(ofx_session *s, const uint8_t *d_gray1, int pitch, void *stream, int *completed_pair)
{
    return stream_submit(s, d_gray1, pitch, stream, completed_pair, 1, "ofx_session_stream_submit");
}

extern "C" int ofx_session_stream_submit_3ch(ofx_session *s, const uint8_t *d_img3, int pitch, void *stream, int *completed_pair)
{
    return stream_submit(s, d_img3, pitch, stream, completed_pair, 2, "ofx_session_stream_submit_3ch");
}

extern "C" int ofx_session_stream_submit_frames_3ch(ofx_session *s, const uint8_t *const *d_img3, const int *pitches, int pitch0, int n,
                                                    void *stream, int *completed_pair)
{
    OFX_REQUIRE(s && d_img3 && n >= 1, "ofx_session_stream_submit_frames_3ch: bad arguments");
    int newest = -1;
    for (int i = 0; i < n; ++i) {
        int done = -1;
        OFX_TRY(ofx_session_stream_submit_3ch(s, d_img3[i], pitches ? pitches[i] : pitch0, stream, &done));
        newest = done > newest ? done : newest;
    }
    if (completed_pair) *completed_pair = newest;
    return OFX_OK;
}

extern "C" int ofx_session_stream_frontend(ofx_session *s, int mode, int window, double sigma_s, double sigma_b, int flags)
{
    OFX_REQUIRE(s, "ofx_session_stream_frontend: null session");
    if (s->p.sharded) {
        ofx_set_error("ofx_session_stream_frontend: not on a sharded session (each rank would filter the whole frame)");
        return OFX_E_UNSUPPORTED;
    }
    if (s->stream_n > 0 || s->n_held > 0) {
        ofx_set_error("ofx_session_stream_frontend: the stream has frames already; set the front end before the first frame of a stream");
        return OFX_E_STATE;
    }
    OFX_REQUIRE(mode == OFX_FRONTEND_OFF || mode == OFX_FRONTEND_GREY || mode == OFX_FRONTEND_BILATERAL,
                "ofx_session_stream_frontend: mode %d (OFX_FRONTEND_OFF / _GREY / _BILATERAL)", mode);
    OFX_REQUIRE((flags & ~(OFX_FRONTEND_FLAG_FAST | OFX_FRONTEND_FLAG_FIRST_GREY)) == 0, "ofx_session_stream_frontend: unknown flags %#x", flags);
    OFX_HIP(hipSetDevice(s->p.device));
    if (mode == OFX_FRONTEND_OFF) {
        ofx_frontend_tables_free(s->fe);
        s->fe = nullptr;
        s->fe_mode = s->fe_flags = 0;
        for (uint8_t *&pl : s->fplane) pl = nullptr;
        void *a = s->fe_arena;
        s->fe_arena = nullptr;
        if (a) OFX_HIP(hipFree(a));
        return OFX_OK;
    }
    ofx_frontend_tables *t = nullptr;
    OFX_TRY(ofx_frontend_tables_make(mode == OFX_FRONTEND_BILATERAL ? window : 0, sigma_s, sigma_b, &t));
    if (s->p.borrow_frames && !s->fe_arena) {
        const size_t plane = align_up((size_t)s->pitch[0] * (size_t)s->h[0] + 64, 256);
        const hipError_t e = hipMalloc(&s->fe_arena, plane * (size_t)s->n_sets);
        if (e != hipSuccess) {
            ofx_frontend_tables_free(t);
            s->fe_arena = nullptr;
            ofx_set_error("ofx_session_stream_frontend: hipMalloc(%zu bytes): %s", plane * (size_t)s->n_sets, hipGetErrorString(e));
            return OFX_E_HIP;
        }
        for (int i = 0; i < s->n_sets; ++i) s->fplane[i] = static_cast<uint8_t *>(s->fe_arena) + plane * (size_t)i;
    }
    ofx_frontend_tables_free(s->fe);
    s->fe = t;
    s->fe_mode = mode == OFX_FRONTEND_GREY ? OFX_FRONTEND_GREY : (flags & OFX_FRONTEND_FLAG_FAST) ? OFX_FRONTEND_BILATERAL_FAST : OFX_FRONTEND_BILATERAL;
    s->fe_flags = flags;
    return OFX_OK;
}

extern "C" int ofx_session_stream_submit_frames(ofx_session *s, const uint8_t *const *d_gray1, const int *pitches, int pitch0, int n,
                                                void *stream, int *completed_pair)
{
    OFX_REQUIRE(s && d_gray1 && n >= 1, "ofx_session_stream_submit_frames: bad arguments");
    int newest = -1;
    for (int i = 0; i < n; ++i) {
        int done = -1;
        OFX_TRY(ofx_session_stream_submit(s, d_gray1[i], pitches ? pitches[i] : pitch0, stream, &done));
        newest = done > newest ? done : newest;
    }
    if (completed_pair) *completed_pair = newest;
    return OFX_OK;
}

extern "C" int ofx_session_stream_drain(ofx_session *s, void *stream, int *completed_pair)
{
    OFX_REQUIRE(s && completed_pair, "ofx_session_stream_drain: null argument");
    if (s->stream_n < 0) {
        ofx_set_error("ofx_session_stream_drain: not streaming");
        return OFX_E_STATE;
    }
    const uint8_t *fr[kMaxBatch];
    int pt[kMaxBatch];
    const int n = s->n_held;
    for (int i = 0; i < n; ++i) fr[i] = s->held_frame[i], pt[i] = s->held_pitch[i];
    s->n_held = 0;
    if (s->stream_frames < 0) s->stream_frames = s->stream_n + n;
    if (n == 0 && s->reported >= s->stream_frames - 1) {
        *completed_pair = -2;
        s->stream_n = -1;
        s->stream_frames = -1;
        return OFX_OK;
    }
    return s->stream_input == 2 ? frontend_tick(s, fr, pt, n, stream, completed_pair) : stream_tick(s, fr, pt, n, stream, completed_pair);
}

extern "C" int ofx_session_flow_of(ofx_session *s, int pair, int level, float **d_ptr, int *row0, int *rows)
{
    OFX_REQUIRE(s && level >= 0 && level < s->p.levels, "ofx_session_flow_of: bad arguments");
    const int B = stream_batch_of(s);
    OFX_REQUIRE(pair >= 1 && pair <= s->reported && pair > s->reported - B,
                "ofx_session_flow_of: pair %d is not among the newest %d completed pairs (newest: %ld)", pair, B, s->reported);
    if (d_ptr) *d_ptr = s->flowset[pair % B][level] + s->flow_own_offset(level);
    if (row0) *row0 = s->own0[level];
    if (rows) *rows = s->own1[level] - s->own0[level];
    return OFX_OK;
}

extern "C" int ofx_session_stream_compose(ofx_session *s, int level, float *d_ring, size_t slot_stride_bytes, int n_slots)
{
    OFX_REQUIRE(s, "ofx_session_stream_compose: null session");
    if (s->stream_n > 0 || s->n_held > 0) {
        ofx_set_error("ofx_session_stream_compose: the stream has frames already; set the ring before the first frame of a stream");
        return OFX_E_STATE;
    }
    if (!d_ring) {
        s->ring = nullptr;
        s->composed = 0;
        return OFX_OK;
    }
    const int B = stream_batch_of(s);
    OFX_REQUIRE(level >= 0 && level < s->p.levels, "ofx_session_stream_compose: level %d out of range (0 .. %d)", level, s->p.levels - 1);
    OFX_REQUIRE(n_slots >= B, "ofx_session_stream_compose: %d slots, the ring needs at least stream_batch = %d (the pairs one call completes)",
                n_slots, B);
    const size_t slot_bytes = (size_t)(s->own1[level] - s->own0[level]) * (size_t)s->w[level] * 2 * sizeof(float);
    OFX_REQUIRE(((uintptr_t)d_ring & 15) == 0, "ofx_session_stream_compose: the ring must be 16-byte aligned");
    OFX_REQUIRE(slot_stride_bytes % 16 == 0 && slot_stride_bytes >= slot_bytes,
                "ofx_session_stream_compose: slot stride %zu bytes must be a multiple of 16 and at least the slot's %zu bytes", slot_stride_bytes,
                slot_bytes);
    if (slot_bytes / 8 >= ((size_t)1 << 31)) {
        ofx_set_error("ofx_session_stream_compose: a slot of %zu pixels is more than this build composes (2^31)", slot_bytes / 8);
        return OFX_E_UNSUPPORTED;
    }
    for (int k = level + 1; k < s->p.levels && s->own1[level] > s->own0[level]; ++k) {
        const int sc = k - level;
        if ((s->own0[level] >> sc) < s->own0[k] || ((s->own1[level] - 1) >> sc) >= s->own1[k]) {
            ofx_set_error("ofx_session_stream_compose: own rows [%d,%d) of level %d read rows [%d,%d] of level %d, which owns [%d,%d)", s->own0[level],
                          s->own1[level], level, s->own0[level] >> sc, (s->own1[level] - 1) >> sc, k, s->own0[k], s->own1[k]);
            return OFX_E_UNSUPPORTED;
        }
    }
    s->ring = d_ring;
    s->ring_stride = slot_stride_bytes;
    s->ring_slots = n_slots;
    s->ring_level = level;
    s->composed = 0;
    return OFX_OK;
}

extern "C" int ofx_session_composed_of(ofx_session *s, int pair, float **d_ptr, int *row0, int *rows)
{
    OFX_REQUIRE(s, "ofx_session_composed_of: null session");
    if (!s->ring) {
        ofx_set_error("ofx_session_composed_of: no ring set (ofx_session_stream_compose)");
        return OFX_E_STATE;
    }
    OFX_REQUIRE(pair >= 1 && pair <= s->composed && pair > s->composed - s->ring_slots,
                "ofx_session_composed_of: pair %d is not among the newest %d composed pairs (newest: %ld)", pair, s->ring_slots, s->composed);
    const int lv = s->ring_level;
    if (d_ptr) *d_ptr = reinterpret_cast<float *>(reinterpret_cast<char *>(s->ring) + (size_t)((pair - 1) % s->ring_slots) * s->ring_stride);
    if (row0) *row0 = s->own0[lv];
    if (rows) *rows = s->own1[lv] - s->own0[lv];
    return OFX_OK;
}

static int sampled_settable(ofx_session *s, const char *who)
{
    if (s->stream_n > 0 || s->n_held > 0) {
        ofx_set_error("%s: the stream has frames already; set the output before the first frame of a stream", who);
        return OFX_E_STATE;
    }
    if (s->p.sharded) {
        ofx_set_error("%s: not on a sharded session (sampled positions cross shard boundaries)", who);
        return OFX_E_UNSUPPORTED;
    }
    return OFX_OK;
}

static int sampled_ring_ok(const ofx_session *s, const void *ring, size_t stride, size_t slot_bytes, int n_slots, const char *who)
{
    const int B = stream_batch_of(s);
    OFX_REQUIRE(n_slots >= B, "%s: %d slots, the ring needs at least stream_batch = %d (the pairs one call completes)", who, n_slots, B);
    OFX_REQUIRE(((uintptr_t)ring & 15) == 0, "%s: the ring must be 16-byte aligned", who);
    OFX_REQUIRE(stride % 16 == 0 && stride >= slot_bytes, "%s: slot stride %zu bytes must be a multiple of 16 and at least the slot's %zu bytes", who,
                stride, slot_bytes);
    return OFX_OK;
}

extern "C" int ofx_session_stream_arrows(ofx_session *s, int level, int arrow_res, int32_t *d_ring, size_t slot_stride_bytes, int n_slots)
{
    const char *who = "ofx_session_stream_arrows";
    OFX_REQUIRE(s, "%s: null session", who);
    OFX_TRY(sampled_settable(s, who));
    if (!d_ring) {
        s->arrow_ring = nullptr;
        s->sampled = 0;
        return OFX_OK;
    }
    OFX_REQUIRE(level >= 0 && level < s->p.levels, "%s: level %d out of range (0 .. %d)", who, level, s->p.levels - 1);
    int offset, ny, nx;
    OFX_TRY(ofx_arrow_grid(s->w[level], s->h[level], arrow_res, &offset, &ny, &nx, who));
    OFX_TRY(ofx_check_sample_pyramid(s->w[level], s->h[level], s->p.levels, level, who));
    OFX_TRY(sampled_ring_ok(s, d_ring, slot_stride_bytes, (size_t)ny * (size_t)nx * 16, n_slots, who));
    s->arrow_ring = d_ring;
    s->arrow_stride = slot_stride_bytes;
    s->arrow_slots = n_slots;
    s->arrow_level = level;
    s->arrow_offset = offset, s->arrow_ny = ny, s->arrow_nx = nx;
    s->sampled = 0;
    return OFX_OK;
}

extern "C" int ofx_session_arrows_of(ofx_session *s, int pair, int32_t **d_ptr, int *ny, int *nx)
{
    OFX_REQUIRE(s, "ofx_session_arrows_of: null session");
    if (!s->arrow_ring) {
        ofx_set_error("ofx_session_arrows_of: no ring set (ofx_session_stream_arrows)");
        return OFX_E_STATE;
    }
    OFX_REQUIRE(pair >= 1 && pair <= s->sampled && pair > s->sampled - s->arrow_slots,
                "ofx_session_arrows_of: pair %d is not among the newest %d sampled pairs (newest: %ld)", pair, s->arrow_slots, s->sampled);
    if (d_ptr) *d_ptr = reinterpret_cast<int32_t *>(reinterpret_cast<char *>(s->arrow_ring) + (size_t)((pair - 1) % s->arrow_slots) * s->arrow_stride);
    if (ny) *ny = s->arrow_ny;
    if (nx) *nx = s->arrow_nx;
    return OFX_OK;
}

extern "C" int ofx_session_stream_tracks(ofx_session *s, int level, float *d_points, int32_t *d_status, int n_points, float *d_history,
                                         size_t slot_stride_bytes, int n_slots)
{
    const char *who = "ofx_session_stream_tracks";
    OFX_REQUIRE(s, "%s: null session", who);
    OFX_TRY(sampled_settable(s, who));
    if (!d_points) {
        s->trk_points = s->trk_hist = nullptr;
        s->trk_status = nullptr;
        return OFX_OK;
    }
    OFX_REQUIRE(level >= 0 && level < s->p.levels, "%s: level %d out of range (0 .. %d)", who, level, s->p.levels - 1);
    OFX_REQUIRE(d_status && n_points >= 1, "%s: %d points need a status word each", who, n_points);
    OFX_REQUIRE(((uintptr_t)d_points & 7) == 0 && ((uintptr_t)d_status & 3) == 0, "%s: points must be 8-byte, statuses 4-byte aligned", who);
    OFX_TRY(ofx_check_sample_pyramid(s->w[level], s->h[level], s->p.levels, level, who));
    if (d_history) OFX_TRY(sampled_ring_ok(s, d_history, slot_stride_bytes, (size_t)n_points * 8, n_slots, who));
    s->trk_points = d_points;
    s->trk_status = d_status;
    s->trk_n = n_points;
    s->trk_level = level;
    s->trk_hist = d_history;
    s->trk_stride = d_history ? slot_stride_bytes : 0;
    s->trk_slots = d_history ? n_slots : 0;
    return OFX_OK;
}

extern "C" int ofx_calc_opt_flow_host(const uint8_t *h_prev3, const uint8_t *h_next3, int w, int h, float **h_flow_pyr, int level,
                                      int max_level, int window, int mode)
{
    OFX_REQUIRE(h_prev3 && h_next3 && h_flow_pyr && w > 0 && h > 0, "ofx_calc_opt_flow_host: bad arguments");
    OFX_REQUIRE(max_level >= 1 && max_level <= OFX_MAX_LEVELS && level >= 0 && level < max_level,
                "ofx_calc_opt_flow_host: bad level %d of %d", level, max_level);
    OFX_REQUIRE(h_flow_pyr[level] != nullptr, "ofx_calc_opt_flow_host: flow level %d is null", level);
    const size_t n = (size_t)w * (size_t)h;
    const int pitch = (int)align_up((size_t)w, 64);
    const size_t plane = (size_t)pitch * (size_t)h + 64;
    ofx_compat::Scratch sc;
    uint8_t *d_p1 = sc.alloc<uint8_t>(plane), *d_n1 = sc.alloc<uint8_t>(plane), *d_s1 = sc.alloc<uint8_t>(plane);
    float *d_flow = sc.alloc<float>(2 * n);
    float *d_coarse = sc.alloc<float>(2 * OFX_MAX_LEVELS + 2);
    if (!sc.ok()) return sc.rc();
    float *d_uv = d_coarse + 2 * OFX_MAX_LEVELS;
    OFX_TRY(ofx_compat::stage_h2d_ch0(d_p1, pitch, h_prev3, w, h));
    OFX_TRY(ofx_compat::stage_h2d_ch0(d_n1, pitch, h_next3, w, h));
    ofx_geom g{w, h, pitch, 0, h, 0, h};
    const uint8_t *d_next = d_n1;
    if (level != max_level - 1) {
        float coarse[2 * OFX_MAX_LEVELS] = {};
        const float *lv[OFX_MAX_LEVELS] = {};
        for (int k = level + 1; k < max_level; ++k) {
            OFX_REQUIRE(h_flow_pyr[k] != nullptr, "ofx_calc_opt_flow_host: flow level %d is null", k);
            coarse[2 * k] = h_flow_pyr[k][0];
            coarse[2 * k + 1] = h_flow_pyr[k][1];
            lv[k] = d_coarse + 2 * k;
        }
        OFX_HIP(hipMemcpy(d_coarse, coarse, sizeof coarse, hipMemcpyHostToDevice));
        OFX_TRY(ofx_shift_vector(lv, level, max_level, d_uv, nullptr));
        OFX_TRY(ofx_shift_1ch(d_n1, d_s1, &g, d_uv, nullptr));
        d_next = d_s1;
    }
    OFX_TRY(ofx_lk_level(d_p1, d_next, &g, window, mode, d_flow, 0, nullptr));
    sc.download(h_flow_pyr[level], d_flow, 2 * n);
    return sc.rc();
}


extern "C" int ofx_compose_flow_host(float *const *h_flow_pyr, int w, int h, int levels, int level, float *h_dst)
{
    OFX_REQUIRE(h_flow_pyr && h_dst && w > 0 && h > 0, "ofx_compose_flow_host: bad arguments");
    OFX_REQUIRE(levels >= 1 && levels <= OFX_MAX_LEVELS && level >= 0 && level < levels, "ofx_compose_flow_host: bad level");
    OFX_REQUIRE(w % (1 << (levels - 1 - level)) == 0 && h % (1 << (levels - 1 - level)) == 0,
                "ofx_compose_flow_host: %dx%d is not a multiple of %d (the coarsest level's scale)", w, h, 1 << (levels - 1 - level));
    ofx_compat::Scratch sc;
    const float *d_lv[OFX_MAX_LEVELS] = {};
    for (int k = level; k < levels; ++k) {
        OFX_REQUIRE(h_flow_pyr[k] != nullptr, "ofx_compose_flow_host: flow level %d is null", k);
        d_lv[k] = sc.upload(h_flow_pyr[k], 2 * (size_t)(w >> (k - level)) * (size_t)(h >> (k - level)));
    }
    float *d_dst = sc.alloc<float>(2 * (size_t)w * (size_t)h);
    if (sc.ok()) sc.run(ofx_compose_flow(d_lv, w, h, levels, level, d_dst, nullptr));
    sc.download(h_dst, d_dst, 2 * (size_t)w * (size_t)h);
    return sc.rc();
}
```

Before: 30390 Mpix/s.

## Fuse pairs of LK refinement iterations into one kernel via LDS rings

Adds a paired-iteration LK kernel that runs two refinement iterations in a single launch. The first pass writes its flow and the warped next-frame rows into per-wave LDS ring buffers, and the second pass consumes them directly. This removes one kernel launch, one global flow round trip and one warped-plane round trip per pair. In exchange it uses ping-pong flow buffers, more LDS per wave (with lower occupancy) and extra halo rows of redundant compute per strip, since the output tile is inset.

```diff
diff --git a/cuda_optical_flow_2_amd/build.py b/cuda_optical_flow_2_amd/build.py
--- a/cuda_optical_flow_2_amd/build.py
+++ b/cuda_optical_flow_2_amd/build.py
@@ -14,7 +14,7 @@
 OBJ = os.path.join(PKG, "csrc", "_obj" + os.environ.get("OFX_BUILD_TAG", ""))
 ARCH = "gfx950"
 
-SOURCES = ["lk_inst_stream_f8.hip", "lk_inst_stream_fast8.hip", "lk_inst_stream_fw.hip", "lk_inst_stream_fastw.hip", "lk_inst_stream_fwr.hip", "lk_inst_stream_fastwr.hip", "lk_inst_iter_f4.hip", "lk_inst_iter_fast4.hip", "lk_inst_stream_f.hip", "lk_inst_stream_fast.hip", "lk_inst_stream_c.hip", "lk_inst_levels_f.hip", "lk_inst_levels_fast.hip",
+SOURCES = ["lk_inst_pair_f.hip", "lk_inst_pair_fast.hip", "lk_inst_stream_f8.hip", "lk_inst_stream_fast8.hip", "lk_inst_stream_fw.hip", "lk_inst_stream_fastw.hip", "lk_inst_stream_fwr.hip", "lk_inst_stream_fastwr.hip", "lk_inst_iter_f4.hip", "lk_inst_iter_fast4.hip", "lk_inst_stream_f.hip", "lk_inst_stream_fast.hip", "lk_inst_stream_c.hip", "lk_inst_levels_f.hip", "lk_inst_levels_fast.hip",
            "lk_inst_levels_c.hip", "lk_inst_iter_f2.hip", "lk_inst_iter_fast2.hip", "lk_inst_iter_f3.hip", "lk_inst_iter_fast3.hip", "lk_inst_iter_f1.hip", "lk_inst_iter_fast1.hip", "lk_level.hip", "corner.hip", "pyr_corner.hip", "pyramid.hip", "compose_ring.hip", "sample_ring.hip", "frontend.hip", "primitives.hip", "srm_march.hip", "ofx_core.cpp", "session.cpp",
            "compat_gpu.cpp", "compat_cpu.cpp", "compat_stage.cpp"]
 FLAGS = ["-O3", "-std=c++17", "-fPIC", "-ffp-contract=off", "-fno-slp-vectorize", f"--offload-arch={ARCH}", "-I" + INCLUDE, "-I" + CSRC,
diff --git a/cuda_optical_flow_2_amd/csrc/lk_body.h b/cuda_optical_flow_2_amd/csrc/lk_body.h
--- a/cuda_optical_flow_2_amd/csrc/lk_body.h
+++ b/cuda_optical_flow_2_amd/csrc/lk_body.h
@@ -12,7 +12,10 @@
     const uint8_t *next;
     const float *uv;
     float *flow;
-    int32_t *sums;
+    union {
+        int32_t *sums;
+        const float *flow_in;
+    };
     size_t sums_plane;
     int w, h, pitch, row0, row_end;
     int out_y0, out_y1, flow_row0;
@@ -792,6 +795,7 @@
 #include "lk_body_warp.h"
 #include "lk_body_buf.h"
 #include "lk_body_wide.h"
+#include "lk_body_pair.h"
 #undef OFX_LK_PRIO_STEP
 namespace ofx_dev {
 
diff --git a/cuda_optical_flow_2_amd/csrc/lk_body_pair.h b/cuda_optical_flow_2_amd/csrc/lk_body_pair.h
--- /dev/null
+++ b/cuda_optical_flow_2_amd/csrc/lk_body_pair.h
@@ -0,0 +1,318 @@
+#pragma once
+
+namespace ofx_dev {
+
+template <int R>
+struct TileGeomP {
+    static constexpr int INSET = (R + 1 + 3) / 4;
+    static constexpr int LO_LANE = TileGeom<R>::LO_LANE + INSET;
+    static constexpr int HI_LANE = TileGeom<R>::HI_LANE - INSET;
+    static constexpr int OUT_W = (HI_LANE - LO_LANE + 1) * 4;
+};
+static_assert(TileGeomP<4>::LO_LANE == 4 && TileGeomP<4>::HI_LANE == 59 && TileGeomP<4>::OUT_W == 224, "9x9: lanes 4..59");
+
+constexpr int kLkPairMaxR = 4;
+constexpr int pair_warp_rows(int r) { return 2 * r + 4; }
+constexpr int pair_flow_rows(int r) { return r + 3; }
+constexpr int pair_wave_lds(int r) { return kLkWaveLds + 256 * pair_warp_rows(r) + 2048 * pair_flow_rows(r); }
+static_assert(pair_wave_lds(4) == 19584 && 8 * pair_wave_lds(4) <= 160 * 1024, "two waves per SIMD at 9x9");
+
+template <int R, bool FAST, bool INTERIOR, bool WOUT>
+__device__ __forceinline__ void lk_wave_pair(const LkTable &T, int wave, int lane, uint8_t *xlds)
+{
+    constexpr int MODE = OFX_MODE_LK_FLOAT;
+    using G = TileGeomP<R>;
+    constexpr int NS = 2 * R + 1, H = R - 1, PR = 2 * R - H;
+    constexpr int kLagSteps = 2 * R + 3;
+    constexpr int WN = pair_warp_rows(R), FN = pair_flow_rows(R);
+
+    if (wave >= T.first_block[T.n]) return;
+    int level = 0, hi = T.n;
+    while (hi - level > 1) {
+        const int mid = (level + hi) >> 1;
+        if (wave >= T.first_block[mid]) level = mid;
+        else hi = mid;
+    }
+    LkArgs A = T.lv[level];
+    pin_scalar(A.w);
+    pin_scalar(A.h);
+    pin_scalar(A.pitch);
+    pin_scalar(A.min_det);
+    pin_scalar(A.warp_scale);
+    const SolveOpts sopt{A.min_det};
+    const int block = wave - T.first_block[level];
+    const int tile = block % A.tiles_x;
+    const int strip = block / A.tiles_x;
+    const int cb = tile * G::OUT_W - G::LO_LANE * 4 + 4 * lane;
+    const int ysB = A.out_y0 + strip * A.strip_h, yeB = min(ysB + A.strip_h, A.out_y1);
+    const int ysA = ysB - (R + 1), yeA = min(yeB + R + 1, A.h);
+
+    const int plane_bytes = A.h * A.pitch;
+    const __amdgpu_buffer_rsrc_t rs_prev = make_rsrc(A.prev, plane_bytes), rs_next = make_rsrc(A.next, plane_bytes);
+    const __amdgpu_buffer_rsrc_t rs_fin = make_rsrc(A.flow_in, A.h * A.w * 8), rs_flow = make_rsrc(A.flow, A.h * A.w * 8);
+    const __amdgpu_buffer_rsrc_t rs_wsrc = make_rsrc(A.warp_src, plane_bytes + 3);
+    [[maybe_unused]] __amdgpu_buffer_rsrc_t rs_wout = rs_prev;
+    if constexpr (WOUT) rs_wout = make_rsrc(A.warp_out, plane_bytes);
+
+    const bool ld_ok = INTERIOR || (cb >= 0 && cb < A.w);
+    uint32_t bmask = INTERIOR ? 0xffffffffu : 0u;
+    if constexpr (!INTERIOR) {
+#pragma unroll
+        for (int j = 0; j < 4; ++j) {
+            const bool in = (cb + j) >= 0 && (cb + j) < A.w;
+            bmask |= in ? (0xffu << (8 * j)) : 0u;
+        }
+    }
+    uint32_t col_off = ld_ok ? (uint32_t)cb : 0u;
+    uint32_t nat_off = (uint32_t)cb * 8u;
+    auto finish_row = [&](uint32_t raw) -> uint32_t {
+        if constexpr (INTERIOR) return raw;
+        else return raw & bmask;
+    };
+    const int x0 = tile * G::OUT_W;
+    const int nv = min(x0 + G::OUT_W, A.w) - x0;
+    uint32_t l16 = 16u * (uint32_t)lane;
+    const int lim = 8 * nv - 16, c16 = 16 * lane;
+    const bool st_lo4 = c16 <= lim, st_lo2 = c16 == lim + 8, st_hi4 = c16 <= lim - 1024, st_hi2 = c16 == lim + 8 - 1024;
+    const uint32_t vo_lo = st_lo4 ? l16 : (uint32_t)kOob, vo_hi = st_hi4 ? l16 + 1024u : (uint32_t)kOob;
+    const bool ragged = __any(st_lo2 || st_hi2) != 0;
+    const lds_ptr xl_w = (lds_ptr)xlds + 32 * lane;
+    const lds_ptr xl_base = (lds_ptr)xlds + 32 * G::LO_LANE;
+    const lds_ptr wring = (lds_ptr)xlds + kLkWaveLds + 4 * lane;
+    const lds_ptr fring = (lds_ptr)xlds + kLkWaveLds + 256 * WN + 32 * lane;
+    auto wslot = [&](int y) -> int { return __builtin_amdgcn_readfirstlane((int)((uint32_t)(y + 2 * WN) % (uint32_t)WN) * 256); };
+    auto fslot = [&](int y) -> int { return __builtin_amdgcn_readfirstlane((int)((uint32_t)(y + 4 * FN) % (uint32_t)FN) * 2048); };
+    [[maybe_unused]] uint32_t wvo = (uint32_t)kOob;
+    if constexpr (WOUT) {
+        const bool out_lane = lane >= G::LO_LANE && lane <= G::HI_LANE && cb < A.w;
+        wvo = out_lane ? (uint32_t)cb : (uint32_t)kOob;
+    }
+    uint32_t wmiss = 0u;
+    WarpRowState WA;
+    [[maybe_unused]] WarpRowState WB;
+    warp_row_clear(WA);
+    if constexpr (WOUT) warp_row_clear(WB);
+    const s2 two = pk_two();
+    const int fstep = A.w * 8;
+
+    const int y_limA = min(yeA + R + 1, A.h);
+    const int y_firstA = ysA - R, y_lo0A = y_firstA + H;
+    const int nstepsA = (yeA - ysA) + PR;
+    const int y_min_outA = max(0, y_firstA - 1), span_outA = max(y_limA - y_min_outA, 0);
+    auto row_offA = [&](int y) -> int { return (uint32_t)y < (uint32_t)y_limA ? y * A.pitch : kOob; };
+    auto row_off_outA = [&](int y) -> int { return (uint32_t)(y - y_min_outA) < (uint32_t)span_outA ? y * A.pitch : kOob; };
+    auto load_u32 = [&](const __amdgpu_buffer_rsrc_t &rs, int po) -> uint32_t { return __builtin_amdgcn_raw_buffer_load_b32(rs, col_off, po, 0); };
+    RowPk<MODE> wa[3];
+    {
+        uint32_t pi, ni, po = 0u, no = 0u;
+#pragma unroll
+        for (int t = 0; t < 3; ++t) {
+            const int oi = row_offA(y_lo0A - 1 + t);
+            pi = finish_row(load_u32(rs_prev, oi)), ni = finish_row(load_u32(rs_next, oi));
+            if constexpr (H > 0) {
+                const int oo = row_off_outA(y_firstA - 1 + t);
+                po = finish_row(load_u32(rs_prev, oo)), no = finish_row(load_u32(rs_next, oo));
+            }
+            unpack_pk(pi, ni, po, no, wa[t]);
+        }
+    }
+    int axx[4] = {0, 0, 0, 0}, ayy[4] = {0, 0, 0, 0}, axy[4] = {0, 0, 0, 0}, axt[4] = {0, 0, 0, 0}, ayt[4] = {0, 0, 0, 0};
+
+    auto ring_warped = [&](int y) {
+        const uint32_t wn = finish_row(warp_row_finish(WA));
+        *(__attribute__((address_space(3))) uint32_t *)(wring + wslot(y)) = wn;
+    };
+    auto stepA = [&](auto K, int s) {
+        constexpr int k = decltype(K)::value;
+        const int yy = y_lo0A + s, yo = yy - NS;
+        const bool folded = H > 0 && s < H;
+        const int yh = folded ? y_firstA + s : yo;
+        const int ro = (H > 1 && s + 1 < H) ? y_firstA + s + 2 : yo + 2;
+        const int po_in = row_offA(yy + 2), po_out = row_off_outA(ro);
+        const uint32_t pf_ip = load_u32(rs_prev, po_in), pf_in = load_u32(rs_next, po_in);
+        const uint32_t pf_op = load_u32(rs_prev, po_out), pf_on = load_u32(rs_next, po_out);
+        const bool emit = s >= PR;
+        const int yw = yy - R;
+        f32x4 old_a, old_b;
+        asm("" : "=v"(old_a), "=v"(old_b));
+        if (emit) {
+            const int fnat = __builtin_amdgcn_readfirstlane(yw >= 0 ? yw * fstep : kOob);
+            if constexpr (INTERIOR) {
+                old_a = __builtin_bit_cast(f32x4, __builtin_amdgcn_raw_buffer_load_b128(rs_fin, nat_off, fnat, 0));
+                old_b = __builtin_bit_cast(f32x4, __builtin_amdgcn_raw_buffer_load_b128(rs_fin, nat_off + 16u, fnat, 0));
+            } else {
+                auto off = [&](int j) { return ((bmask >> (8 * j)) & 1u) ? nat_off + 8u * (uint32_t)j : (uint32_t)kOob; };
+                const u32x2 p0 = __builtin_amdgcn_raw_buffer_load_b64(rs_fin, off(0), fnat, 0), p1 = __builtin_amdgcn_raw_buffer_load_b64(rs_fin, off(1), fnat, 0);
+                const u32x2 p2 = __builtin_amdgcn_raw_buffer_load_b64(rs_fin, off(2), fnat, 0), p3 = __builtin_amdgcn_raw_buffer_load_b64(rs_fin, off(3), fnat, 0);
+                old_a = __builtin_bit_cast(f32x4, u32x4{p0.x, p0.y, p1.x, p1.y});
+                old_b = __builtin_bit_cast(f32x4, u32x4{p2.x, p2.y, p3.x, p3.y});
+            }
+        }
+        const uint32_t him = folded ? 0x00010000u : (yo >= y_firstA ? 0xffff0000u : 0u);
+        uint32_t rowm = ((uint32_t)yy < (uint32_t)A.h ? 0x00000001u : 0u) | ((uint32_t)yh < (uint32_t)A.h ? him : 0u);
+        if constexpr (INTERIOR) rowm = (uint32_t)__builtin_amdgcn_readfirstlane((int)rowm);
+        uint32_t mm[4];
+#pragma unroll
+        for (int j = 0; j < 4; ++j) mm[j] = INTERIOR ? rowm : ((uint32_t)__builtin_amdgcn_sbfe((int)bmask, 8 * j, 1) & rowm);
+        s2 ix[4], iy[4], it[4];
+        derivs_pk(wa[k], wa[(k + 1) % 3], wa[(k + 2) % 3], two, ix, iy, it);
+        accumulate_pk(ix, iy, it, mm, axx, ayy, axy, axt, ayt);
+        if (emit) {
+            float uv[8];
+            int hb[5][4];
+            {
+                int va[5][4];
+#pragma unroll
+                for (int j = 0; j < 4; ++j) va[0][j] = axx[j], va[1][j] = ayy[j], va[2][j] = axy[j], va[3][j] = axt[j], va[4][j] = ayt[j];
+                hbox4x5<R>(va, hb);
+            }
+            solve_lane<MODE, FAST>(hb[0], hb[1], hb[2], hb[3], hb[4], sopt, uv);
+            uv[0] = old_a.x + uv[0], uv[1] = old_a.y + uv[1], uv[2] = old_a.z + uv[2], uv[3] = old_a.w + uv[3];
+            uv[4] = old_b.x + uv[4], uv[5] = old_b.y + uv[5], uv[6] = old_b.z + uv[6], uv[7] = old_b.w + uv[7];
+            ring_warped(yw - 1);
+            const float fu[4] = {uv[0], uv[2], uv[4], uv[6]}, fv[4] = {uv[1], uv[3], uv[5], uv[7]};
+            warp_row_prepare<false>(rs_wsrc, A.warp_scale, A.w, A.h, A.pitch, 0, A.h, cb, yw, 4, fu, fv, WA, wmiss);
+            const lds_ptr fr = fring + fslot(yw);
+            *(__attribute__((address_space(3))) f32x4 *)(fr) = f32x4{uv[0], uv[1], uv[2], uv[3]};
+            *(__attribute__((address_space(3))) f32x4 *)(fr + 16) = f32x4{uv[4], uv[5], uv[6], uv[7]};
+        }
+        unpack_pk(finish_row(pf_ip), finish_row(pf_in), finish_row(pf_op), finish_row(pf_on), wa[k]);
+        pin_row(wa[k]);
+    };
+
+    const int y_limB = min(yeB + R + 1, A.h);
+    const int y_firstB = ysB - R, y_lo0B = y_firstB + H;
+    const int nstepsB = (yeB - ysB) + PR;
+    const int y_min_outB = max(0, y_firstB - 1), span_outB = max(y_limB - y_min_outB, 0);
+    auto row_offB = [&](int y) -> int { return (uint32_t)y < (uint32_t)y_limB ? y * A.pitch : kOob; };
+    auto row_off_outB = [&](int y) -> int { return (uint32_t)(y - y_min_outB) < (uint32_t)span_outB ? y * A.pitch : kOob; };
+    auto ring_row = [&](int y, int po) -> uint32_t {
+        uint32_t v = 0u;
+        if (po != kOob) v = *(const __attribute__((address_space(3))) uint32_t *)(wring + wslot(y));
+        return v;
+    };
+    RowPk<MODE> wb[3];
+    uint32_t pfb_i = 0u, pfb_o = 0u;
+    int bxx[4] = {0, 0, 0, 0}, byy[4] = {0, 0, 0, 0}, bxy[4] = {0, 0, 0, 0}, bxt[4] = {0, 0, 0, 0}, byt[4] = {0, 0, 0, 0};
+    const int fso0 = __builtin_amdgcn_readfirstlane((ysB * A.w + x0) * 8);
+    auto high_rowB = [&](int s) -> int { return (H > 0 && (s == 0 || s < H)) ? y_firstB + s + 1 : y_lo0B + s - NS + 1; };
+    auto primeB = [&]() {
+        uint32_t pi, ni, po = 0u, no = 0u;
+#pragma unroll
+        for (int t = 0; t < 2; ++t) {
+            const int yi = y_lo0B - 1 + t, oi = row_offB(yi);
+            pi = finish_row(load_u32(rs_prev, oi)), ni = ring_row(yi, oi);
+            if constexpr (H > 0) {
+                const int yo = y_firstB - 1 + t, oo = row_off_outB(yo);
+                po = finish_row(load_u32(rs_prev, oo)), no = ring_row(yo, oo);
+            }
+            unpack_pk(pi, ni, po, no, wb[t]);
+        }
+        pfb_i = load_u32(rs_prev, row_offB(y_lo0B + 1));
+        pfb_o = load_u32(rs_prev, H > 0 ? row_off_outB(high_rowB(0)) : kOob);
+    };
+    auto store_row = [&](int s_row, const f32x4 xlo, const f32x4 xhi) {
+        const int fso = __builtin_amdgcn_readfirstlane(fso0 + (s_row - PR) * fstep);
+        __builtin_amdgcn_raw_buffer_store_b128(__builtin_bit_cast(u32x4, xlo), rs_flow, INTERIOR ? lane_off_var(l16) : vo_lo, fso, kLkStoreAux);
+        __builtin_amdgcn_raw_buffer_store_b128(__builtin_bit_cast(u32x4, xhi), rs_flow, vo_hi, fso, kLkStoreAux);
+        if (__builtin_expect(ragged, 0)) {
+            const u32x4 ql = __builtin_bit_cast(u32x4, xlo), qh = __builtin_bit_cast(u32x4, xhi);
+            __builtin_amdgcn_raw_buffer_store_b64(u32x2{ql.x, ql.y}, rs_flow, st_lo2 ? l16 : (uint32_t)kOob, fso, kLkStoreAux);
+            __builtin_amdgcn_raw_buffer_store_b64(u32x2{qh.x, qh.y}, rs_flow, st_hi2 ? l16 + 1024u : (uint32_t)kOob, fso, kLkStoreAux);
+        }
+    };
+    auto stepB = [&](auto K, int s) {
+        constexpr int k = decltype(K)::value;
+        const int yy = y_lo0B + s, yo = yy - NS;
+        const bool folded = H > 0 && s < H;
+        const int yh = folded ? y_firstB + s : yo;
+        {
+            const int rh = high_rowB(s);
+            const int oi = row_offB(yy + 1), oo = (H > 0 || s > 0) ? row_off_outB(rh) : kOob;
+            unpack_pk(finish_row(pfb_i), ring_row(yy + 1, oi), finish_row(pfb_o), ring_row(rh, oo), wb[(k + 2) % 3]);
+            pin_row(wb[(k + 2) % 3]);
+            pfb_i = load_u32(rs_prev, row_offB(yy + 2));
+            pfb_o = load_u32(rs_prev, row_off_outB(high_rowB(s + 1)));
+        }
+        const bool emit = s >= PR;
+        const int yw = yy - R;
+        f32x4 old_a, old_b;
+        asm("" : "=v"(old_a), "=v"(old_b));
+        if (emit) {
+            const lds_ptr fr = fring + fslot(yw);
+            old_a = *(const __attribute__((address_space(3))) f32x4 *)(fr);
+            old_b = *(const __attribute__((address_space(3))) f32x4 *)(fr + 16);
+        }
+        const uint32_t him = folded ? 0x00010000u : (yo >= y_firstB ? 0xffff0000u : 0u);
+        uint32_t rowm = ((uint32_t)yy < (uint32_t)A.h ? 0x00000001u : 0u) | ((uint32_t)yh < (uint32_t)A.h ? him : 0u);
+        if constexpr (INTERIOR) rowm = (uint32_t)__builtin_amdgcn_readfirstlane((int)rowm);
+        uint32_t mm[4];
+#pragma unroll
+        for (int j = 0; j < 4; ++j) mm[j] = INTERIOR ? rowm : ((uint32_t)__builtin_amdgcn_sbfe((int)bmask, 8 * j, 1) & rowm);
+        s2 ix[4], iy[4], it[4];
+        derivs_pk(wb[k], wb[(k + 1) % 3], wb[(k + 2) % 3], two, ix, iy, it);
+        accumulate_pk(ix, iy, it, mm, bxx, byy, bxy, bxt, byt);
+        if (emit) {
+            float uv[8];
+            int hb[5][4];
+            {
+                int va[5][4];
+#pragma unroll
+                for (int j = 0; j < 4; ++j) va[0][j] = bxx[j], va[1][j] = byy[j], va[2][j] = bxy[j], va[3][j] = bxt[j], va[4][j] = byt[j];
+                hbox4x5<R>(va, hb);
+            }
+            solve_lane<MODE, FAST>(hb[0], hb[1], hb[2], hb[3], hb[4], sopt, uv);
+            uv[0] = old_a.x + uv[0], uv[1] = old_a.y + uv[1], uv[2] = old_a.z + uv[2], uv[3] = old_a.w + uv[3];
+            uv[4] = old_b.x + uv[4], uv[5] = old_b.y + uv[5], uv[6] = old_b.z + uv[6], uv[7] = old_b.w + uv[7];
+            if constexpr (WOUT) {
+                const uint32_t wn = warp_row_finish(WB);
+                const int wso = __builtin_amdgcn_readfirstlane(s > PR ? (yw - 1) * A.pitch : kOob);
+                __builtin_amdgcn_raw_buffer_store_b32(wn, rs_wout, wvo, wso, 0);
+                const float fu[4] = {uv[0], uv[2], uv[4], uv[6]}, fv[4] = {uv[1], uv[3], uv[5], uv[7]};
+                warp_row_prepare<false>(rs_wsrc, A.warp_scale, A.w, A.h, A.pitch, 0, A.h, cb, yw, 4, fu, fv, WB, wmiss);
+            }
+            *(__attribute__((address_space(3))) f32x4 *)(xl_w) = f32x4{uv[0], uv[1], uv[2], uv[3]};
+            *(__attribute__((address_space(3))) f32x4 *)(xl_w + 16) = f32x4{uv[4], uv[5], uv[6], uv[7]};
+            __builtin_amdgcn_fence(__ATOMIC_SEQ_CST, "wavefront");
+            __builtin_amdgcn_wave_barrier();
+            const lds_ptr xl_r = xl_base + lane_off_var(l16);
+            const f32x4 xlo = *(__attribute__((address_space(3))) f32x4 *)(xl_r);
+            const f32x4 xhi = *(__attribute__((address_space(3))) f32x4 *)(xl_r + 1024);
+            store_row(s, xlo, xhi);
+        }
+    };
+
+    const int nsteps = nstepsB + kLagSteps;
+    auto body = [&](auto K, int t) {
+        constexpr int k = decltype(K)::value;
+        constexpr int kb = (k + 3 - kLagSteps % 3) % 3;
+        if (t < nstepsA) stepA(K, t);
+        else if (t == nstepsA) ring_warped(yeA - 1);
+        if (t >= kLagSteps) {
+            __builtin_amdgcn_fence(__ATOMIC_SEQ_CST, "wavefront");
+            __builtin_amdgcn_wave_barrier();
+            if constexpr (kb == 0) {
+                if (t == kLagSteps) primeB();
+            }
+            stepB(std::integral_constant<int, kb>{}, t - kLagSteps);
+        }
+    };
+    const int q1 = nsteps / 4, q2 = nsteps / 2, q3 = nsteps - nsteps / 4;
+    __builtin_amdgcn_s_setprio(3);
+    int s = 0;
+    while (true) {
+        body(std::integral_constant<int, 0>{}, s);
+        if (++s >= nsteps) break;
+        body(std::integral_constant<int, 1>{}, s);
+        if (++s >= nsteps) break;
+        body(std::integral_constant<int, 2>{}, s);
+        if (++s >= nsteps) break;
+        OFX_LK_PRIO_STEP();
+    }
+    if constexpr (WOUT) {
+        const uint32_t wn = warp_row_finish(WB);
+        __builtin_amdgcn_raw_buffer_store_b32(wn, rs_wout, wvo, (yeB - 1) * A.pitch, 0);
+    }
+}
+
+}
diff --git a/cuda_optical_flow_2_amd/csrc/lk_inst.h b/cuda_optical_flow_2_amd/csrc/lk_inst.h
--- a/cuda_optical_flow_2_amd/csrc/lk_inst.h
+++ b/cuda_optical_flow_2_amd/csrc/lk_inst.h
@@ -36,6 +36,15 @@
     return rc;
 }
 
+template <bool FAST, bool WOUT>
+int iter_pair(int radius, const LkLevelIn *lv, int n, hipStream_t st)
+{
+    int rc = OFX_E_UNSUPPORTED;
+    const bool known = dispatch_radius<kLkPairMaxR>(radius, [&](auto R) { rc = launch_pair_r<decltype(R)::value, FAST, WOUT>(lv, n, st); });
+    if (!known) ofx_set_error("ofx_lk_levels_pair: window %d not supported", 2 * radius + 1);
+    return rc;
+}
+
 template <int MODE, bool FAST, int WOUT, int NC>
 int stream(int radius, const LkLevelIn *lv, int n, StreamArgs &S, const int *stage_blocks, size_t lds, hipStream_t st)
 {
diff --git a/cuda_optical_flow_2_amd/csrc/lk_inst_pair_f.hip b/cuda_optical_flow_2_amd/csrc/lk_inst_pair_f.hip
--- /dev/null
+++ b/cuda_optical_flow_2_amd/csrc/lk_inst_pair_f.hip
@@ -0,0 +1,4 @@
+#include "lk_inst.h"
+
+template int ofx_launch::iter_pair<false, false>(int, const LkLevelIn *, int, hipStream_t);
+template int ofx_launch::iter_pair<false, true>(int, const LkLevelIn *, int, hipStream_t);
diff --git a/cuda_optical_flow_2_amd/csrc/lk_inst_pair_fast.hip b/cuda_optical_flow_2_amd/csrc/lk_inst_pair_fast.hip
--- /dev/null
+++ b/cuda_optical_flow_2_amd/csrc/lk_inst_pair_fast.hip
@@ -0,0 +1,4 @@
+#include "lk_inst.h"
+
+template int ofx_launch::iter_pair<true, false>(int, const LkLevelIn *, int, hipStream_t);
+template int ofx_launch::iter_pair<true, true>(int, const LkLevelIn *, int, hipStream_t);
diff --git a/cuda_optical_flow_2_amd/csrc/lk_launch.h b/cuda_optical_flow_2_amd/csrc/lk_launch.h
--- a/cuda_optical_flow_2_amd/csrc/lk_launch.h
+++ b/cuda_optical_flow_2_amd/csrc/lk_launch.h
@@ -65,6 +65,24 @@
     else lk_wave_buf<R, MODE, FAST, false, DMA, ITER>(T, wave, lane, xlds);
 }
 
+template <int R, bool FAST, bool WOUT>
+__global__ __launch_bounds__(64, 2) void lk_pair_kernel(const LkTable T)
+{
+    __shared__ __attribute__((aligned(16))) uint8_t xlds[pair_wave_lds(R)];
+    const int wave = (int)blockIdx.x, lane = (int)threadIdx.x;
+    if (wave >= T.first_block[T.n]) return;
+    int level = 0, hi = T.n;
+    while (hi - level > 1) {
+        const int mid = (level + hi) >> 1;
+        if (wave >= T.first_block[mid]) level = mid;
+        else hi = mid;
+    }
+    const int tile = (wave - T.first_block[level]) % T.lv[level].tiles_x;
+    const int cb0 = tile * TileGeomP<R>::OUT_W - TileGeomP<R>::LO_LANE * 4;
+    if (cb0 >= 0 && cb0 + 256 <= T.lv[level].w) lk_wave_pair<R, FAST, true, WOUT>(T, wave, lane, xlds);
+    else lk_wave_pair<R, FAST, false, WOUT>(T, wave, lane, xlds);
+}
+
 using ofx_launch::kCornerScratch;
 using ofx_launch::kPyrStages;
 using ofx_launch::StreamArgs;
@@ -127,10 +145,9 @@
     return e && atoi(e) > 0 ? atoi(e) : dflt;
 }
 
-template <int R, int NC = 4>
-int plan_table(const LkLevelIn *lv, int n, int capacity, LkTable *out)
-{
-    using G = TileGeomW<R, NC>;
+template <typename G>
+int plan_table_g(const LkLevelIn *lv, int n, int capacity, LkTable *out)
+{
     const int min_h = env_int("OFX_LK_MIN_STRIP", 8);
     int max_rows = 1;
     for (int i = 0; i < n; ++i) max_rows = lv[i].rows_out > max_rows ? lv[i].rows_out : max_rows;
@@ -160,8 +177,14 @@
     return blocks;
 }
 
+template <int R, int NC = 4>
+int plan_table(const LkLevelIn *lv, int n, int capacity, LkTable *out)
+{
+    return plan_table_g<TileGeomW<R, NC>>(lv, n, capacity, out);
+}
+
 template <typename K>
-int lk_wave_target(K kernel, int threads, size_t lds, int reserve, int dflt_per_simd)
+int lk_wave_target(K kernel, int threads, size_t lds, int reserve, int dflt_per_simd, int full_fill = 95)
 {
     int dev = 0, cus = 256, per_cu = 0;
     hipDeviceProp_t prop;
@@ -172,7 +195,7 @@
     int per_simd = env_int("OFX_LK_WAVES_PER_SIMD", dflt_per_simd);
     if (per_simd > occ - reserve) per_simd = occ - reserve;
     if (per_simd < 1) per_simd = 1;
-    const int fill = env_int("OFX_LK_FILL", per_simd < occ ? 100 : 95);
+    const int fill = env_int("OFX_LK_FILL", per_simd < occ ? 100 : full_fill);
     return env_int("OFX_LK_TARGET_WAVES", (int)((long)cus * 4 * per_simd * fill / 100));
 }
 
@@ -206,6 +229,17 @@
     for (int i = 0; i < n; ++i) max_px = (long)lv[i].a.w * lv[i].a.h > max_px ? (long)lv[i].a.w * lv[i].a.h : max_px;
     if (forced > 0 || (forced < 0 && max_px >= 16l * 1000 * 1000)) return launch_iter_rd<R, MODE, FAST, ITER, true>(lv, n, st);
     return launch_iter_rd<R, MODE, FAST, ITER, false>(lv, n, st);
+}
+
+template <int R, bool FAST, bool WOUT>
+int launch_pair_r(const LkLevelIn *lv, int n, hipStream_t st)
+{
+    static const int capacity = lk_wave_target(lk_pair_kernel<R, FAST, WOUT>, 64, 0, 0, 2, 100);
+    LkTable t{};
+    const int blocks = plan_table_g<TileGeomP<R>>(lv, n, capacity, &t);
+    hipLaunchKernelGGL((lk_pair_kernel<R, FAST, WOUT>), dim3((unsigned)blocks), dim3(64), 0, st, t);
+    OFX_HIP(hipGetLastError());
+    return OFX_OK;
 }
 
 template <int R, int MODE, bool FAST, bool DMA, int WOUT, int NC = 4>
@@ -273,6 +307,8 @@
 int levels(int radius, const LkLevelIn *lv, int n, bool sums, hipStream_t st);
 template <int MODE, bool FAST, int ITER, int NC = 4>
 int iter(int radius, const LkLevelIn *lv, int n, hipStream_t st);
+template <bool FAST, bool WOUT>
+int iter_pair(int radius, const LkLevelIn *lv, int n, hipStream_t st);
 template <int MODE, bool FAST, int WOUT = 0, int NC = 4>
 int stream(int radius, const LkLevelIn *lv, int n, StreamArgs &S, const int *stage_blocks, size_t lds, hipStream_t st);
 }
diff --git a/cuda_optical_flow_2_amd/csrc/lk_level.hip b/cuda_optical_flow_2_amd/csrc/lk_level.hip
--- a/cuda_optical_flow_2_amd/csrc/lk_level.hip
+++ b/cuda_optical_flow_2_amd/csrc/lk_level.hip
@@ -275,6 +275,32 @@
     return lk_dispatch(levels, n, window, mode, nullptr, stream);
 }
 
+int ofx_lk_levels_pair(const ofx_lk_desc *d, const float *const *d_flow_in, int n, int window, int mode, void *stream)
+{
+    LkLevelIn lv[OFX_MAX_LK_ITEMS];
+    int m = 0;
+    OFX_REQUIRE(d != nullptr && d_flow_in != nullptr && n >= 1 && n <= OFX_MAX_LK_ITEMS, "ofx_lk_levels_pair: bad arguments");
+    OFX_REQUIRE(mode == OFX_MODE_LK_FLOAT || mode == OFX_MODE_LK_FLOAT_FAST, "ofx_lk_levels_pair: mode %d not supported", mode);
+    OFX_REQUIRE(window >= 3 && (window & 1) && (window >> 1) <= kLkPairMaxR, "ofx_lk_levels_pair: window %d not supported", window);
+    OFX_TRY(lk_build_levels(d, n, window, mode, nullptr, lv, &m));
+    OFX_REQUIRE(m == n, "ofx_lk_levels_pair: empty level");
+    const bool wout = d[0].d_warp_out != nullptr;
+    for (int i = 0; i < n; ++i) {
+        LkArgs &a = lv[i].a;
+        OFX_REQUIRE(a.accumulate && a.uv == nullptr && a.flow != nullptr && d_flow_in[i] != nullptr && d_flow_in[i] != a.flow && d[i].d_warp_src != nullptr,
+                    "ofx_lk_levels_pair: needs accumulate, no d_uv, d_warp_src and two distinct flow buffers");
+        OFX_REQUIRE(a.row0 == 0 && a.row_end == a.h && a.out_y0 == 0 && a.out_y1 == a.h && a.flow_row0 == 0, "ofx_lk_levels_pair: whole levels only");
+        OFX_REQUIRE(fits_buffer_offsets(a), "ofx_lk_levels_pair: levels must stay below 2 GB");
+        a.flow_in = d_flow_in[i];
+        a.warp_src = d[i].d_warp_src;
+        a.warp_scale = d[i].warp_scale;
+    }
+    hipStream_t st = ofx_stream(stream);
+    const int radius = window >> 1;
+    if (mode == OFX_MODE_LK_FLOAT_FAST) return wout ? ofx_launch::iter_pair<true, true>(radius, lv, n, st) : ofx_launch::iter_pair<true, false>(radius, lv, n, st);
+    return wout ? ofx_launch::iter_pair<false, true>(radius, lv, n, st) : ofx_launch::iter_pair<false, false>(radius, lv, n, st);
+}
+
 extern "C" int ofx_lk_level(const uint8_t *d_prev, const uint8_t *d_next, const ofx_geom *g, int window, int mode,
                             float *d_flow, int flow_row0, void *stream)
 {
diff --git a/cuda_optical_flow_2_amd/csrc/ofx_internal.h b/cuda_optical_flow_2_amd/csrc/ofx_internal.h
--- a/cuda_optical_flow_2_amd/csrc/ofx_internal.h
+++ b/cuda_optical_flow_2_amd/csrc/ofx_internal.h
@@ -67,6 +67,8 @@
                            const ofx_corner_stage *C, int first, int window, int mode, void *stream);
 int ofx_shard_margin_check(const float *d_uv, int levels, const int *heights, const int *shard_rows, int *d_status, void *stream);
 
+int ofx_lk_levels_pair(const ofx_lk_desc *levels, const float *const *d_flow_in, int n, int window, int mode, void *stream);
+
 struct ofx_compose_batch {
     const float *lv[OFX_STREAM_MAX_BATCH][OFX_MAX_LEVELS];
     float *dst[OFX_STREAM_MAX_BATCH];
diff --git a/cuda_optical_flow_2_amd/csrc/session.cpp b/cuda_optical_flow_2_amd/csrc/session.cpp
--- a/cuda_optical_flow_2_amd/csrc/session.cpp
+++ b/cuda_optical_flow_2_amd/csrc/session.cpp
@@ -7,6 +7,9 @@
 #include "compat_scratch.h"
 #include "ofx_internal.h"
 
+#ifndef OFX_ITER_PAIRS_DEFAULT
+#define OFX_ITER_PAIRS_DEFAULT 1
+#endif
 namespace {
 constexpr size_t kAlign = 256;
 constexpr int kMaxBatch = OFX_STREAM_MAX_BATCH;
@@ -27,6 +30,8 @@
     uint8_t *sh[2][OFX_MAX_LEVELS]{};
     uint8_t *itsh[kMaxBatch][3][OFX_MAX_LEVELS]{};
     bool fused_iters = false;
+    bool iter_pairs = false;
+    float *flowset2[kMaxBatch][OFX_MAX_LEVELS]{};
     int cur = 0, sht = 0;
     uint8_t *plane[3][OFX_MAX_LEVELS]{};
     hipStream_t aux = nullptr;
@@ -175,7 +180,12 @@
     s->n_sets = n_sets;
     size_t total = 0;
     const int n_iter_sets = p->iters > 1 ? 3 * (p->stream_batch >= 2 ? p->stream_batch : 1) : 0;
-    std::vector<size_t> off_plane[kSets + 2 + 3 * kMaxBatch], off_flow, off_flow2, flow_stride;
+    std::vector<size_t> off_plane[kSets + 2 + 3 * kMaxBatch], off_flow, off_flow2, off_flow_alt, flow_stride;
+    const bool want_pairs = p->iters >= 3 && !p->sharded && (p->mode == OFX_MODE_LK_FLOAT || p->mode == OFX_MODE_LK_FLOAT_FAST) &&
+                            (p->window >> 1) >= 1 && (p->window >> 1) <= 4 && (long)p->width * p->height < 16l * 1000 * 1000 &&
+                            [] { const char *e = getenv("OFX_ITER_DMA"); return !e || atoi(e) <= 0; }() &&
+                            [] { const char *e = getenv("OFX_ITER_PAIRS"); return e ? atoi(e) != 0 : OFX_ITER_PAIRS_DEFAULT != 0; }();
+    const int n_flow_slots = p->stream_batch >= 2 ? p->stream_batch : 1;
     for (int k = 0; k < p->levels; ++k) {
         s->w[k] = p->width >> k;
         s->h[k] = p->height >> k;
@@ -298,6 +308,10 @@
     total += align_up((size_t)OFX_MAX_LEVELS * 2 * sizeof(float) * kUvSlots, kAlign);
     const size_t off_staging = total;
     if (!p->sharded) total += align_up((size_t)p->width * (size_t)p->height * 3, kAlign);
+    for (int k = 0; k < p->levels; ++k) {
+        off_flow_alt.push_back(total);
+        if (want_pairs) total += flow_stride[k] * (size_t)n_flow_slots;
+    }
 
     hipError_t e = hipMalloc(&s->arena, total);
     if (e != hipSuccess) {
@@ -322,6 +336,7 @@
         for (int t = 1; t < kMaxBatch; ++t)
             s->flowset[t][k] = reinterpret_cast<float *>(base + (t < p->stream_batch ? off_flow2[k] + (size_t)(t - 1) * flow_stride[k] : off_flow[k]));
         s->flow[k] = s->flowset[0][k];
+        for (int t = 0; t < n_flow_slots && want_pairs; ++t) s->flowset2[t][k] = reinterpret_cast<float *>(base + off_flow_alt[k] + (size_t)t * flow_stride[k]);
     }
     if (p->local_corner && !p->stream_two_stage)
         for (int k = 0; k < p->levels; ++k)
@@ -343,6 +358,7 @@
     if ((size_t)(s->buf1[0] - s->buf0[0]) * (size_t)s->pitch[0] >= ((size_t)1 << 31) ||
         (size_t)(s->buf1[0] - s->buf0[0]) * (size_t)s->w[0] * 8 >= ((size_t)1 << 31))
         s->fused_iters = false;
+    s->iter_pairs = want_pairs && s->fused_iters;
     repoint(s);
     *out = s;
     return OFX_OK;
@@ -1032,7 +1048,7 @@
     for (long pl = f0 - D * B; pl <= f0 - D * B + B - 1; ++pl) {
         if (pl < 1 || pl > last_frame) continue;
         const int b = (int)(pl % B);
-        float *const *fl = s->flowset[b];
+        float *const *fl = s->iter_pairs && (((s->p.iters - 1) / 2) & 1) ? s->flowset2[b] : s->flowset[b];
         if (s->fused_iters)
             OFX_REQUIRE(!s->p.borrow_frames || (pitch_of(pl, 0, false) == s->pitch[0] && pitch_of(pl - 1, 0, false) == s->pitch[0]),
                         "ofx_session_stream_submit: with refinement iterations borrowed frames need a row pitch of %d bytes (the "
@@ -1080,11 +1096,15 @@
         static thread_local ofx_shift_desc sd[OFX_MAX_LK_ITEMS];
         static thread_local ofx_warp_desc wd[OFX_MAX_LK_ITEMS];
         static thread_local ofx_lk_desc ld[OFX_MAX_LK_ITEMS];
+        static thread_local const float *fin[OFX_MAX_LK_ITEMS];
+        bool alt = s->iter_pairs && (((s->p.iters - 1) / 2) & 1);
+        int wcur = 1;
         const int reach = s->p.window / 2 + 1;
         auto clip = [](int v, int lo, int hi) { return v < lo ? lo : (v > hi ? hi : v); };
-        for (int it = 1; it < s->p.iters; ++it) {
-            const bool fused = s->fused_iters, need_warp = !fused, wout = fused && it + 1 < s->p.iters;
-            const int wi = fused ? 1 + ((it - 1) & 1) : 1, wo = 1 + (it & 1);
+        for (int it = 1; it < s->p.iters;) {
+            const bool two = s->iter_pairs && it + 2 <= s->p.iters;
+            const bool fused = s->fused_iters, need_warp = !fused, wout = fused && it + (two ? 2 : 1) < s->p.iters;
+            const int wi = fused ? wcur : 1, wo = 3 - wi;
             int ns = 0, nw = 0;
             for (long pl = f0 - D * B; pl <= f0 - D * B + B - 1; ++pl) {
                 if (pl < 1 || pl > last_frame) continue;
@@ -1102,9 +1122,15 @@
                         if (it == 1 && !fused) sd[ns++] = ofx_shift_desc{next_k, s->itsh[b][0][k], level_geom(s, k, s->buf0[k], s->buf1[k]), uvslot(pl) + 2 * k};
                         src = s->itsh[b][0][k];
                     }
-                    wd[nw] = ofx_warp_desc{src, s->itsh[b][wi][k], level_geom(s, k, wa, we), s->flowset[b][k], s->fl0[k], OFX_ITER_SCALE,
+                    float *const fcur = alt ? s->flowset2[b][k] : s->flowset[b][k];
+                    wd[nw] = ofx_warp_desc{src, s->itsh[b][wi][k], level_geom(s, k, wa, we), fcur, s->fl0[k], OFX_ITER_SCALE,
                                            s->p.sharded ? s->corner_status : nullptr, 16 + k};
-                    ld[nw] = ofx_lk_desc{plane_of(pl - 1, k), s->itsh[b][wi][k], level_geom(s, k, a, e), s->flowset[b][k], s->fl0[k], nullptr, 1, s->p.min_det};
+                    ld[nw] = ofx_lk_desc{plane_of(pl - 1, k), s->itsh[b][wi][k], level_geom(s, k, a, e), fcur, s->fl0[k], nullptr, 1, s->p.min_det};
+                    if (two) {
+                        fin[nw] = fcur;
+                        ld[nw].d_flow = alt ? s->flowset[b][k] : s->flowset2[b][k];
+                        ld[nw].d_warp_src = src, ld[nw].warp_scale = OFX_ITER_SCALE;
+                    }
                     if (wout) {
                         ld[nw].d_warp_src = src, ld[nw].d_warp_out = s->itsh[b][wo][k], ld[nw].warp_scale = OFX_ITER_SCALE;
                         if (s->p.sharded) ld[nw].d_warp_status = s->corner_status, ld[nw].warp_status_bit = 16 + k;
@@ -1114,7 +1140,12 @@
             }
             if (ns) OFX_TRY(timed_launch(s, OFX_TIME_SHIFT, stream, [&] { return ofx_shift_levels(sd, ns, stream); }));
             if (need_warp) OFX_TRY(timed_launch(s, OFX_TIME_WARP, stream, [&] { return ofx_warp_levels(wd, nw, stream); }));
-            OFX_TRY(timed_launch(s, wout ? OFX_TIME_LK_ACC_WARP : OFX_TIME_LK_ACC, stream, [&] { return ofx_lk_levels(ld, nw, s->p.window, s->p.mode, stream); }));
+            OFX_TRY(timed_launch(s, wout ? OFX_TIME_LK_ACC_WARP : OFX_TIME_LK_ACC, stream, [&] {
+                return two ? ofx_lk_levels_pair(ld, fin, nw, s->p.window, s->p.mode, stream) : ofx_lk_levels(ld, nw, s->p.window, s->p.mode, stream);
+            }));
+            if (two) alt = !alt;
+            wcur = wo;
+            it += two ? 2 : 1;
         }
     }
     if (s->ring && newest >= 1) OFX_TRY(compose_ring(s, oldest, newest, stream));
```

Result: faster. 33440 Mpix/s, median of 6 (+10.0%).
